# Irish-77/adapting-2D-ViTs-for-3D-point-cloud-understanding

Measured on NVIDIA B200. Metric: tokenized clouds/sec (FPS+kNN+embed), higher is better.
Workload: dtype bf16

## Files before the change

### __graft_entry__.py

```python
import os
import sys

ROOT = os.path.dirname(os.path.abspath(__file__))
PKG = os.path.join(ROOT, "adapting-2d-vits-for-3d-point-cloud-understanding_b200")
for _p in (ROOT, PKG):
    if _p not in sys.path:
        sys.path.insert(0, _p)


def build() -> None:
    from p3tok import _build
    path = _build.build_library()
    print(f"[build] {path}")
    from oracle import oracle
    print(f"[build] {oracle.build()} (test oracle)")
    import p3tok
    from p3tok import _lib
    L = _lib.lib()
    missing = [s for s in _lib.declared_symbols() if not hasattr(L, s)]
    if missing:
        raise RuntimeError(f"libp3tok.so does not export {missing}")
    print(f"[build] ok: {len(_lib.declared_symbols())} C-ABI symbols exported")
    n = fps_fused_multiply_adds(path)
    if n:
        raise RuntimeError(f"fps_kernel SASS holds {n} fused multiply-adds: ptxas contracted the distance arithmetic, "
                           "FPS would no longer be bit-exact (csrc/fps.cu)")
    print("[build] ok: fps_kernel distance arithmetic is unfused (no FFMA / FFMA2 in its SASS)")


def fps_fused_multiply_adds(lib_path: str) -> int:
    import re
    import subprocess
    out = subprocess.run(["cuobjdump", "-sass", lib_path], capture_output=True, text=True).stdout
    n, inside = 0, False
    for line in out.splitlines():
        if "Function :" in line:
            inside = "fps_kernel" in line or "fps_culled_kernel" in line or "fps_nd_kernel" in line
        elif inside and re.search(r"\bFFMA2?\b", line):
            n += 1
    return n


def smoke() -> None:
    import numpy as np
    import torch
    from oracle import oracle
    from p3tok import synth
    from p3tok.modules import PointNet, P3Embed

    assert torch.cuda.is_available(), "smoke() needs a CUDA device"
    dev = torch.device("cuda:0")
    B, N, C, G, k, E = 4, 512, 3, 32, 16, 64
    x = synth.make_cloud("clustered", B, N, 77, C)
    start = synth.start_indices(B, N, 77)
    sd = synth.apf_encoder_state(E, 2 * C, 77)
    ref_tok, grp = oracle.pointnet_apf(sd, x, start, G, k)
    xt, st = torch.from_numpy(x).to(dev), torch.from_numpy(start).to(dev)
    for prec, rtol in (("fp32", 1e-4), ("bf16", 1e-2)):
        net = PointNet(E, G, k, 2 * C, precision=prec).eval().to(dev)
        net.encoder.load_state_dict(synth.to_torch_state(sd))
        fidx, ctr, kidx, perm = net.group.indices(xt, st)
        assert np.array_equal(fidx.cpu().numpy(), grp["fps_idx"]), "FPS indices differ from the oracle"
        assert np.array_equal(kidx.cpu().numpy(), grp["knn_idx"]), "kNN indices differ from the oracle"
        assert np.array_equal(perm.cpu().numpy(), grp["perm"]), "Morton order differs from the oracle"
        try:
            tok = net(xt, st).cpu().numpy().astype(np.float64)
        except Exception as e:
            if prec == "bf16" and "not built yet" in str(e):
                print("[smoke] bf16 path not built yet - skipped")
                continue
            raise
        err = np.abs(tok - ref_tok).max() / np.abs(ref_tok).max()
        print(f"[smoke] PointNet {prec}: max err / max|ref| = {err:.3e}")
        assert err < rtol, f"{prec} tokens off by {err}"
    sd2 = synth.p3embed_state(3, 1 / 16, 4, 4, 64, 78)
    mod = P3Embed(sample_ratio=1 / 16, k=8, embed_dim=64).eval().to(dev)
    mod.load_state_dict(synth.to_torch_state(sd2))
    starts = [synth.start_indices(B, N, 78, 0), synth.start_indices(B, N // 4, 78, 1)]
    ps, fs = mod(xt, xt.transpose(1, 2).contiguous(), [torch.from_numpy(s).to(dev) for s in starts])
    op, of, _ = oracle.p3embed(sd2, x, x.copy(), starts, 8, 2)
    for s in (1, 2):
        assert np.array_equal(ps[s].cpu().numpy(), op[s]), "P3Embed centres differ"
        a, b = fs[s].transpose(1, 2).cpu().numpy(), of[s]
        err = np.abs(a - b).max() / np.abs(b).max()
        print(f"[smoke] P3Embed stage {s - 1}: max err / max|ref| = {err:.3e}")
        assert err < 1e-4
    sd3 = synth.p3embed_state(3, 1 / 16, 4, 4, 256, 79)
    mod3 = P3Embed(sample_ratio=1 / 16, k=32, embed_dim=256, precision="bf16").eval().to(dev)
    mod3.load_state_dict(synth.to_torch_state(sd3))
    x3 = synth.make_cloud("uniform", 2, 1024, 79, 3)
    starts3 = [synth.start_indices(2, 1024, 79, 0), synth.start_indices(2, 256, 79, 1)]
    x3t = torch.from_numpy(x3).to(dev)
    ps3, fs3 = mod3(x3t, x3t.transpose(1, 2).contiguous(), [torch.from_numpy(s).to(dev) for s in starts3])
    op3, of3, _ = oracle.p3embed(sd3, x3, x3.copy(), starts3, 32, 2)
    for s in (1, 2):
        assert np.array_equal(ps3[s].cpu().numpy(), op3[s]), "P3Embed (bf16) centres differ"
        a, b = fs3[s].transpose(1, 2).cpu().numpy(), of3[s]
        err = np.abs(a - b).max() / np.abs(b).max()
        print(f"[smoke] P3Embed bf16 stage {s - 1}: max err / max|ref| = {err:.3e}")
        assert err < 1e-2 * s
    from p3tok.apf_model import APFViTLayer, run_blocks
    sdv = synth.apf_vit_state(E, 2, 15, 80)
    tsd = synth.to_torch_state(sdv)
    blocks = torch.nn.Sequential(*[APFViTLayer(E, 2) for _ in range(2)]).eval().to(dev)
    blocks.load_state_dict({k_[len("blocks."):]: v for k_, v in tsd.items() if k_.startswith("blocks.")})
    norm = torch.nn.LayerNorm(E).eval().to(dev)
    norm.load_state_dict({"weight": tsd["encoder_norm.weight"], "bias": tsd["encoder_norm.bias"]})
    tokv = synth.vit_tokens(B, G, E, 80)
    _, pooled = run_blocks(blocks, torch.from_numpy(tokv).to(dev), norm)
    _, op_, _ = oracle.apf_vit(sdv, tokv, 2, 2)
    err = np.abs(pooled.cpu().numpy() - op_).max() / np.abs(op_).max()
    print(f"[smoke] APF ViT block stack (2 layers): max err / max|ref| = {err:.3e}")
    assert err < 1e-2
    torch.cuda.synchronize()
    print("[smoke] ok")


if __name__ == "__main__":
    build()
    if "--smoke" in sys.argv:
        smoke()
```

### adapting-2d-vits-for-3d-point-cloud-understanding_b200/csrc/fps.cu

```cuda
#include <stdlib.h>

#include <cooperative_groups.h>
#include <cuda/ptx>

#include "common.cuh"

namespace cg = cooperative_groups;

namespace p3tok {

constexpr int FPS_PPT = 8;
constexpr int FPS_CL_PPT = 16;
constexpr int FPS_WIDE_PPT = 24;
constexpr int FPS_MAX_THREADS = 1024;
constexpr int FPS_SLICE = FPS_PPT * FPS_MAX_THREADS;
constexpr int FPS_SLICE_X = FPS_WIDE_PPT * 512;
constexpr int fps_max_threads(int ppt) { return ppt == FPS_WIDE_PPT ? 512 : FPS_SLICE / ppt; }

#ifdef P3TOK_FPS_TRACE
__device__ long long fps_trace_buf[16 * 32];
#define FPS_T(slot)                                                                                       \
  do {                                                                                                    \
    if (g == 100 && cloud == 0 && lane == 0 && (warp == 0 || warp == 5))                                  \
      fps_trace_buf[rank * 32 + (warp ? 16 : 0) + (slot)] = clock64();                                    \
    if ((slot) == 0 && (g == 200 || g == 1200) && cloud == 0 && t == 0)                                   \
      fps_trace_buf[rank * 32 + (g == 200 ? 8 : 9)] = clock64();                                          \
  } while (0)
#else
#define FPS_T(slot) do { } while (0)
#endif

struct __align__(16) FpsCand {
  uint32_t key;
  uint32_t idx;
  float x, y, z;
  uint32_t pad[3];
};

__device__ __forceinline__ void warp_argmax(uint32_t& key, uint32_t& idx) {
  const uint32_t m = __reduce_max_sync(0xffffffffu, key);
  const uint32_t cand = (key == m) ? idx : 0xffffffffu;
  idx = __reduce_min_sync(0xffffffffu, cand);
  key = m;
}

__device__ __forceinline__ uint32_t fps_smem_u32(const void* p) { return (uint32_t)__cvta_generic_to_shared(p); }
__device__ __forceinline__ void fps_push_cand(const FpsCand* local_slot, uint64_t* local_bar, uint32_t dst_cta, const FpsCand& c) {
  uint32_t ra, rb;
  asm volatile("mapa.shared::cluster.u32 %0, %1, %2;" : "=r"(ra) : "r"(fps_smem_u32(local_slot)), "r"(dst_cta));
  asm volatile("mapa.shared::cluster.u32 %0, %1, %2;" : "=r"(rb) : "r"(fps_smem_u32(local_bar)), "r"(dst_cta));
  asm volatile("st.async.weak.shared::cluster.mbarrier::complete_tx::bytes.v4.b32 [%0], {%2, %3, %4, %5}, [%1];" ::"r"(ra), "r"(rb),
               "r"(c.key), "r"(c.idx), "r"(__float_as_uint(c.x)), "r"(__float_as_uint(c.y))
               : "memory");
  asm volatile("st.async.weak.shared::cluster.mbarrier::complete_tx::bytes.v4.b32 [%0], {%2, %3, %4, %5}, [%1];" ::"r"(ra + 16), "r"(rb),
               "r"(__float_as_uint(c.z)), "r"(0u), "r"(0u), "r"(0u)
               : "memory");
}
__device__ __forceinline__ void fps_expect_cands(uint64_t* bar, uint32_t bytes) {
  asm volatile("mbarrier.arrive.expect_tx.shared::cta.b64 _, [%0], %1;" ::"r"(fps_smem_u32(bar)), "r"(bytes) : "memory");
}
__device__ __forceinline__ void fps_wait_cands(uint64_t* bar, uint32_t parity) {
  uint32_t ok = 0;
  while (!ok) {
    asm volatile(
        "{\n\t"
        ".reg .pred p;\n\t"
        "mbarrier.try_wait.parity.acquire.cluster.shared::cta.b64 p, [%1], %2;\n\t"
        "selp.u32 %0, 1, 0, p;\n\t"
        "}"
        : "=r"(ok)
        : "r"(fps_smem_u32(bar)), "r"(parity)
        : "memory");
  }
}

__device__ __forceinline__ void fps_add2(float& o0, float& o1, float a0, float a1, float b0, float b1) {
  asm("{ .reg .b64 ra, rb, rd; mov.b64 ra, {%2,%3}; mov.b64 rb, {%4,%5}; add.rn.f32x2 rd, ra, rb; mov.b64 {%0,%1}, rd; }"
      : "=f"(o0), "=f"(o1)
      : "f"(a0), "f"(a1), "f"(b0), "f"(b1));
}
__device__ __forceinline__ void fps_mul2(float& o0, float& o1, float a0, float a1, float b0, float b1) {
  asm("{ .reg .b64 ra, rb, rd; mov.b64 ra, {%2,%3}; mov.b64 rb, {%4,%5}; mul.rn.f32x2 rd, ra, rb; mov.b64 {%0,%1}, rd; }"
      : "=f"(o0), "=f"(o1)
      : "f"(a0), "f"(a1), "f"(b0), "f"(b1));
}

template <int CL, int PPT = FPS_PPT>
__global__ void __launch_bounds__(fps_max_threads(PPT), 1)
fps_kernel(const float* __restrict__ x, int N, int pt_stride, const int64_t* __restrict__ start_idx,
           int G, int64_t* __restrict__ out_idx, int slice, int ncta) {
  extern __shared__ __align__(128) unsigned char smem_raw[];
  float* rows = reinterpret_cast<float*>(smem_raw);
  const int rows_bytes = ((slice * pt_stride * 4 + 127) / 128) * 128;
  uint64_t* mbar = reinterpret_cast<uint64_t*>(smem_raw + rows_bytes);
  uint2* wslot = reinterpret_cast<uint2*>(smem_raw + rows_bytes + 16);
  FpsCand* ccand = reinterpret_cast<FpsCand*>(smem_raw + rows_bytes + 16 + 2 * 32 * sizeof(uint2));
  uint64_t* cbar = reinterpret_cast<uint64_t*>(ccand + 2 * 16);
  FpsCand* cwin = reinterpret_cast<FpsCand*>(cbar + 2);

  const int T = blockDim.x;
  const int t = threadIdx.x;
  const int lane = t & 31, warp = t >> 5, nwarps = T >> 5;
  int cloud, rank;
  if constexpr (CL > 1) {
    rank = (int)cg::this_cluster().block_rank();
    cloud = blockIdx.x / ncta;
  } else {
    rank = 0;
    cloud = blockIdx.x;
  }
  const int p0 = rank * slice;
  const int np = max(0, min(slice, N - p0));
  const float* src = x + ((size_t)cloud * N + p0) * pt_stride;

  const size_t bytes = (size_t)np * pt_stride * 4;
  const bool tma_ok = (bytes > 0) && (bytes % 16 == 0) && ((reinterpret_cast<uintptr_t>(src) & 15) == 0);
  if (tma_ok) {
    if (t == 0) {
      cuda::ptx::mbarrier_init(mbar, 1);
      cuda::ptx::fence_proxy_async(cuda::ptx::space_shared);
    }
    __syncthreads();
    if (t == 0) {
      cuda::ptx::mbarrier_arrive_expect_tx(cuda::ptx::sem_release, cuda::ptx::scope_cta,
                                           cuda::ptx::space_shared, mbar, (uint32_t)bytes);
      cuda::ptx::cp_async_bulk(cuda::ptx::space_cluster, cuda::ptx::space_global, rows, src,
                               (uint32_t)bytes, mbar);
    }
    while (!cuda::ptx::mbarrier_try_wait_parity(mbar, 0)) {
    }
  } else {
    for (int i = t; i < np * pt_stride; i += T) rows[i] = src[i];
    __syncthreads();
  }

  float px[PPT], py[PPT], pz[PPT], md[PPT];
#pragma unroll
  for (int j = 0; j < PPT; ++j) {
    const int i = j * T + t;
    if (i < np) {
      px[j] = rows[i * pt_stride + 0];
      py[j] = rows[i * pt_stride + 1];
      pz[j] = rows[i * pt_stride + 2];
      md[j] = 1e10f;
    } else {
      px[j] = py[j] = pz[j] = 0.f;
      md[j] = -2.f;
    }
  }
  int far = (int)start_idx[cloud];
  far = min(max(far, 0), N - 1);
  float cx, cy, cz;
  if constexpr (CL > 1) {
    cg::cluster_group cluster = cg::this_cluster();
    if (t == 0) {
      cuda::ptx::mbarrier_init(&cbar[0], 1);
      cuda::ptx::mbarrier_init(&cbar[1], 1);
      asm volatile("fence.mbarrier_init.release.cluster;" ::: "memory");
    }
    if (t == 0 && far >= p0 && far < p0 + np) {
      const int l = far - p0;
      FpsCand c;
      c.key = 0; c.idx = (uint32_t)far;
      c.x = rows[l * pt_stride]; c.y = rows[l * pt_stride + 1]; c.z = rows[l * pt_stride + 2];
      c.pad[0] = c.pad[1] = c.pad[2] = 0;
      for (int r = 0; r < ncta; ++r) *cluster.map_shared_rank(&ccand[0], r) = c;
    }
    cluster.sync();
    cx = ccand[0].x; cy = ccand[0].y; cz = ccand[0].z;
    cluster.sync();
  } else {
    cx = rows[far * pt_stride]; cy = rows[far * pt_stride + 1]; cz = rows[far * pt_stride + 2];
  }

  for (int g = 0; g < G; ++g) {
    if (t == 0 && rank == 0) out_idx[(size_t)cloud * G + g] = far;
    if (g == G - 1) break;
    FPS_T(0);
    const float ncx = -cx, ncy = -cy, ncz = -cz;
#pragma unroll
    for (int j = 0; j < PPT; j += 2) {
      float dx0, dx1, dy0, dy1, dz0, dz1;
      fps_add2(dx0, dx1, px[j], px[j + 1], ncx, ncx);
      fps_add2(dy0, dy1, py[j], py[j + 1], ncy, ncy);
      fps_add2(dz0, dz1, pz[j], pz[j + 1], ncz, ncz);
      fps_mul2(dx0, dx1, dx0, dx1, dx0, dx1);
      fps_mul2(dy0, dy1, dy0, dy1, dy0, dy1);
      fps_mul2(dz0, dz1, dz0, dz1, dz0, dz1);
      const float d0 = __fadd_rn(__fadd_rn(dx0, dy0), dz0);
      const float d1 = __fadd_rn(__fadd_rn(dx1, dy1), dz1);
      md[j] = fminf(md[j], d0);
      md[j + 1] = fminf(md[j + 1], d1);
    }
    float best = md[0];
#pragma unroll
    for (int j = 1; j < PPT; ++j) best = fmaxf(best, md[j]);
    uint32_t key = best >= 0.f ? __float_as_uint(best) : 0u;
    uint32_t idx = 0xffffffffu;
    {
      const uint32_t wmax = __reduce_max_sync(0xffffffffu, key);
      if (key == wmax && best >= 0.f) {
        int besti = PPT - 1;
#pragma unroll
        for (int j = PPT - 2; j >= 0; --j) besti = (md[j] == best) ? j : besti;
        idx = (uint32_t)(p0 + besti * T + t);
      }
      idx = __reduce_min_sync(0xffffffffu, idx);
      key = wmax;
    }
    const int buf = g & 1;
    FPS_T(1);
    if (lane == 0) wslot[buf * 32 + warp] = make_uint2(key, idx);
    __syncthreads();
    FPS_T(2);
    {
      const uint2 s = (lane < nwarps) ? wslot[buf * 32 + lane] : make_uint2(0u, 0xffffffffu);
      key = s.x; idx = s.y;
      warp_argmax(key, idx);
    }
    if constexpr (CL > 1) {
      if (warp == 0) {
        if (lane < ncta) {
          FpsCand c;
          c.key = key; c.idx = idx;
          if (idx != 0xffffffffu) {
            const int l = (int)idx - p0;
            c.x = rows[l * pt_stride]; c.y = rows[l * pt_stride + 1]; c.z = rows[l * pt_stride + 2];
          } else {
            c.x = c.y = c.z = 0.f;
          }
          c.pad[0] = c.pad[1] = c.pad[2] = 0;
          if (lane == 0) fps_expect_cands(&cbar[buf], (uint32_t)ncta * 32u);
          fps_push_cand(&ccand[buf * 16 + rank], &cbar[buf], (uint32_t)lane, c);
        }
        FPS_T(3);
        fps_wait_cands(&cbar[buf], (uint32_t)(g >> 1) & 1);
        FPS_T(4);
        uint32_t k2 = lane < ncta ? ccand[buf * 16 + lane].key : 0u;
        uint32_t i2 = lane < ncta ? ccand[buf * 16 + lane].idx : 0xffffffffu;
        const uint32_t mine = i2;
        warp_argmax(k2, i2);
        const uint32_t src = __ffs(__ballot_sync(0xffffffffu, lane < ncta && mine == i2)) - 1;
        if (lane == (int)src) cwin[buf] = ccand[buf * 16 + lane];
        FPS_T(5);
      }
      __syncthreads();
      FPS_T(6);
      far = (int)min(cwin[buf].idx, (uint32_t)(N - 1));
      cx = cwin[buf].x; cy = cwin[buf].y; cz = cwin[buf].z;
    } else {
      far = (int)min(idx, (uint32_t)(N - 1));
      cx = rows[far * pt_stride]; cy = rows[far * pt_stride + 1]; cz = rows[far * pt_stride + 2];
    }
  }
  if constexpr (CL > 1) cg::this_cluster().sync();
}

static size_t fps_smem_bytes(int slice, int pt_stride) {
  const size_t rows_bytes = (((size_t)slice * pt_stride * 4 + 127) / 128) * 128;
  return rows_bytes + 16 + 2 * 32 * sizeof(uint2) + 2 * 16 * sizeof(FpsCand) + 16 + 2 * sizeof(FpsCand);
}

template <int CL, int PPT>
static int fps_configure() {
  static thread_local bool configured[32] = {false};
  int dev = 0;
  P3_CUDA(cudaGetDevice(&dev));
  if (dev < 32 && !configured[dev]) {
    P3_CUDA((cudaFuncSetAttribute(fps_kernel<CL, PPT>, cudaFuncAttributeMaxDynamicSharedMemorySize, 227 * 1024)));
    if (CL > 8) P3_CUDA((cudaFuncSetAttribute(fps_kernel<CL, PPT>, cudaFuncAttributeNonPortableClusterSizeAllowed, 1)));
    configured[dev] = true;
  }
  return P3TOK_OK;
}

template <int CL, int PPT>
static int fps_max_clusters(int ncta, int threads, size_t smem) {
  if (fps_configure<CL, PPT>() != P3TOK_OK) return -1;
  cudaLaunchConfig_t cfg = {};
  cfg.gridDim = dim3((unsigned)(ncta * 64));
  cfg.blockDim = dim3((unsigned)threads);
  cfg.dynamicSmemBytes = smem;
  cudaLaunchAttribute attr[1];
  attr[0].id = cudaLaunchAttributeClusterDimension;
  attr[0].val.clusterDim.x = (unsigned)ncta;
  attr[0].val.clusterDim.y = 1;
  attr[0].val.clusterDim.z = 1;
  cfg.attrs = attr;
  cfg.numAttrs = 1;
  int n = -1;
  if (cudaOccupancyMaxActiveClusters(&n, fps_kernel<CL, PPT>, &cfg) != cudaSuccess) {
    cudaGetLastError();
    return -1;
  }
  return n;
}

template <int CL, int PPT>
static int fps_launch(const float* x, int B, int N, int pt_stride, const int64_t* start, int G,
                      int64_t* out, int slice, int threads, int ncta, cudaStream_t stream) {
  const size_t smem = fps_smem_bytes(slice, pt_stride);
  int rc = fps_configure<CL, PPT>();
  if (rc) return rc;
  const int CLr = ncta;
  cudaLaunchConfig_t cfg = {};
  cfg.gridDim = dim3((unsigned)(B * CLr));
  cfg.blockDim = dim3((unsigned)threads);
  cfg.dynamicSmemBytes = smem;
  cfg.stream = stream;
  cudaLaunchAttribute attr[1];
  attr[0].id = cudaLaunchAttributeClusterDimension;
  attr[0].val.clusterDim.x = (unsigned)CLr;
  attr[0].val.clusterDim.y = 1;
  attr[0].val.clusterDim.z = 1;
  cfg.attrs = attr;
  cfg.numAttrs = CL > 1 ? 1 : 0;
  P3_CUDA((cudaLaunchKernelEx(&cfg, fps_kernel<CL, PPT>, x, N, pt_stride, start, G, out, slice, ncta)));
  count_launch();
  return P3TOK_OK;
}

}

using namespace p3tok;

extern "C" int p3tok_fps(const float* x, int64_t B, int64_t N, int64_t pt_stride,
                         const int64_t* start_idx, int64_t G, int64_t* out_idx, void* stream) {
  P3_REQUIRE(B >= 0 && N > 0 && G >= 0 && pt_stride >= 3, P3TOK_ERR_INVALID,
             "fps: bad shape B=%lld N=%lld G=%lld stride=%lld", (long long)B, (long long)N, (long long)G,
             (long long)pt_stride);
  if (B == 0 || G == 0) return P3TOK_OK;
  P3_REQUIRE(x && start_idx && out_idx, P3TOK_ERR_INVALID, "fps: null pointer");
  P3_REQUIRE(pt_stride <= 4, P3TOK_ERR_UNSUPPORTED, "fps: pt_stride %lld > 4 (pass xyz or xyz+height rows)",
             (long long)pt_stride);
  P3_REQUIRE(N <= (int64_t)FPS_SLICE * 16, P3TOK_ERR_UNSUPPORTED, "fps: N=%lld exceeds 131072", (long long)N);
  P3_REQUIRE(B * 16 < (1ll << 31) && B * G < (1ll << 40), P3TOK_ERR_UNSUPPORTED, "fps: batch too large");
  cudaStream_t s = as_stream(stream);
  const int Bi = (int)B, Ni = (int)N, Gi = (int)G, ps = (int)pt_stride;
  if (N <= FPS_SLICE) {
    static int ppt_env = -1;
    if (ppt_env < 0) { const char* e = getenv("P3TOK_FPS_PPT"); ppt_env = e ? atoi(e) : 0; }
    const int ppt = ppt_env ? ppt_env : (Ni >= 1024 ? 16 : 8);
    int threads = ((Ni + ppt - 1) / ppt + 31) / 32 * 32;
    if (threads < 32) threads = 32;
    if (ppt == 32) return fps_launch<1, 32>(x, Bi, Ni, ps, start_idx, Gi, out_idx, Ni, threads, 1, s);
    if (ppt == 16) return fps_launch<1, 16>(x, Bi, Ni, ps, start_idx, Gi, out_idx, Ni, threads, 1, s);
    return fps_launch<1, 8>(x, Bi, Ni, ps, start_idx, Gi, out_idx, Ni, threads, 1, s);
  }
  const int lo = (Ni + FPS_SLICE_X - 1) / FPS_SLICE_X;
  const int hi = (Ni + FPS_SLICE - 1) / FPS_SLICE <= 8 ? 8 : 16;
  static thread_local int seats[32][17][33];
  int dev = 0;
  P3_CUDA(cudaGetDevice(&dev));
  static int cl_env = -1;
  if (cl_env < 0) { const char* e = getenv("P3TOK_FPS_CLUSTER"); cl_env = e ? atoi(e) : 0; }
  int best_cl = 0, best_threads = 0, best_slice = 0;
  double best_cost = 0;
  for (int cl = hi; cl >= lo && cl >= 1; --cl) {
    if (cl_env >= lo && cl_env <= hi && cl != cl_env) continue;
    const int slice = (Ni + cl - 1) / cl;
    const bool wide = slice > FPS_SLICE;
    if (wide && cl > 8) continue;
    const int ppt = wide ? FPS_WIDE_PPT : FPS_CL_PPT;
    const int threads = ((slice + ppt - 1) / ppt + 31) / 32 * 32;
    if (threads > fps_max_threads(ppt)) continue;
    int n = dev < 32 ? seats[dev][cl][threads / 32] : 0;
    if (n == 0) {
      const size_t sm = fps_smem_bytes(slice, ps);
      n = cl > 8 ? fps_max_clusters<16, FPS_CL_PPT>(cl, threads, sm)
                 : wide ? fps_max_clusters<8, FPS_WIDE_PPT>(cl, threads, sm) : fps_max_clusters<8, FPS_CL_PPT>(cl, threads, sm);
      if (n <= 0) n = -1;
      if (dev < 32) seats[dev][cl][threads / 32] = n;
    }
    if (n < 0) n = 148 / cl;
    const double cost = (double)((Bi + n - 1) / n) * (1000.0 + 0.11 * slice);
    if (best_cl == 0 || cost < best_cost) { best_cl = cl; best_cost = cost; best_threads = threads; best_slice = slice; }
  }
  P3_REQUIRE(best_cl > 0, P3TOK_ERR_UNSUPPORTED, "fps: no cluster size for N=%lld", (long long)N);
  if (best_cl > 8) return fps_launch<16, FPS_CL_PPT>(x, Bi, Ni, ps, start_idx, Gi, out_idx, best_slice, best_threads, best_cl, s);
  if (best_slice > FPS_SLICE)
    return fps_launch<8, FPS_WIDE_PPT>(x, Bi, Ni, ps, start_idx, Gi, out_idx, best_slice, best_threads, best_cl, s);
  return fps_launch<8, FPS_CL_PPT>(x, Bi, Ni, ps, start_idx, Gi, out_idx, best_slice, best_threads, best_cl, s);
}
```

### adapting-2d-vits-for-3d-point-cloud-understanding_b200/csrc/group.cu

```cuda
#include "common.cuh"

namespace p3tok {

__global__ void gather_points_kernel(const float* __restrict__ x, int64_t N, int C,
                                     const int64_t* __restrict__ idx, int64_t S, int64_t total,
                                     float* __restrict__ out) {
  for (int64_t e = blockIdx.x * (int64_t)blockDim.x + threadIdx.x; e < total;
       e += (int64_t)gridDim.x * blockDim.x) {
    const int c = (int)(e % C);
    const int64_t bs = e / C;
    const int64_t b = bs / S;
    out[e] = x[(b * N + idx[bs]) * C + c];
  }
}

__global__ void apf_group_kernel(const float* __restrict__ x, int64_t N, int C,
                                 const int64_t* __restrict__ fps_idx, const int64_t* __restrict__ knn_idx,
                                 const int64_t* __restrict__ perm, int64_t G, int k, int64_t total,
                                 float* __restrict__ neigh, float* __restrict__ center) {
  const int C2 = 2 * C;
  for (int64_t e = blockIdx.x * (int64_t)blockDim.x + threadIdx.x; e < total;
       e += (int64_t)gridDim.x * blockDim.x) {
    const int c = (int)(e % C2);
    const int64_t r = e / C2;
    const int n = (int)(r % k);
    const int64_t bj = r / k;
    const int64_t b = bj / G;
    const int64_t g = perm ? perm[bj] : (bj - b * G);
    const int64_t ci = fps_idx[b * G + g];
    const float* crow = x + (b * N + ci) * C;
    float v;
    if (c < C) {
      const int64_t ni = knn_idx[(b * G + g) * k + n];
      v = __fsub_rn(x[(b * N + ni) * C + c], crow[c]);
    } else {
      v = crow[c - C];
    }
    neigh[e] = v;
    if (n == 0 && c < 3) center[bj * 3 + c] = crow[c];
  }
}

__global__ void group_gather_kernel(const float* __restrict__ pnts, const float* __restrict__ feats,
                                    int64_t N, int D, const int32_t* __restrict__ idx, int64_t G, int k,
                                    int64_t rows, float* __restrict__ gp, float* __restrict__ gf) {
  const int W = 3 + D;
  const int64_t total = rows * W;
  for (int64_t e = blockIdx.x * (int64_t)blockDim.x + threadIdx.x; e < total;
       e += (int64_t)gridDim.x * blockDim.x) {
    const int c = (int)(e % W);
    const int64_t r = e / W;
    const int64_t b = r / (G * k);
    const int64_t ni = idx[r];
    if (c < 3) gp[r * 3 + c] = pnts[(b * N + ni) * 3 + c];
    else gf[r * D + (c - 3)] = feats[(b * N + ni) * D + (c - 3)];
  }
}

__device__ __forceinline__ int64_t part1by2(int64_t n) {
  n = n & 0x000003ff;
  n = (n ^ (n << 16)) & 0xff0000ff;
  n = (n ^ (n << 8)) & 0x0300f00f;
  n = (n ^ (n << 4)) & 0x030c30c3;
  n = (n ^ (n << 2)) & 0x09249249;
  return n;
}

__global__ void __launch_bounds__(1024)
morton_kernel(const float* __restrict__ centres, int G, int P2, int64_t* __restrict__ perm,
              int64_t* __restrict__ codes_out) {
  extern __shared__ uint64_t keys[];
  __shared__ float red[2][3][32];
  __shared__ float mnmx[2][3];
  const int b = blockIdx.x, t = threadIdx.x, lane = t & 31, warp = t >> 5, nw = blockDim.x >> 5;
  const float* Cn = centres + (size_t)b * G * 3;
  float mn[3] = {3.4e38f, 3.4e38f, 3.4e38f}, mx[3] = {-3.4e38f, -3.4e38f, -3.4e38f};
  for (int g = t; g < G; g += blockDim.x)
#pragma unroll
    for (int a = 0; a < 3; ++a) {
      const float v = Cn[g * 3 + a];
      mn[a] = fminf(mn[a], v);
      mx[a] = fmaxf(mx[a], v);
    }
#pragma unroll
  for (int a = 0; a < 3; ++a) {
#pragma unroll
    for (int o = 16; o > 0; o >>= 1) {
      mn[a] = fminf(mn[a], __shfl_xor_sync(0xffffffffu, mn[a], o));
      mx[a] = fmaxf(mx[a], __shfl_xor_sync(0xffffffffu, mx[a], o));
    }
    if (lane == 0) { red[0][a][warp] = mn[a]; red[1][a][warp] = mx[a]; }
  }
  __syncthreads();
  if (warp == 0) {
#pragma unroll
    for (int a = 0; a < 3; ++a) {
      float m0 = lane < nw ? red[0][a][lane] : 3.4e38f, m1 = lane < nw ? red[1][a][lane] : -3.4e38f;
#pragma unroll
      for (int o = 16; o > 0; o >>= 1) {
        m0 = fminf(m0, __shfl_xor_sync(0xffffffffu, m0, o));
        m1 = fmaxf(m1, __shfl_xor_sync(0xffffffffu, m1, o));
      }
      if (lane == 0) { mnmx[0][a] = m0; mnmx[1][a] = m1; }
    }
  }
  __syncthreads();
  for (int g = t; g < P2; g += blockDim.x) {
    uint64_t key = 0xffffffffffffffffull;
    if (g < G) {
      int64_t q[3];
#pragma unroll
      for (int a = 0; a < 3; ++a) {
        const float num = __fsub_rn(Cn[g * 3 + a], mnmx[0][a]);
        const float den = __fadd_rn(__fsub_rn(mnmx[1][a], mnmx[0][a]), 1e-8f);
        const float sc = __fmul_rn(__fdiv_rn(num, den), 1023.0f);
        q[a] = (int64_t)sc;
      }
      const int64_t code = (part1by2(q[2]) << 2) + (part1by2(q[1]) << 1) + part1by2(q[0]);
      if (codes_out) codes_out[(size_t)b * G + g] = code;
      key = ((uint64_t)code << 32) | (uint32_t)g;
    }
    keys[g] = key;
  }
  __syncthreads();
  for (int k = 2; k <= P2; k <<= 1)
    for (int j = k >> 1; j > 0; j >>= 1) {
      for (int i = t; i < P2; i += blockDim.x) {
        const int p = i ^ j;
        if (p > i) {
          const uint64_t a = keys[i], c = keys[p];
          const bool up = (i & k) == 0;
          if ((a > c) == up) { keys[i] = c; keys[p] = a; }
        }
      }
      __syncthreads();
    }
  for (int g = t; g < G; g += blockDim.x) perm[(size_t)b * G + g] = (int64_t)(keys[g] & 0xffffffffu);
}

static inline unsigned blocks_for(int64_t total, int threads) {
  int64_t b = (total + threads - 1) / threads;
  const int64_t cap = 148 * 16;
  return (unsigned)(b < 1 ? 1 : (b > cap ? cap : b));
}

}

using namespace p3tok;

extern "C" int p3tok_gather_points(const float* x, int64_t B, int64_t N, int64_t C, const int64_t* idx,
                                   int64_t S, float* out, void* stream) {
  P3_REQUIRE(B >= 0 && N > 0 && C > 0 && S >= 0, P3TOK_ERR_INVALID, "gather_points: bad shape");
  const int64_t total = B * S * C;
  if (total == 0) return P3TOK_OK;
  P3_REQUIRE(x && idx && out, P3TOK_ERR_INVALID, "gather_points: null pointer");
  gather_points_kernel<<<blocks_for(total, 256), 256, 0, as_stream(stream)>>>(x, N, (int)C, idx, S, total, out);
  P3_LAUNCH_CHECK("gather_points_kernel");
  return P3TOK_OK;
}

extern "C" int p3tok_apf_group(const float* x, int64_t B, int64_t N, int64_t C, const int64_t* fps_idx,
                               const int64_t* knn_idx, const int64_t* perm, int64_t G, int64_t k,
                               float* neigh, float* center, void* stream) {
  P3_REQUIRE(B >= 0 && N > 0 && C >= 3 && G >= 0 && k > 0, P3TOK_ERR_INVALID, "apf_group: bad shape");
  const int64_t total = B * G * k * 2 * C;
  if (total == 0) return P3TOK_OK;
  P3_REQUIRE(x && fps_idx && knn_idx && neigh && center, P3TOK_ERR_INVALID, "apf_group: null pointer");
  apf_group_kernel<<<blocks_for(total, 256), 256, 0, as_stream(stream)>>>(x, N, (int)C, fps_idx, knn_idx, perm, G,
                                                                          (int)k, total, neigh, center);
  P3_LAUNCH_CHECK("apf_group_kernel");
  return P3TOK_OK;
}

extern "C" int p3tok_group_gather(const float* pnts, const float* feats, int64_t B, int64_t N, int64_t D,
                                  const int32_t* idx, int64_t G, int64_t k, float* gp, float* gf, void* stream) {
  P3_REQUIRE(B >= 0 && N > 0 && D >= 0 && G >= 0 && k > 0, P3TOK_ERR_INVALID, "group_gather: bad shape");
  const int64_t rows = B * G * k;
  if (rows == 0) return P3TOK_OK;
  P3_REQUIRE(pnts && idx && gp && (D == 0 || (feats && gf)), P3TOK_ERR_INVALID, "group_gather: null pointer");
  group_gather_kernel<<<blocks_for(rows * (3 + D), 256), 256, 0, as_stream(stream)>>>(pnts, feats, N, (int)D, idx, G,
                                                                                     (int)k, rows, gp, gf);
  P3_LAUNCH_CHECK("group_gather_kernel");
  return P3TOK_OK;
}

extern "C" int p3tok_morton_order(const float* centres, int64_t B, int64_t G, int64_t* perm, int64_t* codes_out,
                                  void* stream) {
  P3_REQUIRE(B >= 0 && G > 0, P3TOK_ERR_INVALID, "morton_order: bad shape");
  P3_REQUIRE(G <= 8192, P3TOK_ERR_UNSUPPORTED, "morton_order: G=%lld > 8192", (long long)G);
  if (B == 0) return P3TOK_OK;
  P3_REQUIRE(centres && perm, P3TOK_ERR_INVALID, "morton_order: null pointer");
  int P2 = 1;
  while (P2 < G) P2 <<= 1;
  int threads = P2 < 64 ? 64 : (P2 > 1024 ? 1024 : P2);
  const size_t smem = (size_t)P2 * 8;
  if (smem > 48 * 1024) P3_CUDA(cudaFuncSetAttribute(morton_kernel, cudaFuncAttributeMaxDynamicSharedMemorySize, 64 * 1024));
  morton_kernel<<<(unsigned)B, threads, smem, as_stream(stream)>>>(centres, (int)G, P2, perm, codes_out);
  P3_LAUNCH_CHECK("morton_kernel");
  return P3TOK_OK;
}
```

### adapting-2d-vits-for-3d-point-cloud-understanding_b200/csrc/knn.cu

```cuda
#include <stdlib.h>

#include "common.cuh"

namespace p3tok {

constexpr int KNN_WARPS = 8;
constexpr int KNN_CPW = 4;
constexpr int KNN_TILE = 2048;
constexpr uint64_t KNN_SENTINEL = 0xffffffffffffffffull;

__device__ __forceinline__ uint64_t shfl_xor_u64(uint64_t v, int m) {
  uint32_t lo = (uint32_t)v, hi = (uint32_t)(v >> 32);
  lo = __shfl_xor_sync(0xffffffffu, lo, m);
  hi = __shfl_xor_sync(0xffffffffu, hi, m);
  return ((uint64_t)hi << 32) | lo;
}
__device__ __forceinline__ uint64_t shfl_u64(uint64_t v, int src) {
  uint32_t lo = (uint32_t)v, hi = (uint32_t)(v >> 32);
  lo = __shfl_sync(0xffffffffu, lo, src);
  hi = __shfl_sync(0xffffffffu, hi, src);
  return ((uint64_t)hi << 32) | lo;
}
__device__ __forceinline__ uint64_t umin64(uint64_t a, uint64_t b) { return a < b ? a : b; }
__device__ __forceinline__ uint64_t umax64(uint64_t a, uint64_t b) { return a < b ? b : a; }

__device__ __forceinline__ uint64_t warp_sort_asc(uint64_t v, int lane) {
#pragma unroll
  for (int k = 2; k <= 32; k <<= 1) {
#pragma unroll
    for (int j = k >> 1; j > 0; j >>= 1) {
      const uint64_t o = shfl_xor_u64(v, j);
      const bool up = ((lane & k) == 0);
      const bool lower = ((lane & j) == 0);
      v = (up == lower) ? umin64(v, o) : umax64(v, o);
    }
  }
  return v;
}
__device__ __forceinline__ uint64_t warp_bitonic_merge_asc(uint64_t v, int lane) {
#pragma unroll
  for (int j = 16; j > 0; j >>= 1) {
    const uint64_t o = shfl_xor_u64(v, j);
    v = ((lane & j) == 0) ? umin64(v, o) : umax64(v, o);
  }
  return v;
}

template <int KPL>
__device__ __forceinline__ void list_insert_run(uint64_t (&L)[KPL], uint64_t q, int lane) {
#pragma unroll
  for (int j = 0; j < KPL; ++j) {
    const uint64_t r = shfl_u64(q, 31 - lane);
    const uint64_t lo = umin64(L[j], r);
    if (j + 1 < KPL) {
      const uint64_t hi = umax64(L[j], r);
      q = warp_bitonic_merge_asc(hi, lane);
    }
    L[j] = warp_bitonic_merge_asc(lo, lane);
  }
}

template <int KPL, int MODE>
__global__ void __launch_bounds__(KNN_WARPS * 32)
knn_kernel(const float* __restrict__ x, int N, int pt_stride, const float* __restrict__ centres, int G,
           int k, void* __restrict__ idx_out, int idx_is_i64, float* __restrict__ dist_out) {
  __shared__ float4 tile[KNN_TILE];
  __shared__ uint64_t queue[KNN_WARPS * KNN_CPW][64];

  const int t = threadIdx.x, lane = t & 31, warp = t >> 5;
  const int b = blockIdx.y;
  const int g0 = (blockIdx.x * KNN_WARPS + warp) * KNN_CPW;
  const float* P = x + (size_t)b * N * pt_stride;

  float c0[KNN_CPW], c1[KNN_CPW], c2[KNN_CPW], cn[KNN_CPW];
#pragma unroll
  for (int c = 0; c < KNN_CPW; ++c) {
    const int g = min(g0 + c, G - 1);
    const float* cp = centres + ((size_t)b * G + g) * 3;
    const float cx = cp[0], cy = cp[1], cz = cp[2];
    cn[c] = sq3(cx, cy, cz);
    if (MODE == P3TOK_KNN_APF_SQ) {
      c0[c] = cx; c1[c] = cy; c2[c] = cz;
    } else {
      c0[c] = __fmul_rn(-2.f, cx); c1[c] = __fmul_rn(-2.f, cy); c2[c] = __fmul_rn(-2.f, cz);
    }
  }

  uint64_t L[KNN_CPW][KPL];
  float thr[KNN_CPW];
  float thr_d[KNN_CPW];
  int qn[KNN_CPW];
#pragma unroll
  for (int c = 0; c < KNN_CPW; ++c) {
#pragma unroll
    for (int j = 0; j < KPL; ++j) L[c][j] = KNN_SENTINEL;
    thr[c] = __int_as_float(0x7f800000);
    thr_d[c] = __int_as_float(0x7f800000);
    qn[c] = 0;
  }
  const int kth_lane = (k - 1) & 31, kth_j = (k - 1) >> 5;

  auto merge_queue = [&](int c, uint64_t (&Lc)[KPL], int cnt) {
    uint64_t* q = queue[warp * KNN_CPW + c];
    uint64_t v = (lane < cnt) ? q[lane] : KNN_SENTINEL;
    v = warp_sort_asc(v, lane);
    list_insert_run<KPL>(Lc, v, lane);
    uint64_t kth = 0;
#pragma unroll
    for (int j = 0; j < KPL; ++j)
      if (j == kth_j) kth = shfl_u64(Lc[j], kth_lane);
    const uint32_t ko = (uint32_t)(kth >> 32);
    const float kd = (ko == 0xffffffffu) ? __int_as_float(0x7f800000) : ord2f(ko);
    return kd;
  };

  for (int base = 0; base < N; base += KNN_TILE) {
    __syncthreads();
    const int cnt = min(KNN_TILE, N - base);
    for (int i = t; i < cnt; i += KNN_WARPS * 32) {
      const float* pp = P + (size_t)(base + i) * pt_stride;
      const float px = pp[0], py = pp[1], pz = pp[2];
      tile[i] = make_float4(px, py, pz, sq3(px, py, pz));
    }
    __syncthreads();
    if (g0 >= G) continue;
    for (int i0 = 0; i0 < cnt; i0 += 32) {
      const int i = i0 + lane;
      const bool valid = i < cnt;
      const float4 p = tile[valid ? i : 0];
      float dc[KNN_CPW];
      bool pc[KNN_CPW];
      bool any = false;
#pragma unroll
      for (int c = 0; c < KNN_CPW; ++c) {
        if (MODE == P3TOK_KNN_APF_SQ) {
          const float dot = __fmaf_rn(c2[c], p.z, __fmaf_rn(c1[c], p.y, __fmul_rn(c0[c], p.x)));
          float tt = __fmul_rn(-2.f, dot);
          tt = __fadd_rn(tt, cn[c]);
          dc[c] = __fadd_rn(__fadd_rn(tt, p.w), 0.f);
          pc[c] = valid && (dc[c] < thr[c]);
        } else {
          float tt = __fmul_rn(c0[c], p.x);
          tt = __fmaf_rn(c1[c], p.y, tt);
          tt = __fmaf_rn(c2[c], p.z, tt);
          tt = __fadd_rn(tt, cn[c]);
          tt = __fadd_rn(tt, p.w);
          dc[c] = tt;
          pc[c] = valid && (tt <= thr[c]);
        }
        any = any || pc[c];
      }
      if (!__any_sync(0xffffffffu, any)) continue;
#pragma unroll
      for (int c = 0; c < KNN_CPW; ++c) {
        float d = dc[c];
        bool pass = pc[c];
        uint32_t ball = __ballot_sync(0xffffffffu, pass);
        if (ball == 0) continue;
        if (MODE == P3TOK_KNN_P4P_CDIST) {
          d = __fadd_rn(__fsqrt_rn(fmaxf(d, 0.f)), 0.f);
          pass = pass && (d < thr_d[c]);
          ball = __ballot_sync(0xffffffffu, pass);
          if (ball == 0) continue;
        }
        uint64_t* q = queue[warp * KNN_CPW + c];
        if (pass) {
          const int pos = qn[c] + __popc(ball & ((1u << lane) - 1u));
          q[pos] = ((uint64_t)f2ord(d) << 32) | (uint32_t)(base + i);
        }
        qn[c] += __popc(ball);
        __syncwarp();
        if (qn[c] >= 32) {
          const float kd = merge_queue(c, L[c], 32);
          __syncwarp();
          if (lane + 32 < qn[c]) q[lane] = q[lane + 32];
          qn[c] -= 32;
          __syncwarp();
          if (MODE == P3TOK_KNN_APF_SQ) {
            thr[c] = kd;
          } else {
            thr_d[c] = kd;
            thr[c] = (kd == __int_as_float(0x7f800000)) ? kd
                     : __fmul_ru(__fmul_ru(kd, kd), 1.0000002384185791f);
          }
        }
      }
    }
  }
  if (g0 >= G) return;
#pragma unroll
  for (int c = 0; c < KNN_CPW; ++c) {
    if (qn[c] > 0) (void)merge_queue(c, L[c], qn[c]);
    const int g = g0 + c;
    if (g >= G) continue;
    const size_t o = ((size_t)b * G + g) * k;
#pragma unroll
    for (int j = 0; j < KPL; ++j) {
      const int r = j * 32 + lane;
      if (r < k) {
        const uint32_t id = (uint32_t)L[c][j];
        if (idx_is_i64) reinterpret_cast<int64_t*>(idx_out)[o + r] = (int64_t)id;
        else reinterpret_cast<int32_t*>(idx_out)[o + r] = (int32_t)id;
        if (dist_out) dist_out[o + r] = ord2f((uint32_t)(L[c][j] >> 32));
      }
    }
  }
}

template <int KPL>
static int knn_launch(const float* x, int B, int N, int pt_stride, const float* centres, int G, int k,
                      int mode, void* idx_out, int i64, float* dist_out, cudaStream_t s) {
  dim3 grid((unsigned)((G + KNN_WARPS * KNN_CPW - 1) / (KNN_WARPS * KNN_CPW)), (unsigned)B);
  if (mode == P3TOK_KNN_APF_SQ)
    knn_kernel<KPL, P3TOK_KNN_APF_SQ><<<grid, KNN_WARPS * 32, 0, s>>>(x, N, pt_stride, centres, G, k, idx_out, i64, dist_out);
  else
    knn_kernel<KPL, P3TOK_KNN_P4P_CDIST><<<grid, KNN_WARPS * 32, 0, s>>>(x, N, pt_stride, centres, G, k, idx_out, i64, dist_out);
  P3_LAUNCH_CHECK("knn_kernel");
  return P3TOK_OK;
}


#ifndef KNS_MIN_BLOCKS
#define KNS_MIN_BLOCKS 5
#endif
constexpr int KNS_MAX_N = 8192;
constexpr int KNS_MAX_SEG = 16;
constexpr int KNS_CELLS = 512;

struct KnsLayout {
  int64_t S, seg, nblk_seg;
  int64_t off_pts, off_ids, off_bb, off_lut, off_meta, total;
};
static KnsLayout kns_layout(int64_t B, int64_t N) {
  KnsLayout L;
  L.S = (N + KNS_MAX_N - 1) / KNS_MAX_N;
  L.seg = (N + L.S - 1) / L.S;
  L.nblk_seg = (L.seg + 31) / 32;
  const int64_t nblk = L.S * L.nblk_seg;
  int64_t o = 0;
  L.off_pts = o; o += B * nblk * 32 * 16;
  L.off_ids = o; o += B * nblk * 32 * 4;
  L.off_bb = o; o += B * nblk * 32;
  L.off_lut = o; o += B * L.S * (KNS_CELLS + 1) * 4;
  L.off_meta = o; o += B * L.S * 32;
  L.total = o + 256;
  return L;
}

__device__ __forceinline__ uint32_t kns_part1by2(uint32_t n) {
  n &= 0x000003ff;
  n = (n ^ (n << 16)) & 0xff0000ff;
  n = (n ^ (n << 8)) & 0x0300f00f;
  n = (n ^ (n << 4)) & 0x030c30c3;
  n = (n ^ (n << 2)) & 0x09249249;
  return n;
}
__device__ __forceinline__ uint32_t kns_code(float x, float y, float z, const float* meta) {
  const int qx = min(1023, max(0, (int)((x - meta[0]) * meta[3])));
  const int qy = min(1023, max(0, (int)((y - meta[1]) * meta[4])));
  const int qz = min(1023, max(0, (int)((z - meta[2]) * meta[5])));
  return (kns_part1by2((uint32_t)qz) << 2) | (kns_part1by2((uint32_t)qy) << 1) | kns_part1by2((uint32_t)qx);
}

__global__ void __launch_bounds__(1024)
knn_prep_kernel(const float* __restrict__ x, int Ntot, int S, int seg, int nblk, int pt_stride, int P2, float4* __restrict__ pts,
                int* __restrict__ ids, float* __restrict__ bb, int* __restrict__ lut, float* __restrict__ meta_out) {
  extern __shared__ uint64_t keys[];
  __shared__ float red[7][32];
  __shared__ float meta[8];
  __shared__ int slut[KNS_CELLS + 1];
  const int b = blockIdx.x, t = threadIdx.x, lane = t & 31, warp = t >> 5, nw = blockDim.x >> 5, T = blockDim.x;
  const int cloud = b / S, id0 = (b - cloud * S) * seg;
  const int N = min(seg, Ntot - id0);
  const float* P = x + ((size_t)cloud * Ntot + id0) * pt_stride;
  float mn[3] = {3.4e38f, 3.4e38f, 3.4e38f}, mx[3] = {-3.4e38f, -3.4e38f, -3.4e38f}, wmax = 0.f;
  for (int i = t; i < N; i += T) {
    const float px = P[(size_t)i * pt_stride], py = P[(size_t)i * pt_stride + 1], pz = P[(size_t)i * pt_stride + 2];
    mn[0] = fminf(mn[0], px); mx[0] = fmaxf(mx[0], px);
    mn[1] = fminf(mn[1], py); mx[1] = fmaxf(mx[1], py);
    mn[2] = fminf(mn[2], pz); mx[2] = fmaxf(mx[2], pz);
    wmax = fmaxf(wmax, sq3(px, py, pz));
  }
#pragma unroll
  for (int o = 16; o > 0; o >>= 1) {
#pragma unroll
    for (int a = 0; a < 3; ++a) {
      mn[a] = fminf(mn[a], __shfl_xor_sync(0xffffffffu, mn[a], o));
      mx[a] = fmaxf(mx[a], __shfl_xor_sync(0xffffffffu, mx[a], o));
    }
    wmax = fmaxf(wmax, __shfl_xor_sync(0xffffffffu, wmax, o));
  }
  if (lane == 0) {
#pragma unroll
    for (int a = 0; a < 3; ++a) { red[a][warp] = mn[a]; red[3 + a][warp] = mx[a]; }
    red[6][warp] = wmax;
  }
  __syncthreads();
  if (warp == 0) {
    float v[7];
#pragma unroll
    for (int a = 0; a < 7; ++a) v[a] = lane < nw ? red[a][lane] : (a < 3 ? 3.4e38f : (a < 6 ? -3.4e38f : 0.f));
#pragma unroll
    for (int o = 16; o > 0; o >>= 1) {
#pragma unroll
      for (int a = 0; a < 7; ++a) {
        const float u = __shfl_xor_sync(0xffffffffu, v[a], o);
        v[a] = a < 3 ? fminf(v[a], u) : fmaxf(v[a], u);
      }
    }
    if (lane == 0) {
#pragma unroll
      for (int a = 0; a < 3; ++a) {
        meta[a] = v[a];
        const float ext = v[3 + a] - v[a];
        meta[3 + a] = ext > 0.f ? 1023.f / ext : 0.f;
      }
      meta[6] = v[6];
      meta[7] = 0.f;
    }
  }
  for (int c = t; c <= KNS_CELLS; c += T) slut[c] = N;
  __syncthreads();
  if (t < 8) meta_out[(size_t)b * 8 + t] = meta[t];
  for (int i = t; i < P2; i += T) {
    uint64_t key = 0xffffffffffffffffull;
    if (i < N) key = ((uint64_t)kns_code(P[(size_t)i * pt_stride], P[(size_t)i * pt_stride + 1], P[(size_t)i * pt_stride + 2], meta) << 32) | (uint32_t)i;
    keys[i] = key;
  }
  __syncthreads();
  int prev_j = 32;
  for (int kk = 2; kk <= P2; kk <<= 1) {
    for (int j = kk >> 1; j > 0; j >>= 1) {
      if (j >= 32 || prev_j >= 32) __syncthreads();
      else __syncwarp();
      for (int i = t; i < P2; i += T) {
        const int ixj = i ^ j;
        if (ixj > i) {
          const uint64_t a = keys[i], c = keys[ixj];
          const bool up = (i & kk) == 0;
          if ((a > c) == up) { keys[i] = c; keys[ixj] = a; }
        }
      }
      prev_j = j;
    }
  }
  __syncthreads();
  for (int j0 = warp * 32; j0 < nblk * 32; j0 += nw * 32) {
    const int j = j0 + lane;
    float4 pt = make_float4(0.f, 0.f, 0.f, __int_as_float(0x7fc00000));
    int id = -1;
    float lo[3] = {3.4e38f, 3.4e38f, 3.4e38f}, hi[3] = {-3.4e38f, -3.4e38f, -3.4e38f};
    if (j < N) {
      const uint64_t key = keys[j];
      id = (int)(uint32_t)key;
      const float px = P[(size_t)id * pt_stride], py = P[(size_t)id * pt_stride + 1], pz = P[(size_t)id * pt_stride + 2];
      pt = make_float4(px, py, pz, sq3(px, py, pz));
      lo[0] = hi[0] = px; lo[1] = hi[1] = py; lo[2] = hi[2] = pz;
      const int cell = (int)(key >> (32 + 21));
      const int prev = j > 0 ? (int)(keys[j - 1] >> (32 + 21)) : -1;
      if (cell != prev) slut[cell] = j;
    }
    pts[((size_t)b * nblk) * 32 + j] = pt;
    ids[((size_t)b * nblk) * 32 + j] = id < 0 ? id : id + id0;
#pragma unroll
    for (int o = 16; o > 0; o >>= 1) {
#pragma unroll
      for (int a = 0; a < 3; ++a) {
        lo[a] = fminf(lo[a], __shfl_xor_sync(0xffffffffu, lo[a], o));
        hi[a] = fmaxf(hi[a], __shfl_xor_sync(0xffffffffu, hi[a], o));
      }
    }
    if (lane < 8) {
      const float v = lane < 3 ? lo[lane] : (lane < 6 ? hi[lane - 3] : 0.f);
      bb[(((size_t)b * nblk) + (j0 >> 5)) * 8 + lane] = v;
    }
  }
  __syncthreads();
  if (t == 0) {
    for (int c = KNS_CELLS - 1; c >= 0; --c) slut[c] = min(slut[c], slut[c + 1]);
  }
  __syncthreads();
  for (int c = t; c <= KNS_CELLS; c += T) lut[(size_t)b * (KNS_CELLS + 1) + c] = slut[c];
}

template <int KPL, int MODE>
__global__ void __launch_bounds__(KNN_WARPS * 32, KPL == 1 ? KNS_MIN_BLOCKS : 4)
knn_sorted_kernel(const float4* __restrict__ pts, const int* __restrict__ ids, const float* __restrict__ bb,
                  const int* __restrict__ lut, const float* __restrict__ meta_all, int S, int nblk, const float* __restrict__ centres,
                  int G, int64_t total, int k, void* __restrict__ idx_out, int idx_is_i64, float* __restrict__ dist_out, int best_first) {
  __shared__ uint64_t queue[KNN_WARPS][64];
  const int lane = threadIdx.x & 31, warp = threadIdx.x >> 5;
  const int64_t cw = (int64_t)blockIdx.x * KNN_WARPS + warp;
  if (cw >= total) return;
  const int b = (int)(cw / G);
  const float* cp = centres + (size_t)cw * 3;
  const float cx = cp[0], cy = cp[1], cz = cp[2];
  const float cn = sq3(cx, cy, cz);
  float c0, c1, c2;
  if (MODE == P3TOK_KNN_APF_SQ) { c0 = cx; c1 = cy; c2 = cz; }
  else { c0 = __fmul_rn(-2.f, cx); c1 = __fmul_rn(-2.f, cy); c2 = __fmul_rn(-2.f, cz); }

  uint64_t L[KPL];
#pragma unroll
  for (int j = 0; j < KPL; ++j) L[j] = KNN_SENTINEL;
  float thr = __int_as_float(0x7f800000);
  float thr_d = __int_as_float(0x7f800000);
  int qn = 0;
  const int kth_lane = (k - 1) & 31, kth_j = (k - 1) >> 5;
  uint64_t* q = queue[warp];

  auto merge = [&](int cnt) {
    uint64_t v = (lane < cnt) ? q[lane] : KNN_SENTINEL;
    v = warp_sort_asc(v, lane);
    list_insert_run<KPL>(L, v, lane);
    uint64_t kth = 0;
#pragma unroll
    for (int j = 0; j < KPL; ++j)
      if (j == kth_j) kth = shfl_u64(L[j], kth_lane);
    const uint32_t ko = (uint32_t)(kth >> 32);
    const float kd = (ko == 0xffffffffu) ? __int_as_float(0x7f800000) : ord2f(ko);
    if (MODE == P3TOK_KNN_APF_SQ) {
      thr = kd;
    } else {
      thr_d = kd;
      thr = (kd == __int_as_float(0x7f800000)) ? kd : __fmul_ru(__fmul_ru(kd, kd), 1.0000002384185791f);
    }
  };
  auto process = [&](const float4 p, const int id) {
    float d;
    bool pass;
    if (MODE == P3TOK_KNN_APF_SQ) {
      const float dot = __fmaf_rn(c2, p.z, __fmaf_rn(c1, p.y, __fmul_rn(c0, p.x)));
      float tt = __fmul_rn(-2.f, dot);
      tt = __fadd_rn(tt, cn);
      d = __fadd_rn(__fadd_rn(tt, p.w), 0.f);
      pass = (id >= 0) && (d <= thr);
    } else {
      float tt = __fmul_rn(c0, p.x);
      tt = __fmaf_rn(c1, p.y, tt);
      tt = __fmaf_rn(c2, p.z, tt);
      tt = __fadd_rn(tt, cn);
      tt = __fadd_rn(tt, p.w);
      d = tt;
      pass = (id >= 0) && (tt <= thr);
    }
    uint32_t ball = __ballot_sync(0xffffffffu, pass);
    if (ball == 0) return;
    if (MODE == P3TOK_KNN_P4P_CDIST) {
      d = __fadd_rn(__fsqrt_rn(fmaxf(d, 0.f)), 0.f);
      pass = pass && (d <= thr_d);
      ball = __ballot_sync(0xffffffffu, pass);
      if (ball == 0) return;
    }
    if (pass) q[qn + __popc(ball & ((1u << lane) - 1u))] = ((uint64_t)f2ord(d) << 32) | (uint32_t)id;
    qn += __popc(ball);
    __syncwarp();
    if (qn >= 32) {
      merge(32);
      __syncwarp();
      if (lane + 32 < qn) q[lane] = q[lane + 32];
      qn -= 32;
      __syncwarp();
    }
  };

  for (int sg = 0; sg < S; ++sg) {
  const size_t bs = (size_t)b * S + sg;
  const float* meta = meta_all + bs * 8;
  const float4* P4 = pts + bs * nblk * 32;
  const int* ID = ids + bs * nblk * 32;
  const float* BB = bb + bs * nblk * 8;
  const float margin = 1e-5f * (cn + meta[6]) + 1e-30f;
  if (best_first && nblk >= 128) {
    for (int r0 = 0; r0 < nblk; r0 += 256) {
      uint32_t key[8];
#pragma unroll
      for (int u = 0; u < 8; ++u) {
        const int blk = r0 + u * 32 + lane;
        key[u] = 0xffffffffu;
        if (blk < nblk) {
          const float4 lo = *reinterpret_cast<const float4*>(BB + (size_t)blk * 8);
          const float4 hi = *reinterpret_cast<const float4*>(BB + (size_t)blk * 8 + 4);
          const float dx = fmaxf(fmaxf(lo.x - cx, cx - lo.w), 0.f);
          const float dy = fmaxf(fmaxf(lo.y - cy, cy - hi.x), 0.f);
          const float dz = fmaxf(fmaxf(lo.z - cz, cz - hi.y), 0.f);
          const float lb = fmaxf((dx * dx + dy * dy + dz * dz) * 0.999999f - margin, 0.f);
          if (lb <= thr) key[u] = (__float_as_uint(lb) & 0xffffff00u) | (uint32_t)(u * 32 + lane);
        }
      }
      while (true) {
        uint32_t m = key[0];
#pragma unroll
        for (int u = 1; u < 8; ++u) m = min(m, key[u]);
        const uint32_t w = __reduce_min_sync(0xffffffffu, m);
        if (w == 0xffffffffu) break;
        if (__uint_as_float(w & 0xffffff00u) > thr) break;
        const int id = (int)(w & 0xffu);
#pragma unroll
        for (int u = 0; u < 8; ++u)
          if (u == (id >> 5) && lane == (id & 31)) key[u] = 0xffffffffu;
        const int bk = r0 + id;
        process(P4[bk * 32 + lane], ID[bk * 32 + lane]);
      }
    }
    continue;
  }
  const int cell = (int)(kns_code(cx, cy, cz, meta) >> 21);
  const int pos = lut[bs * (KNS_CELLS + 1) + cell];
  int s0 = (pos >> 5) - 1;
  s0 = max(0, min(s0, nblk - 3));
  const int s1 = min(nblk, s0 + 3);
  {
    float4 sp[3];
    int si[3];
#pragma unroll
    for (int u = 0; u < 3; ++u) {
      const int blk = min(s0 + u, nblk - 1);
      sp[u] = P4[blk * 32 + lane];
      si[u] = ID[blk * 32 + lane];
    }
#pragma unroll
    for (int u = 0; u < 3; ++u)
      if (s0 + u < s1) process(sp[u], si[u]);
  }

  for (int r0 = 0; r0 < nblk; r0 += 32) {
    const int blk = r0 + lane;
    float lb = __int_as_float(0x7f800000);
    const bool mine = blk < nblk && (blk < s0 || blk >= s1);
    if (mine) {
      const float4 lo = *reinterpret_cast<const float4*>(BB + (size_t)blk * 8);
      const float4 hi = *reinterpret_cast<const float4*>(BB + (size_t)blk * 8 + 4);
      const float dx = fmaxf(fmaxf(lo.x - cx, cx - lo.w), 0.f);
      const float dy = fmaxf(fmaxf(lo.y - cy, cy - hi.x), 0.f);
      const float dz = fmaxf(fmaxf(lo.z - cz, cz - hi.y), 0.f);
      lb = (dx * dx + dy * dy + dz * dz) * 0.999999f - margin;
    }
    uint32_t todo = __ballot_sync(0xffffffffu, mine && lb <= thr);
    while (todo) {
      const int bit = __ffs(todo) - 1;
      todo &= todo - 1;
      const float lbb = __shfl_sync(0xffffffffu, lb, bit);
      if (lbb > thr) continue;
      const int bk = r0 + bit;
      process(P4[bk * 32 + lane], ID[bk * 32 + lane]);
    }
  }
  }
  if (qn > 0) merge(qn);
  const int g = (int)(cw - (int64_t)b * G);
  const size_t o = ((size_t)b * G + g) * k;
#pragma unroll
  for (int j = 0; j < KPL; ++j) {
    const int r = j * 32 + lane;
    if (r < k) {
      const uint32_t id = (uint32_t)L[j];
      if (idx_is_i64) reinterpret_cast<int64_t*>(idx_out)[o + r] = (int64_t)id;
      else reinterpret_cast<int32_t*>(idx_out)[o + r] = (int32_t)id;
      if (dist_out) dist_out[o + r] = ord2f((uint32_t)(L[j] >> 32));
    }
  }
}

template <int KPL>
static int knn_sorted_launch(const float4* pts, const int* ids, const float* bb, const int* lut, const float* meta, int S, int nblk,
                             const float* centres, int G, int64_t total, int k, int mode, void* idx_out, int i64, float* dist_out,
                             cudaStream_t s) {
  const unsigned grid = (unsigned)((total + KNN_WARPS - 1) / KNN_WARPS);
  static int bf = -1;
  if (bf < 0) { const char* e = getenv("P3TOK_KNN_BEST_FIRST"); bf = e ? atoi(e) : 1; }
  if (mode == P3TOK_KNN_APF_SQ)
    knn_sorted_kernel<KPL, P3TOK_KNN_APF_SQ><<<grid, KNN_WARPS * 32, 0, s>>>(pts, ids, bb, lut, meta, S, nblk, centres, G, total, k, idx_out, i64, dist_out, bf);
  else
    knn_sorted_kernel<KPL, P3TOK_KNN_P4P_CDIST><<<grid, KNN_WARPS * 32, 0, s>>>(pts, ids, bb, lut, meta, S, nblk, centres, G, total, k, idx_out, i64, dist_out, bf);
  P3_LAUNCH_CHECK("knn_sorted_kernel");
  return P3TOK_OK;
}

}

using namespace p3tok;

extern "C" int p3tok_knn(const float* x, int64_t B, int64_t N, int64_t pt_stride, const float* centres,
                         int64_t G, int64_t k, int mode, void* idx_out, int idx_dtype, float* dist_out,
                         void* stream) {
  P3_REQUIRE(B >= 0 && N > 0 && G >= 0 && pt_stride >= 3, P3TOK_ERR_INVALID, "knn: bad shape");
  P3_REQUIRE(mode == P3TOK_KNN_APF_SQ || mode == P3TOK_KNN_P4P_CDIST, P3TOK_ERR_INVALID, "knn: bad mode %d", mode);
  P3_REQUIRE(idx_dtype == P3TOK_I64 || idx_dtype == P3TOK_I32, P3TOK_ERR_INVALID, "knn: idx dtype must be i32/i64");
  P3_REQUIRE(k >= 1 && k <= N, P3TOK_ERR_INVALID, "knn: k=%lld out of range for N=%lld", (long long)k, (long long)N);
  P3_REQUIRE(k <= 128, P3TOK_ERR_UNSUPPORTED, "knn: k=%lld > 128", (long long)k);
  P3_REQUIRE(N < (1ll << 31) && B < 65536, P3TOK_ERR_UNSUPPORTED, "knn: N or B too large");
  if (B == 0 || G == 0) return P3TOK_OK;
  P3_REQUIRE(x && centres && idx_out, P3TOK_ERR_INVALID, "knn: null pointer");
  cudaStream_t s = as_stream(stream);
  const int i64 = idx_dtype == P3TOK_I64;
  if (k <= 32) return knn_launch<1>(x, (int)B, (int)N, (int)pt_stride, centres, (int)G, (int)k, mode, idx_out, i64, dist_out, s);
  if (k <= 64) return knn_launch<2>(x, (int)B, (int)N, (int)pt_stride, centres, (int)G, (int)k, mode, idx_out, i64, dist_out, s);
  return knn_launch<4>(x, (int)B, (int)N, (int)pt_stride, centres, (int)G, (int)k, mode, idx_out, i64, dist_out, s);
}

extern "C" int64_t p3tok_knn_workspace_bytes(int64_t B, int64_t N) {
  if (B < 0 || N <= 0 || N > (int64_t)KNS_MAX_N * KNS_MAX_SEG) return 0;
  return kns_layout(B, N).total;
}

struct KnsPtrs {
  float4* pts; int* ids; float* bb; int* lut; float* meta;
};
static KnsPtrs kns_ptrs(void* workspace, int64_t B, int64_t N) {
  const KnsLayout L = kns_layout(B, N);
  char* base = reinterpret_cast<char*>((reinterpret_cast<uintptr_t>(workspace) + 255) & ~(uintptr_t)255);
  KnsPtrs p;
  p.pts = reinterpret_cast<float4*>(base + L.off_pts);
  p.ids = reinterpret_cast<int*>(base + L.off_ids);
  p.bb = reinterpret_cast<float*>(base + L.off_bb);
  p.lut = reinterpret_cast<int*>(base + L.off_lut);
  p.meta = reinterpret_cast<float*>(base + L.off_meta);
  return p;
}

namespace p3tok {
int kns_workspace_views(const void* workspace, int64_t workspace_bytes, int64_t B, int64_t N, const float4** pts, const int** ids,
                        const float** bb) {
  P3_REQUIRE(N > 0 && N <= KNS_MAX_N && B >= 0, P3TOK_ERR_UNSUPPORTED, "sorted workspace: N=%lld outside (0, %d]", (long long)N, KNS_MAX_N);
  P3_REQUIRE(workspace_bytes >= kns_layout(B, N).total, P3TOK_ERR_WORKSPACE, "sorted workspace %lld < %lld bytes",
             (long long)workspace_bytes, (long long)kns_layout(B, N).total);
  const KnsPtrs w = kns_ptrs(const_cast<void*>(workspace), B, N);
  *pts = w.pts; *ids = w.ids; *bb = w.bb;
  return P3TOK_OK;
}
}

extern "C" int p3tok_knn_prepare(const float* x, int64_t B, int64_t N, int64_t pt_stride, void* workspace, int64_t workspace_bytes,
                                 void* stream) {
  P3_REQUIRE(B >= 0 && N > 0 && pt_stride >= 3, P3TOK_ERR_INVALID, "knn_prepare: bad shape");
  P3_REQUIRE(N <= (int64_t)KNS_MAX_N * KNS_MAX_SEG, P3TOK_ERR_UNSUPPORTED, "knn_prepare: N=%lld > %d (use p3tok_knn)", (long long)N,
             KNS_MAX_N * KNS_MAX_SEG);
  P3_REQUIRE(B < 65536, P3TOK_ERR_UNSUPPORTED, "knn_prepare: B too large");
  if (B == 0) return P3TOK_OK;
  P3_REQUIRE(x && workspace, P3TOK_ERR_INVALID, "knn_prepare: null pointer");
  P3_REQUIRE(workspace_bytes >= kns_layout(B, N).total, P3TOK_ERR_WORKSPACE, "knn_prepare: workspace %lld < %lld bytes",
             (long long)workspace_bytes, (long long)kns_layout(B, N).total);
  const KnsPtrs w = kns_ptrs(workspace, B, N);
  const KnsLayout L = kns_layout(B, N);
  int P2 = 32;
  while (P2 < L.seg) P2 <<= 1;
  const int threads = P2 > 1024 ? 1024 : P2;
  const size_t smem = (size_t)P2 * 8;
  static thread_local bool configured[32] = {false};
  int dev = 0;
  P3_CUDA(cudaGetDevice(&dev));
  if (dev < 32 && !configured[dev]) {
    P3_CUDA(cudaFuncSetAttribute(knn_prep_kernel, cudaFuncAttributeMaxDynamicSharedMemorySize, KNS_MAX_N * 8));
    configured[dev] = true;
  }
  knn_prep_kernel<<<(unsigned)(B * L.S), threads, smem, as_stream(stream)>>>(x, (int)N, (int)L.S, (int)L.seg, (int)L.nblk_seg, (int)pt_stride,
                                                                              P2, w.pts, w.ids, w.bb, w.lut, w.meta);
  P3_LAUNCH_CHECK("knn_prep_kernel");
  return P3TOK_OK;
}

extern "C" int p3tok_knn_query(const void* workspace, int64_t workspace_bytes, int64_t B, int64_t N, const float* centres, int64_t G,
                               int64_t k, int mode, void* idx_out, int idx_dtype, float* dist_out, void* stream) {
  P3_REQUIRE(B >= 0 && N > 0 && G >= 0, P3TOK_ERR_INVALID, "knn_query: bad shape");
  P3_REQUIRE(mode == P3TOK_KNN_APF_SQ || mode == P3TOK_KNN_P4P_CDIST, P3TOK_ERR_INVALID, "knn_query: bad mode %d", mode);
  P3_REQUIRE(idx_dtype == P3TOK_I64 || idx_dtype == P3TOK_I32, P3TOK_ERR_INVALID, "knn_query: idx dtype must be i32/i64");
  P3_REQUIRE(k >= 1 && k <= N, P3TOK_ERR_INVALID, "knn_query: k=%lld out of range for N=%lld", (long long)k, (long long)N);
  P3_REQUIRE(k <= 128, P3TOK_ERR_UNSUPPORTED, "knn_query: k=%lld > 128", (long long)k);
  P3_REQUIRE(N <= (int64_t)KNS_MAX_N * KNS_MAX_SEG, P3TOK_ERR_UNSUPPORTED, "knn_query: N=%lld > %d (use p3tok_knn)", (long long)N,
             KNS_MAX_N * KNS_MAX_SEG);
  if (B == 0 || G == 0) return P3TOK_OK;
  P3_REQUIRE(centres && idx_out && workspace, P3TOK_ERR_INVALID, "knn_query: null pointer");
  P3_REQUIRE(workspace_bytes >= kns_layout(B, N).total, P3TOK_ERR_WORKSPACE, "knn_query: workspace %lld < %lld bytes",
             (long long)workspace_bytes, (long long)kns_layout(B, N).total);
  const KnsPtrs w = kns_ptrs(const_cast<void*>(workspace), B, N);
  cudaStream_t s = as_stream(stream);
  const int i64 = idx_dtype == P3TOK_I64;
  const int64_t total = B * G;
  const KnsLayout L = kns_layout(B, N);
  const int S = (int)L.S, nb = (int)L.nblk_seg;
  if (k <= 32) return knn_sorted_launch<1>(w.pts, w.ids, w.bb, w.lut, w.meta, S, nb, centres, (int)G, total, (int)k, mode, idx_out, i64, dist_out, s);
  if (k <= 64) return knn_sorted_launch<2>(w.pts, w.ids, w.bb, w.lut, w.meta, S, nb, centres, (int)G, total, (int)k, mode, idx_out, i64, dist_out, s);
  return knn_sorted_launch<4>(w.pts, w.ids, w.bb, w.lut, w.meta, S, nb, centres, (int)G, total, (int)k, mode, idx_out, i64, dist_out, s);
}

extern "C" int p3tok_knn_sorted(const float* x, int64_t B, int64_t N, int64_t pt_stride, const float* centres, int64_t G,
                                int64_t k, int mode, void* idx_out, int idx_dtype, float* dist_out, void* workspace,
                                int64_t workspace_bytes, void* stream) {
  P3_REQUIRE(k >= 1 && k <= N, P3TOK_ERR_INVALID, "knn_sorted: k=%lld out of range for N=%lld", (long long)k, (long long)N);
  if (B == 0 || G == 0) return P3TOK_OK;
  int rc = p3tok_knn_prepare(x, B, N, pt_stride, workspace, workspace_bytes, stream);
  if (rc) return rc;
  return p3tok_knn_query(workspace, workspace_bytes, B, N, centres, G, k, mode, idx_out, idx_dtype, dist_out, stream);
}
```

### adapting-2d-vits-for-3d-point-cloud-understanding_b200/p3tok/_build.py

```python
from __future__ import annotations

import concurrent.futures as cf
import os
import shutil
import subprocess
from typing import List

_PKG = os.path.dirname(os.path.abspath(__file__))
_ROOT = os.path.dirname(os.path.dirname(_PKG))
CSRC = os.path.join(os.path.dirname(_PKG), "csrc")
INCLUDE = os.path.join(_ROOT, "include")
LIB_PATH = os.path.join(_PKG, "libp3tok.so")
OBJ_DIR = os.path.join(CSRC, "_obj")

SOURCES = ["capi.cu", "fps.cu", "fps_culled.cu", "fps_nd.cu", "sqdist.cu", "knn.cu", "group.cu", "mlp_f32.cu", "embed_tc.cu", "embed_fused.cu", "embed_stage.cu", "embed_gather.cu", "vit.cu", "train.cu", "train_vit.cu"]
NVCC_FLAGS = [
    "-gencode", "arch=compute_100a,code=sm_100a", "-lineinfo", "-O3", "-std=c++17",
    "--expt-extended-lambda", "--expt-relaxed-constexpr", "-Xcompiler", "-fPIC",
    "-Xcompiler", "-fvisibility=hidden", "-I", INCLUDE, "-I", CSRC,
]


def _nvcc() -> str:
    for cand in (os.environ.get("NVCC"), shutil.which("nvcc"), "/usr/local/cuda/bin/nvcc"):
        if cand and os.path.isfile(cand):
            return cand
    raise RuntimeError("nvcc not found; libp3tok.so must be built where the CUDA toolkit is installed")


def _newer(target: str, deps: List[str]) -> bool:
    if not os.path.isfile(target):
        return True
    t = os.path.getmtime(target)
    return any(os.path.getmtime(d) > t for d in deps)


def build_library(force: bool = False, verbose: bool = False) -> str:
    os.makedirs(OBJ_DIR, exist_ok=True)
    extra = []
    if os.environ.get("P3TOK_EPI_WARPS"):
        extra = ["-DP3TOK_EPI_WARPS=" + os.environ["P3TOK_EPI_WARPS"]]
        force = True
    headers = [os.path.join(CSRC, f) for f in os.listdir(CSRC) if f.endswith((".cuh", ".h"))]
    headers += [os.path.join(INCLUDE, f) for f in os.listdir(INCLUDE)]
    nvcc = _nvcc()
    jobs = []
    objs = []
    for src in SOURCES:
        s = os.path.join(CSRC, src)
        o = os.path.join(OBJ_DIR, src.replace(".cu", ".o"))
        objs.append(o)
        if force or _newer(o, [s] + headers):
            jobs.append([nvcc] + NVCC_FLAGS + extra + (["-Xptxas", "-v"] if verbose else []) + ["-c", s, "-o", o])

    def run(cmd):
        r = subprocess.run(cmd, capture_output=True, text=True)
        if r.returncode != 0:
            raise RuntimeError("nvcc failed:\n" + " ".join(cmd) + "\n" + r.stdout + r.stderr)
        return r.stderr

    if jobs:
        with cf.ThreadPoolExecutor(max_workers=min(len(jobs), os.cpu_count() or 1)) as ex:
            for out in ex.map(run, jobs):
                if verbose and out:
                    print(out)
    if jobs or force or _newer(LIB_PATH, objs):
        run([nvcc, "-shared", "-o", LIB_PATH] + objs + ["-gencode", "arch=compute_100a,code=sm_100a"])
    return LIB_PATH


if __name__ == "__main__":
    import sys
    print(build_library(force="--force" in sys.argv, verbose="-v" in sys.argv))
```

### adapting-2d-vits-for-3d-point-cloud-understanding_b200/p3tok/_lib.py

```python
from __future__ import annotations

import ctypes
import os
import re
from typing import List

_PKG = os.path.dirname(os.path.abspath(__file__))
LIB_PATH = os.environ.get("P3TOK_LIB") or os.path.join(_PKG, "libp3tok.so")
HEADER_PATH = os.path.join(os.path.dirname(os.path.dirname(_PKG)), "include", "p3tok.h")

OK, ERR_INVALID, ERR_UNSUPPORTED, ERR_CUDA, ERR_WORKSPACE = 0, 1, 2, 3, 4
KNN_APF_SQ, KNN_P4P_CDIST = 0, 1
F32, BF16, I32, I64, BF16X3 = 0, 1, 2, 3, 4
ROWS_APF, ROWS_P4P, ROWS_DIRECT = 0, 1, 2
EW_AXPBY, EW_MUL, EW_GELU, EW_GELU_BWD, EW_RELU, EW_RELU_BWD = 0, 1, 2, 3, 4, 5

_i32, _i64, _vp, _int = ctypes.c_int32, ctypes.c_int64, ctypes.c_void_p, ctypes.c_int


class MlpStruct(ctypes.Structure):
    _fields_ = [
        ("cin", _i32), ("n_pre", _i32), ("pre_dim", _i32 * 4), ("pre_relu", _i32 * 4),
        ("mid_dim", _i32), ("out_dim", _i32), ("out_relu", _i32), ("wdtype", _i32),
        ("w_pre", _vp * 4), ("b_pre", _vp * 4),
        ("w_mid_g", _vp), ("w_mid_f", _vp), ("b_mid", _vp), ("w_out", _vp), ("b_out", _vp),
    ]


class RowsStruct(ctypes.Structure):
    _fields_ = [
        ("kind", _i32), ("C", _i32), ("D", _i32), ("idx_dtype", _i32),
        ("B", _i64), ("N", _i64), ("G", _i64), ("k", _i64),
        ("x", _vp), ("feats", _vp), ("ctr_idx", _vp), ("knn_idx", _vp), ("perm", _vp),
    ]


class VitLayerStruct(ctypes.Structure):
    _fields_ = [(n, _vp) for n in ("qkv_w", "qkv_b", "proj_w", "proj_b", "fc1d_w", "fc1d_b", "fc2u_w", "fc2u_b")]


_f32 = ctypes.c_float

_SIGNATURES = {
    "p3tok_abi_version": (_int, []),
    "p3tok_last_error": (ctypes.c_char_p, []),
    "p3tok_kernel_launches": (_i64, []),
    "p3tok_fps": (_int, [_vp, _i64, _i64, _i64, _vp, _i64, _vp, _vp]),
    "p3tok_fps_sorted": (_int, [_vp, _i64, _i64, _i64, _vp, _i64, _vp, _vp]),
    "p3tok_fps_nd": (_int, [_vp, _i64, _i64, _i64, _i64, _vp, _i64, _vp, _vp, _vp]),
    "p3tok_square_distance": (_int, [_vp, _i64, _i64, _vp, _i64, _i64, _vp, _vp]),
    "p3tok_gather_points": (_int, [_vp, _i64, _i64, _i64, _vp, _i64, _vp, _vp]),
    "p3tok_knn": (_int, [_vp, _i64, _i64, _i64, _vp, _i64, _i64, _int, _vp, _int, _vp, _vp]),
    "p3tok_knn_workspace_bytes": (_i64, [_i64, _i64]),
    "p3tok_knn_sorted": (_int, [_vp, _i64, _i64, _i64, _vp, _i64, _i64, _int, _vp, _int, _vp, _vp, _i64, _vp]),
    "p3tok_knn_prepare": (_int, [_vp, _i64, _i64, _i64, _vp, _i64, _vp]),
    "p3tok_knn_query": (_int, [_vp, _i64, _i64, _i64, _vp, _i64, _i64, _int, _vp, _int, _vp, _vp]),
    "p3tok_morton_order": (_int, [_vp, _i64, _i64, _vp, _vp, _vp]),
    "p3tok_apf_group": (_int, [_vp, _i64, _i64, _i64, _vp, _vp, _vp, _i64, _i64, _vp, _vp, _vp]),
    "p3tok_group_gather": (_int, [_vp, _vp, _i64, _i64, _i64, _vp, _i64, _i64, _vp, _vp, _vp]),
    "p3tok_patch_embed_workspace_bytes": (_i64, [ctypes.POINTER(MlpStruct), _i64, _i64, _int]),
    "p3tok_patch_embed": (_int, [ctypes.POINTER(RowsStruct), ctypes.POINTER(MlpStruct), _int, _int, _vp, _i64, _vp, _vp]),
    "p3tok_linear_f32": (_int, [_vp, _i64, _i64, _vp, _i64, _vp, _vp, _i64, _int, _vp, _vp]),
    "p3tok_linear_x3_workspace_bytes": (_i64, [_i64, _i64, _i64]),
    "p3tok_linear_x3_f32": (_int, [_vp, _i64, _i64, _vp, _i64, _vp, _vp, _i64, _int, _vp, _vp, _i64, _vp]),
    "p3tok_linear_bf16": (_int, [_vp, _i64, _i64, _vp, _i64, _vp, _vp, _i64, _int, _vp, _vp, _vp, _vp]),
    "p3tok_token_head_f32": (_int, [_vp, _vp, _i64, _i64, _i64, _i64, _i64] + [_vp] * 12),
    "p3tok_group_max": (_int, [_vp, _i64, _i64, _i64, _vp, _vp]),
    "p3tok_linear_tn_f32": (_int, [_vp, _vp, _i64, _i64, _i64, _vp, _int, _vp]),
    "p3tok_colstats_f32": (_int, [_vp, _i64, _i64, _vp, _vp, _vp]),
    "p3tok_bn_act_f32": (_int, [_vp, _i64, _i64, _vp, _vp, _vp, _vp, _int, _vp, _vp]),
    "p3tok_bn_bwd_stats_f32": (_int, [_vp, _vp, _i64, _i64, _vp, _vp, _vp, _vp, _int, _vp, _vp, _vp]),
    "p3tok_bn_bwd_apply_f32": (_int, [_vp, _vp, _i64, _i64, _i64, _vp, _vp, _vp, _vp, _int, _vp, _vp, _vp, _vp]),
    "p3tok_group_max_arg_f32": (_int, [_vp, _i64, _i64, _i64, _vp, _vp, _vp]),
    "p3tok_group_max_bwd_f32": (_int, [_vp, _vp, _i64, _i64, _i64, _int, _vp, _vp]),
    "p3tok_group_sum_f32": (_int, [_vp, _i64, _i64, _i64, _vp, _vp]),
    "p3tok_scatter_rows_add_f32": (_int, [_vp, _vp, _i64, _i64, _i64, _i64, _i64, _vp, _vp, _vp]),
    "p3tok_build_rows_f32": (_int, [ctypes.POINTER(RowsStruct), _vp, _vp]),
    "p3tok_ln_fwd_f32": (_int, [_vp, _i64, _i64, _vp, _vp, _f32, _vp, _vp, _vp, _vp]),
    "p3tok_ln_bwd_f32": (_int, [_vp, _vp, _i64, _i64, _vp, _vp, _vp, _int, _vp, _vp]),
    "p3tok_ln_param_grad_f32": (_int, [_vp, _vp, _i64, _i64, _vp, _vp, _vp, _vp, _vp]),
    "p3tok_attn_fwd_f32": (_int, [_vp, _i64, _i64, _i64, _i64, _f32, _vp, _vp, _vp]),
    "p3tok_attn_bwd_f32": (_int, [_vp, _vp, _vp, _i64, _i64, _i64, _i64, _f32, _vp, _vp, _vp]),
    "p3tok_ew_f32": (_int, [_int, _vp, _vp, _f32, _f32, _i64, _i64, _vp, _vp]),
    "p3tok_apf_vit_workspace_bytes": (_i64, [_i64, _i64, _i64, _i64, _i64]),
    "p3tok_apf_vit_forward": (_int, [_vp, _i64, _i64, _i64, _i64, _i64, _i64, ctypes.POINTER(VitLayerStruct), _i64, _vp, _vp,
                                     _f32, _vp, _vp, _i64, _vp]),
    "p3tok_vit_forward": (_int, [_vp, _i64, _i64, _i64, _i64, _i64, ctypes.POINTER(VitLayerStruct), _i64, _vp, _vp, _vp, _f32, _vp, _vp,
                                 _i64, _vp, _i64, _vp]),
    "p3tok_layernorm_bf16": (_int, [_vp, _i64, _i64, _f32, _vp, _vp, _vp, _vp]),
    "p3tok_attention_bf16": (_int, [_vp, _i64, _i64, _i64, _i64, _vp, _vp]),
    "p3tok_linear_bf16_ex": (_int, [_vp, _i64, _i64, _vp, _i64, _vp, _int, _i64, _vp, _f32, _f32, _vp, _vp, _vp]),
}


def declared_symbols() -> List[str]:
    with open(HEADER_PATH) as f:
        return sorted(set(re.findall(r"P3TOK_API\s+[\w\s\*]+?\b(p3tok_\w+)\s*\(", f.read())))


_lib = None


def lib() -> ctypes.CDLL:
    global _lib
    if _lib is None:
        if not os.path.isfile(LIB_PATH):
            raise RuntimeError(
                f"{LIB_PATH} is missing: build it with `python -c 'import __graft_entry__ as g; g.build()'` "
                "(p3tok has no CPU or eager fallback)")
        L = ctypes.CDLL(LIB_PATH)
        for name, (res, args) in _SIGNATURES.items():
            fn = getattr(L, name)
            fn.restype = res
            fn.argtypes = args
        if L.p3tok_abi_version() != 2:
            raise RuntimeError("libp3tok.so ABI version mismatch; rebuild")
        _lib = L
    return _lib


class P3tokError(RuntimeError):
    pass


def check(rc: int, what: str) -> None:
    if rc != OK:
        msg = lib().p3tok_last_error().decode("utf-8", "replace")
        kind = {ERR_INVALID: "invalid argument", ERR_UNSUPPORTED: "unsupported", ERR_CUDA: "CUDA failure",
                ERR_WORKSPACE: "workspace too small"}.get(rc, f"error {rc}")
        raise P3tokError(f"{what}: {kind}: {msg}")
```

### adapting-2d-vits-for-3d-point-cloud-understanding_b200/p3tok/modules.py

```python
from __future__ import annotations

import math
from typing import List, Optional, Tuple

import torch
from torch import nn

from . import _lib, fold, ops, train
from .functional import _start


def _check_precision(p: str) -> bool:
    if p not in ("fp32", "bf16", "fp32tc"):
        raise ValueError(f"precision must be 'fp32', 'fp32tc' or 'bf16', got {p!r}")
    return p == "bf16"


def _check_token_dtype(token_dtype, precision: str) -> bool:
    if token_dtype in (None, torch.float32):
        return False
    if token_dtype != torch.bfloat16:
        raise ValueError(f"token_dtype must be torch.float32 or torch.bfloat16, got {token_dtype!r}")
    if precision != "bf16":
        raise ValueError("token_dtype=torch.bfloat16 needs precision='bf16'")
    return True


def _bn_eps(module: nn.Module):
    return {name: float(m.eps) for name, m in module.named_modules()
            if isinstance(m, (nn.BatchNorm1d, nn.BatchNorm2d))}


class _FoldedMixin:

    def _folded(self, build, device, bf16: bool) -> fold.PatchMLP:
        ver = tuple((t._version, t.data_ptr()) for t in list(self.parameters()) + list(self.buffers()))
        cache = self.__dict__.setdefault("_fold_cache", {})
        if cache.get("ver") != ver:
            cache.clear()
            cache["ver"] = ver
            cache["host"] = build()
        if getattr(self, "precision", None) == "fp32tc":
            return cache["host"].to_x3(device)
        return cache["host"].to(device, torch.bfloat16 if bf16 else torch.float32)

    def _require_eval(self):
        if self.training:
            raise RuntimeError(
                f"{type(self).__name__}: p3tok implements the eval-mode (folded BatchNorm) forward only; "
                "call .eval() first (training-mode batch statistics are out of scope, SURVEY.md 8f)")


class Group(nn.Module):

    def __init__(self, num_group: int, group_size: int):
        super().__init__()
        self.num_group = num_group
        self.group_size = group_size

    def indices(self, x: torch.Tensor, start_idx: Optional[torch.Tensor] = None):
        fps_idx, ws = ops.fps_with_knn_prepare(x, _start(x, start_idx), self.num_group)
        center = ops.gather_points(x, fps_idx)[..., :3].contiguous() if x.shape[-1] != 3 else ops.gather_points(x, fps_idx)
        knn_idx = ops.knn_query(x, ws, center, self.group_size, _lib.KNN_APF_SQ, False)
        perm = ops.morton_order(center)[0]
        return fps_idx, center, knn_idx, perm

    @staticmethod
    def _xyz_is_prefix_of(x: torch.Tensor, xyz: torch.Tensor) -> bool:
        return (xyz.shape[-1] == 3 and xyz.dtype == x.dtype and xyz.device == x.device and xyz.data_ptr() == x.data_ptr()
                and xyz.stride() == x.stride())

    def forward(self, x: torch.Tensor, xyz: torch.Tensor, start_idx: Optional[torch.Tensor] = None):
        if xyz.shape[:2] != x.shape[:2] or xyz.shape[-1] != 3:
            raise RuntimeError("Group.forward: xyz must be (B,N,3) with x's B and N")
        if x.dtype == torch.float32 and x.is_contiguous() and self._xyz_is_prefix_of(x, xyz):
            fps_idx, _, knn_idx, perm = self.indices(x, start_idx)
            return ops.apf_group(x, fps_idx, knn_idx, perm)
        x = x.float().contiguous()
        pts = xyz.float().contiguous()
        fps_idx, center, knn_idx, perm = self.indices(pts, start_idx)
        neigh, _ = ops.apf_group(x, fps_idx, knn_idx, perm)
        center = torch.gather(center, 1, perm.unsqueeze(-1).expand(-1, -1, 3))
        return neigh, center


class Encoder(nn.Module, _FoldedMixin):

    def __init__(self, encoder_channel: int, in_channel: int, precision: str = "fp32", token_dtype=None, sync_bn: bool = False):
        super().__init__()
        self.encoder_channel = encoder_channel
        self.precision = precision
        self.token_dtype = token_dtype
        self.sync_bn = sync_bn
        E = encoder_channel
        self.first_conv = nn.Sequential(
            nn.Conv1d(in_channel, 256, 1), nn.BatchNorm1d(256), nn.ReLU(inplace=True),
            nn.Conv1d(256, 512, 1), nn.BatchNorm1d(512), nn.ReLU(inplace=True),
            nn.Conv1d(512, E, 1))
        self.second_conv = nn.Sequential(
            nn.Conv1d(2 * E, 2 * E, 1), nn.BatchNorm1d(2 * E), nn.ReLU(inplace=True),
            nn.Conv1d(2 * E, E, 1))

    def folded(self, device) -> fold.PatchMLP:
        return self._folded(lambda: fold.fold_apf_encoder(self.state_dict(), _bn_eps(self)), device,
                            _check_precision(self.precision))

    def forward(self, point_groups: torch.Tensor) -> torch.Tensor:
        B, G, k, cin = point_groups.shape
        if self.training:
            rows = point_groups.float().reshape(B * G * k, cin)
            return train.encoder_train(self, rows, k, self.sync_bn).view(B, G, self.encoder_channel)
        m = self.folded(point_groups.device)
        rows = point_groups.float().reshape(B * G * k, cin)
        tok = ops.patch_embed(_lib.ROWS_DIRECT, rows, None, None, None, None, B * G, k, m.tensors(), m.meta(),
                              _check_precision(self.precision), _check_token_dtype(self.token_dtype, self.precision),
                              self.precision == "fp32tc")
        return tok.view(B, G, self.encoder_channel)

    get_features = forward


class PointNet(nn.Module):

    def __init__(self, embed_dim: int, num_group: int, group_size: int, in_channel: int, precision: str = "fp32",
                 token_dtype=None, sync_bn: bool = False):
        super().__init__()
        self.group = Group(num_group, group_size)
        self.encoder = Encoder(embed_dim, in_channel, precision, token_dtype, sync_bn)

    def forward(self, x: torch.Tensor, start_idx: Optional[torch.Tensor] = None) -> torch.Tensor:
        x = x.float().contiguous()
        B, N, C = x.shape
        G, k = self.group.num_group, self.group.group_size
        with torch.no_grad():
            fps_idx, _, knn_idx, perm = self.group.indices(x, start_idx)
        if self.encoder.training:
            rows = train.apf_rows(x, fps_idx, knn_idx, perm)
            return train.encoder_train(self.encoder, rows, k, self.encoder.sync_bn).view(B, G, -1)
        m = self.encoder.folded(x.device)
        if m.cin != 2 * C:
            raise RuntimeError(f"PointNet: in_channel={m.cin} but input has C={C} (expects in_channel == 2*C)")
        tok = ops.patch_embed(_lib.ROWS_APF, x, None, fps_idx, knn_idx, perm, B * G, k, m.tensors(), m.meta(),
                              _check_precision(self.encoder.precision),
                              _check_token_dtype(self.encoder.token_dtype, self.encoder.precision), self.encoder.precision == "fp32tc")
        return tok.view(B, G, -1)


class P3Embed(nn.Module, _FoldedMixin):

    def __init__(self, in_channels: int = 3, sample_ratio: float = 0.25, scale: int = 4, k: int = 32,
                 layers: int = 4, embed_dim: int = 256, precision: str = "fp32", token_dtype=None, sync_bn: bool = False,
                 **kwargs):
        super().__init__()
        if layers != 4:
            raise ValueError("p3tok P3Embed supports the reference's layers=4 layout only")
        self.sample_ratio = sample_ratio
        self.k = k
        self.precision = precision
        self.token_dtype = token_dtype
        self.sync_bn = sync_bn
        stages = int(math.log(1 / sample_ratio, scale))
        embed_dim = int(embed_dim // 2 ** (stages - 1))
        self.convs = nn.ModuleList()
        self.channel_list = [in_channels]
        for _ in range(stages):
            W = embed_dim
            conv1 = nn.Sequential(nn.Conv2d(in_channels + 3, W, 1, bias=False), nn.Conv2d(W, W, 1, bias=True),
                                  nn.BatchNorm2d(W), nn.ReLU())
            conv2 = nn.Sequential(nn.Conv2d(2 * W, 2 * W, 1, bias=False), nn.BatchNorm2d(2 * W), nn.ReLU(),
                                  nn.Conv2d(2 * W, W, 1, bias=False), nn.BatchNorm2d(W), nn.ReLU())
            self.convs.append(nn.ModuleList([conv1, conv2]))
            self.channel_list.append(W)
            in_channels = W
            embed_dim *= 2
        self.out_channels = self.channel_list[-1]

    def folded(self, device) -> List[fold.PatchMLP]:
        bf16 = _check_precision(self.precision)
        ver = tuple((t._version, t.data_ptr()) for t in list(self.parameters()) + list(self.buffers()))
        cache = self.__dict__.setdefault("_fold_cache", {})
        if cache.get("ver") != ver:
            cache.clear()
            cache["ver"] = ver
            sd = self.state_dict()
            eps = _bn_eps(self)
            cache["host"] = [fold.fold_p3embed_stage(sd, s, eps) for s in range(len(self.convs))]
        if self.precision == "fp32tc":
            return [m.to_x3(device) for m in cache["host"]]
        return [m.to(device, torch.bfloat16 if bf16 else torch.float32) for m in cache["host"]]

    def forward(self, p: torch.Tensor, f: torch.Tensor, start_idx: Optional[List[torch.Tensor]] = None
                ) -> Tuple[List[torch.Tensor], List[torch.Tensor]]:
        if self.training:
            return self._forward_train(p, f, start_idx)
        bf16 = _check_precision(self.precision)
        B, N = int(p.shape[0]), int(p.shape[1])
        out_p, out_f = [p], [f]
        pts = p.float().contiguous()
        feat = f.float().transpose(1, 2).contiguous()
        folded = self.folded(p.device)
        bf16_last = _check_token_dtype(self.token_dtype, self.precision)
        for s, m in enumerate(folded):
            N = N // 4
            G = min(N, int(pts.shape[1]))
            st = None if start_idx is None else start_idx[s]
            cidx, ws = ops.fps_with_knn_prepare(pts, _start(pts, st, device_draw=True), G)
            ctr = ops.gather_points(pts, cidx)
            kidx = ops.knn_query(pts, ws, ctr, self.k, _lib.KNN_P4P_CDIST, True)
            tok = ops.patch_embed(_lib.ROWS_P4P, pts, feat, None, kidx, None, B * G, self.k, m.tensors(), m.meta(), bf16,
                                  bf16_last and s == len(folded) - 1, self.precision == "fp32tc")
            feat = tok.view(B, G, -1)
            pts = ctr
            out_p.append(ctr)
            out_f.append(feat.transpose(1, 2))
        return out_p, out_f


def _p3embed_forward_train(self, p, f, start_idx=None):
    B, N = int(p.shape[0]), int(p.shape[1])
    out_p, out_f = [p], [f]
    pts = p.float()
    feat = f.float().transpose(1, 2)
    for s, (conv1, conv2) in enumerate(self.convs):
        N = N // 4
        G = min(N, int(pts.shape[1]))
        st = None if start_idx is None else start_idx[s]
        with torch.no_grad():
            pd = pts.detach().contiguous()
            cidx, ws = ops.fps_with_knn_prepare(pd, _start(pd, st, device_draw=True), G)
            ctr_nd = ops.gather_points(pd, cidx)
            kidx = ops.knn_query(pd, ws, ctr_nd, self.k, _lib.KNN_P4P_CDIST, True)
        ctr = torch.gather(pts, 1, cidx.unsqueeze(-1).expand(-1, -1, 3))
        rows = train.GatherRowsFn.apply(pts.contiguous(), feat.contiguous(), kidx)
        tok = train.p3stage_train(conv1, conv2, rows, self.k, self.sync_bn)
        feat = tok.view(B, G, -1)
        pts = ctr
        out_p.append(ctr)
        out_f.append(feat.transpose(1, 2))
    return out_p, out_f


P3Embed._forward_train = _p3embed_forward_train


class PointViTTokens(nn.Module):

    def __init__(self, in_channels: int = 3, embed_dim: int = 384, k_neighbors: int = 16, precision: str = "fp32",
                 **p3embed_kwargs):
        super().__init__()
        self.num_features = self.embed_dim = embed_dim
        self.patch_embed = P3Embed(in_channels=in_channels, k=k_neighbors, precision=precision, **p3embed_kwargs)
        self.proj = nn.Linear(self.patch_embed.out_channels, embed_dim)
        self.pos_embed = nn.Sequential(nn.Linear(3, 128, bias=True), nn.GELU(), nn.Linear(128, embed_dim))
        self.cls_token = nn.Parameter(torch.zeros(1, 1, embed_dim))
        self.cls_pos = nn.Parameter(torch.zeros(1, 1, embed_dim))

    def forward(self, p: torch.Tensor, x: Optional[torch.Tensor] = None, start_idx: Optional[List[torch.Tensor]] = None):
        if x is None:
            x = p.transpose(1, 2)
        p_list, x_list = self.patch_embed(p, x, start_idx)
        tokens = x_list[-1].transpose(1, 2)
        if self.training or (torch.is_grad_enabled() and tokens.requires_grad):
            from . import train_vit
            feats, pos = train_vit.token_head_train(self, tokens, p_list[-1])
            return p_list, x_list, feats, pos
        d = lambda t: t.detach()
        feats, pos = ops.token_head(tokens, p_list[-1], d(self.proj.weight), d(self.proj.bias),
                                    d(self.pos_embed[0].weight), d(self.pos_embed[0].bias), d(self.pos_embed[2].weight),
                                    d(self.pos_embed[2].bias), d(self.cls_token), d(self.cls_pos))
        return p_list, x_list, feats, pos
```

### adapting-2d-vits-for-3d-point-cloud-understanding_b200/p3tok/ops.py

```python
from __future__ import annotations

import ctypes
import os
from typing import List, Optional, Sequence, Tuple

import torch

from . import _lib
from ._lib import check

_lib_handle = None


def _L():
    global _lib_handle
    if _lib_handle is None:
        _lib_handle = _lib.lib()
    return _lib_handle


def _stream() -> int:
    return torch.cuda.current_stream().cuda_stream


_PROFILE = None


def set_profile(sink):
    global _PROFILE
    _PROFILE = sink


class _timed:
    def __init__(self, name):
        self.name = name

    def __enter__(self):
        if _PROFILE is not None:
            self.e0 = torch.cuda.Event(enable_timing=True)
            self.e1 = torch.cuda.Event(enable_timing=True)
            self.e0.record(torch.cuda.current_stream())

    def __exit__(self, *a):
        if _PROFILE is not None:
            self.e1.record(torch.cuda.current_stream())
            _PROFILE.append((self.name, self.e0, self.e1))
        return False


def kernel_launches() -> int:
    return int(_L().p3tok_kernel_launches())


def _need_cuda(name: str, *tensors: Optional[torch.Tensor]) -> torch.device:
    dev = None
    for t in tensors:
        if t is None:
            continue
        if not t.is_cuda:
            raise RuntimeError(f"p3tok::{name}: CUDA tensors only (got {t.device}); p3tok has no CPU fallback")
        if dev is None:
            dev = t.device
        elif t.device != dev:
            raise RuntimeError(f"p3tok::{name}: tensors on different devices ({dev} vs {t.device})")
    return dev


def _f32c(name: str, t: torch.Tensor) -> torch.Tensor:
    if t.dtype != torch.float32:
        raise RuntimeError(f"p3tok::{name}: expected float32, got {t.dtype}")
    return t.contiguous()


def _ptr(t: Optional[torch.Tensor]) -> Optional[int]:
    return None if t is None else t.data_ptr()


def _point_stride(x: torch.Tensor) -> Tuple[torch.Tensor, int]:
    if x.dim() != 3 or x.shape[-1] < 3:
        raise RuntimeError(f"expected (B,N,C>=3) points, got {tuple(x.shape)}")
    if x.is_contiguous() and x.shape[-1] in (3, 4):
        return x, int(x.shape[-1])
    if x.shape[-1] == 3 and x.stride(-1) == 1 and x.stride(1) == 4 and x.stride(0) == 4 * x.shape[1]:
        return x, 4
    return x[..., :3].contiguous(), 3


_FPS_CULLED = os.environ.get("P3TOK_FPS_CULLED", "0") != "0"
_FPS_CULLED_MIN_N = int(os.environ.get("P3TOK_FPS_CULLED_MIN_N", "4096"))


def _use_culled_fps(B: int, N: int, npoint: int) -> bool:
    return (_FPS_CULLED and _KNN_SORTED and B > 0 and npoint >= 8 and _FPS_CULLED_MIN_N <= N <= 8192
            and int(_L().p3tok_knn_workspace_bytes(B, N)) > 0)


@torch.library.custom_op("p3tok::fps", mutates_args=(), device_types="cuda")
def fps(x: torch.Tensor, start_idx: torch.Tensor, npoint: int) -> torch.Tensor:
    _need_cuda("fps", x, start_idx)
    B, N = int(x.shape[0]), int(x.shape[1])
    if _use_culled_fps(B, N, npoint):
        return fps_sorted(x, knn_prepare(x), start_idx, npoint)
    return fps_sweep(x, start_idx, npoint)


@fps.register_fake
def _(x, start_idx, npoint):
    return x.new_empty((x.shape[0], npoint), dtype=torch.int64)


@torch.library.custom_op("p3tok::fps_sweep", mutates_args=(), device_types="cuda")
def fps_sweep(x: torch.Tensor, start_idx: torch.Tensor, npoint: int) -> torch.Tensor:
    _need_cuda("fps", x, start_idx)
    B, N = int(x.shape[0]), int(x.shape[1])
    x = x if x.dtype == torch.float32 else x.float()
    x, stride = _point_stride(x)
    start = start_idx.to(torch.int64).contiguous()
    if start.shape != (B,):
        raise RuntimeError(f"p3tok::fps: start_idx must have shape ({B},)")
    out = torch.empty((B, npoint), dtype=torch.int64, device=x.device)
    with torch.cuda.device(x.device), _timed("fps"):
        check(_L().p3tok_fps(x.data_ptr(), B, N, stride, start.data_ptr(), npoint, out.data_ptr(), _stream()), "fps")
    return out


@fps_sweep.register_fake
def _(x, start_idx, npoint):
    return x.new_empty((x.shape[0], npoint), dtype=torch.int64)


@torch.library.custom_op("p3tok::fps_nd", mutates_args=(), device_types="cuda")
def fps_nd(points: torch.Tensor, start_idx: torch.Tensor, npoint: int) -> torch.Tensor:
    _need_cuda("fps_nd", points, start_idx)
    if points.dim() != 3:
        raise RuntimeError(f"p3tok::fps_nd: expected (B,N,D) points, got {tuple(points.shape)}")
    x = (points if points.dtype == torch.float32 else points.float()).contiguous()
    B, N, D = (int(v) for v in x.shape)
    start = start_idx.to(torch.int64).contiguous()
    if start.shape != (B,):
        raise RuntimeError(f"p3tok::fps_nd: start_idx must have shape ({B},)")
    out = torch.empty((B, npoint), dtype=torch.int64, device=x.device)
    ws = torch.empty((B, N), dtype=torch.float32, device=x.device)
    with torch.cuda.device(x.device), _timed("fps"):
        check(_L().p3tok_fps_nd(x.data_ptr(), B, N, D, D, start.data_ptr(), npoint, out.data_ptr(), ws.data_ptr(), _stream()),
              "fps_nd")
    return out


@fps_nd.register_fake
def _(points, start_idx, npoint):
    return points.new_empty((points.shape[0], npoint), dtype=torch.int64)


@torch.library.custom_op("p3tok::square_distance", mutates_args=(), device_types="cuda")
def square_distance(src: torch.Tensor, dst: torch.Tensor) -> torch.Tensor:
    _need_cuda("square_distance", src, dst)
    if src.dim() != 3 or dst.dim() != 3 or src.shape[0] != dst.shape[0] or src.shape[-1] != 3 or dst.shape[-1] != 3:
        raise RuntimeError(f"p3tok::square_distance: expected (B,S,3) and (B,N,3), got {tuple(src.shape)} and {tuple(dst.shape)}")
    if dst.dtype != torch.float32:
        raise RuntimeError(f"p3tok::square_distance: expected float32, got {dst.dtype}")
    c = _f32c("square_distance", src)
    d, stride = _point_stride(dst)
    B, S, N = int(c.shape[0]), int(c.shape[1]), int(d.shape[1])
    out = torch.empty((B, S, N), dtype=torch.float32, device=c.device)
    with torch.cuda.device(c.device), _timed("sqdist"):
        check(_L().p3tok_square_distance(c.data_ptr(), B, S, d.data_ptr(), N, stride, out.data_ptr(), _stream()),
              "square_distance")
    return out


@square_distance.register_fake
def _(src, dst):
    return src.new_empty((src.shape[0], src.shape[1], dst.shape[1]), dtype=torch.float32)


@torch.library.custom_op("p3tok::gather_points", mutates_args=(), device_types="cuda")
def gather_points(x: torch.Tensor, idx: torch.Tensor) -> torch.Tensor:
    _need_cuda("gather_points", x, idx)
    x = _f32c("gather_points", x)
    B, N, C = (int(v) for v in x.shape)
    flat = idx.to(torch.int64).reshape(B, -1).contiguous()
    S = int(flat.shape[1])
    out = torch.empty((B, S, C), dtype=torch.float32, device=x.device)
    with torch.cuda.device(x.device), _timed("gather"):
        check(_L().p3tok_gather_points(x.data_ptr(), B, N, C, flat.data_ptr(), S, out.data_ptr(), _stream()),
              "gather_points")
    return out.view(*idx.shape, C)


@gather_points.register_fake
def _(x, idx):
    return x.new_empty((*idx.shape, x.shape[-1]))


_KNN_SORTED = os.environ.get("P3TOK_KNN_SORTED", "1") != "0"
_OVERLAP = os.environ.get("P3TOK_OVERLAP", "auto")


@torch.library.custom_op("p3tok::knn", mutates_args=(), device_types="cuda")
def knn(x: torch.Tensor, centres: torch.Tensor, k: int, mode: int, int32_out: bool,
        return_dist: bool) -> Tuple[torch.Tensor, torch.Tensor]:
    _need_cuda("knn", x, centres)
    x = x if x.dtype == torch.float32 else x.float()
    x, stride = _point_stride(x)
    c = _f32c("knn", centres[..., :3])
    B, N = int(x.shape[0]), int(x.shape[1])
    if c.dim() != 3 or c.shape[0] != B:
        raise RuntimeError("p3tok::knn: centres must be (B,G,3)")
    G = int(c.shape[1])
    if k > N:
        raise RuntimeError(f"p3tok::knn: selected index k out of range (k={k} > N={N})")
    idx = torch.empty((B, G, k), dtype=torch.int32 if int32_out else torch.int64, device=x.device)
    dist = torch.empty((B, G, k) if return_dist else (0,), dtype=torch.float32, device=x.device)
    ws_bytes = int(_L().p3tok_knn_workspace_bytes(B, N)) if _KNN_SORTED and B * G > 0 else 0
    with torch.cuda.device(x.device), _timed("knn"):
        if ws_bytes > 0:
            ws = torch.empty(ws_bytes, dtype=torch.uint8, device=x.device)
            check(_L().p3tok_knn_sorted(x.data_ptr(), B, N, stride, c.data_ptr(), G, k, mode, idx.data_ptr(),
                                        _lib.I32 if int32_out else _lib.I64, dist.data_ptr() if return_dist else None,
                                        ws.data_ptr(), ws_bytes, _stream()), "knn_sorted")
        else:
            check(_L().p3tok_knn(x.data_ptr(), B, N, stride, c.data_ptr(), G, k, mode, idx.data_ptr(),
                                 _lib.I32 if int32_out else _lib.I64, dist.data_ptr() if return_dist else None,
                                 _stream()), "knn")
    return idx, dist


@knn.register_fake
def _(x, centres, k, mode, int32_out, return_dist):
    B, G = x.shape[0], centres.shape[1]
    return (x.new_empty((B, G, k), dtype=torch.int32 if int32_out else torch.int64),
            x.new_empty((B, G, k) if return_dist else (0,), dtype=torch.float32))


@torch.library.custom_op("p3tok::knn_prepare", mutates_args=(), device_types="cuda")
def knn_prepare(x: torch.Tensor) -> torch.Tensor:
    _need_cuda("knn_prepare", x)
    x_in = x
    x = x if x.dtype == torch.float32 else x.float()
    x, stride = _point_stride(x)
    B, N = int(x.shape[0]), int(x.shape[1])
    ws_bytes = int(_L().p3tok_knn_workspace_bytes(B, N)) if _KNN_SORTED and B > 0 else 0
    ws = torch.empty(max(ws_bytes, 0), dtype=torch.uint8, device=x.device)
    if ws_bytes > 0:
        with torch.cuda.device(x.device), _timed("knn"):
            check(_L().p3tok_knn_prepare(x.data_ptr(), B, N, stride, ws.data_ptr(), ws_bytes, _stream()), "knn_prepare")
        _ws_bind(ws, x_in)
    return ws


@knn_prepare.register_fake
def _(x):
    return x.new_empty((0,), dtype=torch.uint8)


@torch.library.custom_op("p3tok::knn_query", mutates_args=(), device_types="cuda")
def knn_query(x: torch.Tensor, ws: torch.Tensor, centres: torch.Tensor, k: int, mode: int, int32_out: bool) -> torch.Tensor:
    if ws.numel() == 0:
        return knn(x, centres, k, mode, int32_out, False)[0]
    _need_cuda("knn_query", x, ws, centres)
    _ws_check(ws, x)
    c = _f32c("knn_query", centres[..., :3])
    B, N, G = int(x.shape[0]), int(x.shape[1]), int(c.shape[1])
    if c.dim() != 3 or c.shape[0] != B:
        raise RuntimeError("p3tok::knn_query: centres must be (B,G,3)")
    if k > N:
        raise RuntimeError(f"p3tok::knn: selected index k out of range (k={k} > N={N})")
    idx = torch.empty((B, G, k), dtype=torch.int32 if int32_out else torch.int64, device=x.device)
    with torch.cuda.device(x.device), _timed("knn"):
        check(_L().p3tok_knn_query(ws.data_ptr(), int(ws.numel()), B, N, c.data_ptr(), G, k, mode, idx.data_ptr(),
                                   _lib.I32 if int32_out else _lib.I64, None, _stream()), "knn_query")
    return idx


@knn_query.register_fake
def _(x, ws, centres, k, mode, int32_out):
    return x.new_empty((x.shape[0], centres.shape[1], k), dtype=torch.int32 if int32_out else torch.int64)


_WS_OWNER = {}


def _ws_key(x: torch.Tensor):
    return (x.data_ptr(), tuple(x.shape), tuple(x.stride()), x._version)


def _ws_bind(ws: torch.Tensor, x: torch.Tensor) -> None:
    if len(_WS_OWNER) > 64:
        _WS_OWNER.clear()
    _WS_OWNER[ws.data_ptr()] = _ws_key(x)


def _ws_check(ws: torch.Tensor, x: torch.Tensor) -> None:
    owner = _WS_OWNER.get(ws.data_ptr())
    if owner is not None and owner != _ws_key(x):
        raise RuntimeError("p3tok::knn_query: this workspace was prepared from a different (or since modified) point tensor; "
                           "call knn_prepare(x) again")


@torch.library.custom_op("p3tok::fps_sorted", mutates_args=(), device_types="cuda")
def fps_sorted(x: torch.Tensor, ws: torch.Tensor, start_idx: torch.Tensor, npoint: int) -> torch.Tensor:
    _need_cuda("fps_sorted", x, ws, start_idx)
    _ws_check(ws, x)
    B, N = int(x.shape[0]), int(x.shape[1])
    start = start_idx.to(torch.int64).contiguous()
    if start.shape != (B,):
        raise RuntimeError(f"p3tok::fps: start_idx must have shape ({B},)")
    out = torch.empty((B, npoint), dtype=torch.int64, device=x.device)
    with torch.cuda.device(x.device), _timed("fps"):
        check(_L().p3tok_fps_sorted(ws.data_ptr(), int(ws.numel()), B, N, start.data_ptr(), npoint, out.data_ptr(), _stream()),
              "fps_sorted")
    return out


@fps_sorted.register_fake
def _(x, ws, start_idx, npoint):
    return x.new_empty((x.shape[0], npoint), dtype=torch.int64)


def fps_with_knn_prepare(x: torch.Tensor, start_idx: torch.Tensor, npoint: int) -> Tuple[torch.Tensor, torch.Tensor]:
    _need_cuda("fps_with_knn_prepare", x)
    if _use_culled_fps(int(x.shape[0]), int(x.shape[1]), npoint):
        ws = knn_prepare(x)
        return fps_sorted(x, ws, start_idx, npoint), ws
    if _OVERLAP == "0" or (_OVERLAP != "1" and 2 * int(x.shape[0]) > _sm_count(x.device)):
        return fps(x, start_idx, npoint), knn_prepare(x)
    cur = torch.cuda.current_stream(x.device)
    side = _side_stream(x.device)
    side.wait_stream(cur)
    with torch.cuda.stream(side):
        ws = knn_prepare(x)
    idx = fps(x, start_idx, npoint)
    cur.wait_stream(side)
    ws.record_stream(cur)
    return idx, ws


_SIDE = {}
_SMS = {}


def _sm_count(device) -> int:
    key = device.index if device.index is not None else torch.cuda.current_device()
    if key not in _SMS:
        _SMS[key] = torch.cuda.get_device_properties(key).multi_processor_count
    return _SMS[key]


def _side_stream(device) -> torch.cuda.Stream:
    key = (device.index if device.index is not None else torch.cuda.current_device())
    s = _SIDE.get(key)
    if s is None:
        s = _SIDE[key] = torch.cuda.Stream(device=device)
    return s


@torch.library.custom_op("p3tok::morton_order", mutates_args=(), device_types="cuda")
def morton_order(centres: torch.Tensor) -> Tuple[torch.Tensor, torch.Tensor]:
    _need_cuda("morton_order", centres)
    c = _f32c("morton_order", centres)
    B, G = int(c.shape[0]), int(c.shape[1])
    perm = torch.empty((B, G), dtype=torch.int64, device=c.device)
    codes = torch.empty((B, G), dtype=torch.int64, device=c.device)
    with torch.cuda.device(c.device), _timed("morton"):
        check(_L().p3tok_morton_order(c.data_ptr(), B, G, perm.data_ptr(), codes.data_ptr(), _stream()), "morton_order")
    return perm, codes


@morton_order.register_fake
def _(centres):
    s = (centres.shape[0], centres.shape[1])
    return centres.new_empty(s, dtype=torch.int64), centres.new_empty(s, dtype=torch.int64)


@torch.library.custom_op("p3tok::apf_group", mutates_args=(), device_types="cuda")
def apf_group(x: torch.Tensor, fps_idx: torch.Tensor, knn_idx: torch.Tensor,
              perm: Optional[torch.Tensor]) -> Tuple[torch.Tensor, torch.Tensor]:
    _need_cuda("apf_group", x, fps_idx, knn_idx, perm)
    x = _f32c("apf_group", x)
    B, N, C = (int(v) for v in x.shape)
    G, k = int(knn_idx.shape[1]), int(knn_idx.shape[2])
    f = fps_idx.to(torch.int64).contiguous()
    kn = knn_idx.to(torch.int64).contiguous()
    pm = perm.to(torch.int64).contiguous() if perm is not None else None
    neigh = torch.empty((B, G, k, 2 * C), dtype=torch.float32, device=x.device)
    center = torch.empty((B, G, 3), dtype=torch.float32, device=x.device)
    with torch.cuda.device(x.device), _timed("apf_group"):
        check(_L().p3tok_apf_group(x.data_ptr(), B, N, C, f.data_ptr(), kn.data_ptr(), _ptr(pm), G, k,
                                   neigh.data_ptr(), center.data_ptr(), _stream()), "apf_group")
    return neigh, center


@apf_group.register_fake
def _(x, fps_idx, knn_idx, perm):
    B, G, k = knn_idx.shape
    return x.new_empty((B, G, k, 2 * x.shape[-1])), x.new_empty((B, G, 3))


@torch.library.custom_op("p3tok::group_gather", mutates_args=(), device_types="cuda")
def group_gather(pnts: torch.Tensor, feats: torch.Tensor, idx: torch.Tensor) -> Tuple[torch.Tensor, torch.Tensor]:
    _need_cuda("group_gather", pnts, feats, idx)
    p = _f32c("group_gather", pnts)
    f = _f32c("group_gather", feats)
    B, N, _ = (int(v) for v in p.shape)
    D = int(f.shape[-1])
    G, k = int(idx.shape[1]), int(idx.shape[2])
    i32 = idx.to(torch.int32).contiguous()
    gp = torch.empty((B, G, k, 3), dtype=torch.float32, device=p.device)
    gf = torch.empty((B, G, k, D), dtype=torch.float32, device=p.device)
    with torch.cuda.device(p.device), _timed("group_gather"):
        check(_L().p3tok_group_gather(p.data_ptr(), f.data_ptr(), B, N, D, i32.data_ptr(), G, k, gp.data_ptr(),
                                      gf.data_ptr(), _stream()), "group_gather")
    return gp, gf


@group_gather.register_fake
def _(pnts, feats, idx):
    B, G, k = idx.shape
    return pnts.new_empty((B, G, k, 3)), pnts.new_empty((B, G, k, feats.shape[-1]))


def _mlp_struct(weights: Sequence[torch.Tensor], meta: Sequence[int], wdtype: int) -> _lib.MlpStruct:
    m = _lib.MlpStruct()
    cin, n_pre = int(meta[0]), int(meta[1])
    m.cin, m.n_pre = cin, n_pre
    dims = [int(v) for v in meta[2:2 + n_pre]]
    relu = [int(v) for v in meta[2 + n_pre:2 + 2 * n_pre]]
    m.mid_dim, m.out_dim, m.out_relu = (int(v) for v in meta[2 + 2 * n_pre:5 + 2 * n_pre])
    m.wdtype = wdtype
    x3 = wdtype == _lib.BF16X3
    want = torch.float32 if wdtype == _lib.F32 else torch.bfloat16
    kw = (lambda k_: 3 * ((k_ + 63) // 64 * 64)) if x3 else (lambda k_: k_)
    kin = cin
    for i in range(n_pre):
        w, b = weights[2 * i], weights[2 * i + 1]
        if x3 and i == 0 and cin <= 16:
            if w.dtype != torch.float32 or tuple(w.shape) != (dims[i], kin) or not w.is_contiguous():
                raise RuntimeError(f"p3tok::patch_embed: bf16x3 layer 0 weight must be contiguous float32 ({dims[i]},{kin})")
        elif w.dtype != want or tuple(w.shape) != (dims[i], kw(kin)) or not w.is_contiguous():
            raise RuntimeError(f"p3tok::patch_embed: layer {i} weight must be contiguous {want} ({dims[i]},{kw(kin)})")
        if b.dtype != torch.float32 or tuple(b.shape) != (dims[i],):
            raise RuntimeError(f"p3tok::patch_embed: layer {i} bias must be float32 ({dims[i]},)")
        m.pre_dim[i], m.pre_relu[i] = dims[i], relu[i]
        m.w_pre[i], m.b_pre[i] = w.data_ptr(), b.data_ptr()
        kin = dims[i]
    wg, wf, bm, wo, bo = weights[2 * n_pre:2 * n_pre + 5]
    for t, shp, dt, nm in ((wg, (m.mid_dim, kw(kin)), want, "w_mid_g"), (wf, (m.mid_dim, kw(kin)), want, "w_mid_f"),
                           (bm, (m.mid_dim,), torch.float32, "b_mid"), (wo, (m.out_dim, kw(m.mid_dim)), want, "w_out"),
                           (bo, (m.out_dim,), torch.float32, "b_out")):
        if t.dtype != dt or tuple(t.shape) != shp or not t.is_contiguous():
            raise RuntimeError(f"p3tok::patch_embed: {nm} must be contiguous {dt} {shp}, got {t.dtype} {tuple(t.shape)}")
    m.w_mid_g, m.w_mid_f, m.b_mid, m.w_out, m.b_out = (t.data_ptr() for t in (wg, wf, bm, wo, bo))
    return m


@torch.library.custom_op("p3tok::patch_embed", mutates_args=(), device_types="cuda")
def patch_embed(kind: int, x: torch.Tensor, feats: Optional[torch.Tensor], ctr_idx: Optional[torch.Tensor],
                knn_idx: Optional[torch.Tensor], perm: Optional[torch.Tensor], ngroups: int, k: int,
                weights: Sequence[torch.Tensor], meta: Sequence[int], bf16: bool, bf16_tokens: bool = False,
                x3: bool = False) -> torch.Tensor:
    _need_cuda("patch_embed", x, feats, ctr_idx, knn_idx, perm, *weights)
    x = _f32c("patch_embed", x)
    prec = _lib.BF16X3 if x3 else (_lib.BF16 if bf16 else _lib.F32)
    m = _mlp_struct(weights, meta, prec)
    r = _lib.RowsStruct()
    r.kind = kind
    keep = [x]
    if kind == _lib.ROWS_DIRECT:
        if x.dim() != 2 or x.shape[0] != ngroups * k or x.shape[1] != m.cin:
            raise RuntimeError(f"p3tok::patch_embed: rows must be ({ngroups * k},{m.cin}), got {tuple(x.shape)}")
        r.B, r.G, r.N, r.k, r.C, r.D = 1, ngroups, 0, k, 0, 0
    else:
        B, N, C = (int(v) for v in x.shape)
        kn = knn_idx if knn_idx.dtype in (torch.int32, torch.int64) else knn_idx.to(torch.int64)
        kn = kn.contiguous()
        G = int(kn.shape[1])
        if B * G != ngroups or int(kn.shape[2]) != k:
            raise RuntimeError("p3tok::patch_embed: knn_idx shape does not match ngroups/k")
        r.B, r.G, r.N, r.k, r.C = B, G, N, k, C
        r.idx_dtype = _lib.I32 if kn.dtype == torch.int32 else _lib.I64
        r.knn_idx = kn.data_ptr()
        keep.append(kn)
        if kind == _lib.ROWS_APF:
            ci = ctr_idx.to(torch.int64).contiguous()
            r.ctr_idx = ci.data_ptr()
            keep.append(ci)
            if perm is not None:
                pm = perm.to(torch.int64).contiguous()
                r.perm = pm.data_ptr()
                keep.append(pm)
        else:
            f = _f32c("patch_embed", feats)
            r.D = int(f.shape[-1])
            r.feats = f.data_ptr()
            keep.append(f)
    r.x = x.data_ptr()
    L = _L()
    ws_bytes = L.p3tok_patch_embed_workspace_bytes(ctypes.byref(m), ngroups, k, prec)
    if ws_bytes < 0:
        raise RuntimeError("p3tok::patch_embed: bad descriptor")
    ws = torch.empty((max(int(ws_bytes), 256),), dtype=torch.uint8, device=x.device)
    if bf16_tokens and not bf16:
        raise RuntimeError("p3tok::patch_embed: bfloat16 tokens are emitted by the bf16 path only")
    tokens = torch.empty((ngroups, m.out_dim), dtype=torch.bfloat16 if bf16_tokens else torch.float32, device=x.device)
    with torch.cuda.device(x.device), _timed("embed"):
        check(L.p3tok_patch_embed(ctypes.byref(r), ctypes.byref(m), prec, _lib.BF16 if bf16_tokens else _lib.F32, ws.data_ptr(),
                                  int(ws.numel()), tokens.data_ptr(), _stream()), "patch_embed")
    del keep
    return tokens


@patch_embed.register_fake
def _(kind, x, feats, ctr_idx, knn_idx, perm, ngroups, k, weights, meta, bf16, bf16_tokens=False, x3=False):
    n_pre = meta[1]
    return x.new_empty((ngroups, meta[3 + 2 * n_pre]), dtype=torch.bfloat16 if bf16_tokens else torch.float32)


@torch.library.custom_op("p3tok::linear_f32", mutates_args=(), device_types="cuda")
def linear_f32(a: torch.Tensor, w: torch.Tensor, bias: Optional[torch.Tensor], relu: bool) -> torch.Tensor:
    _need_cuda("linear_f32", a, w, bias)
    a2 = _f32c("linear_f32", a).reshape(-1, a.shape[-1])
    w = _f32c("linear_f32", w)
    b = _f32c("linear_f32", bias) if bias is not None else None
    M, K = (int(v) for v in a2.shape)
    N = int(w.shape[0])
    out = torch.empty((M, N), dtype=torch.float32, device=a.device)
    with torch.cuda.device(a.device), _timed("linear_f32"):
        check(_L().p3tok_linear_f32(a2.data_ptr(), M, K, w.data_ptr(), N, _ptr(b), None, 1, int(relu), out.data_ptr(),
                                    _stream()), "linear_f32")
    return out.view(*a.shape[:-1], N)


@linear_f32.register_fake
def _(a, w, bias, relu):
    return a.new_empty((*a.shape[:-1], w.shape[0]))


@torch.library.custom_op("p3tok::linear_bf16", mutates_args=(), device_types="cuda")
def linear_bf16(a: torch.Tensor, w: torch.Tensor, bias: Optional[torch.Tensor], relu: bool,
                want_max32: bool) -> Tuple[torch.Tensor, torch.Tensor, torch.Tensor]:
    _need_cuda("linear_bf16", a, w, bias)
    if a.dtype != torch.bfloat16 or w.dtype != torch.bfloat16:
        raise RuntimeError("p3tok::linear_bf16: operands must be bfloat16")
    a, w = a.contiguous(), w.contiguous()
    b = _f32c("linear_bf16", bias) if bias is not None else None
    M, K = (int(v) for v in a.shape)
    N = int(w.shape[0])
    ob = torch.empty((M, N), dtype=torch.bfloat16, device=a.device)
    of = torch.empty((M, N), dtype=torch.float32, device=a.device)
    om = torch.empty(((M + 31) // 32 if want_max32 else 0, N), dtype=torch.float32, device=a.device)
    with torch.cuda.device(a.device), _timed("linear_bf16"):
        check(_L().p3tok_linear_bf16(a.data_ptr(), M, K, w.data_ptr(), N, _ptr(b), None, 1, int(relu), ob.data_ptr(),
                                     of.data_ptr(), om.data_ptr() if want_max32 else None, _stream()), "linear_bf16")
    return ob, of, om


@linear_bf16.register_fake
def _(a, w, bias, relu, want_max32):
    M, N = a.shape[0], w.shape[0]
    return (a.new_empty((M, N)), a.new_empty((M, N), dtype=torch.float32),
            a.new_empty(((M + 31) // 32 if want_max32 else 0, N), dtype=torch.float32))


@torch.library.custom_op("p3tok::token_head", mutates_args=(), device_types="cuda")
def token_head(tokens: torch.Tensor, centres: torch.Tensor, proj_w: torch.Tensor, proj_b: torch.Tensor,
               pos_w1: torch.Tensor, pos_b1: torch.Tensor, pos_w2: torch.Tensor, pos_b2: torch.Tensor,
               cls_token: torch.Tensor, cls_pos: torch.Tensor) -> Tuple[torch.Tensor, torch.Tensor]:
    ts = [_f32c("token_head", t) for t in (tokens, centres, proj_w, proj_b, pos_w1, pos_b1, pos_w2, pos_b2,
                                           cls_token.reshape(-1), cls_pos.reshape(-1))]
    _need_cuda("token_head", *ts)
    tk, ct, pw, pb, w1, b1, w2, b2, cl, cp = ts
    B, G, W = (int(v) for v in tk.shape)
    E, H = int(pw.shape[0]), int(w1.shape[0])
    if tuple(pw.shape) != (E, W) or tuple(w1.shape) != (H, 3) or tuple(w2.shape) != (E, H) or cl.numel() != E or cp.numel() != E:
        raise RuntimeError("p3tok::token_head: weight shapes do not match tokens/centres")
    feats = torch.empty((B, G + 1, E), dtype=torch.float32, device=tk.device)
    pos = torch.empty((B, G + 1, E), dtype=torch.float32, device=tk.device)
    hidden = torch.empty((B * G, H), dtype=torch.float32, device=tk.device)
    with torch.cuda.device(tk.device), _timed("token_head"):
        check(_L().p3tok_token_head_f32(tk.data_ptr(), ct.data_ptr(), B, G, W, E, H, pw.data_ptr(), pb.data_ptr(),
                                        w1.data_ptr(), b1.data_ptr(), w2.data_ptr(), b2.data_ptr(), cl.data_ptr(),
                                        cp.data_ptr(), hidden.data_ptr(), feats.data_ptr(), pos.data_ptr(), _stream()),
              "token_head")
    return feats, pos


@token_head.register_fake
def _(tokens, centres, proj_w, proj_b, pos_w1, pos_b1, pos_w2, pos_b2, cls_token, cls_pos):
    B, G = tokens.shape[0], tokens.shape[1]
    E = proj_w.shape[0]
    return tokens.new_empty((B, G + 1, E)), tokens.new_empty((B, G + 1, E))


@torch.library.custom_op("p3tok::group_max", mutates_args=(), device_types="cuda")
def group_max(x: torch.Tensor, k: int) -> torch.Tensor:
    _need_cuda("group_max", x)
    x = _f32c("group_max", x)
    C = int(x.shape[-1])
    ng = x.numel() // (C * k)
    out = torch.empty((ng, C), dtype=torch.float32, device=x.device)
    with torch.cuda.device(x.device), _timed("group_max"):
        check(_L().p3tok_group_max(x.data_ptr(), ng, k, C, out.data_ptr(), _stream()), "group_max")
    return out


@group_max.register_fake
def _(x, k):
    return x.new_empty((x.numel() // (x.shape[-1] * k), x.shape[-1]))


VIT_LAYER_TENSORS = ("qkv_w", "qkv_b", "proj_w", "proj_b", "fc1d_w", "fc1d_b", "fc2u_w", "fc2u_b")
_NVT = len(VIT_LAYER_TENSORS)


@torch.library.custom_op("p3tok::apf_vit", mutates_args=(), device_types="cuda")
def apf_vit(tokens: torch.Tensor, params: Sequence[torch.Tensor], heads: int, bottleneck: int, final_w: torch.Tensor,
            final_b: torch.Tensor, ln_eps: float = 1e-5) -> Tuple[torch.Tensor, torch.Tensor]:
    if len(params) % _NVT:
        raise RuntimeError(f"p3tok::apf_vit: expected {_NVT} tensors per layer")
    nl = len(params) // _NVT
    _need_cuda("apf_vit", tokens, final_w, final_b, *params)
    x = _f32c("apf_vit", tokens).clone()
    B, G, D = (int(v) for v in x.shape)
    fw, fb = _f32c("apf_vit", final_w), _f32c("apf_vit", final_b)
    keep = []
    layers = (_lib.VitLayerStruct * max(nl, 1))()
    R = int(bottleneck)
    H = 64
    for li in range(nl):
        for j, name in enumerate(VIT_LAYER_TENSORS):
            t = params[li * _NVT + j]
            want = torch.bfloat16 if name.endswith("_w") else torch.float32
            if t.dtype != want:
                raise RuntimeError(f"p3tok::apf_vit: layer {li} {name} must be {want}, got {t.dtype}")
            t = t.contiguous()
            keep.append(t)
            setattr(layers[li], name, t.data_ptr())
        qkv, proj, fc1d, fc2u = (params[li * _NVT + j] for j in (0, 2, 4, 6))
        HR = int(fc1d.shape[0])
        if tuple(qkv.shape) != (3 * D, D) or tuple(proj.shape) != (D, D) or fc1d.shape[1] != D or tuple(fc2u.shape) != (D, HR):
            raise RuntimeError("p3tok::apf_vit: weight shapes do not match the token width")
        H = HR - R
        for j in (1, 3, 5, 7):
            if params[li * _NVT + j].numel() != params[li * _NVT + j - 1].shape[0]:
                raise RuntimeError("p3tok::apf_vit: bias length does not match its matrix")
    pooled = torch.empty((B, D), dtype=torch.float32, device=x.device)
    with torch.cuda.device(x.device):
        nbytes = int(_L().p3tok_apf_vit_workspace_bytes(B, G, D, H, R))
        ws = torch.empty((max(nbytes, 1024),), dtype=torch.uint8, device=x.device)
        with _timed("apf_vit"):
            check(_L().p3tok_apf_vit_forward(x.data_ptr(), B, G, D, int(heads), H, R, layers, nl, fw.data_ptr(), fb.data_ptr(),
                                             float(ln_eps), pooled.data_ptr(), ws.data_ptr(), nbytes, _stream()), "apf_vit")
    return x, pooled


@apf_vit.register_fake
def _(tokens, params, heads, bottleneck, final_w, final_b, ln_eps=1e-5):
    return tokens.new_empty(tokens.shape), tokens.new_empty((tokens.shape[0], tokens.shape[2]))


@torch.library.custom_op("p3tok::vit_blocks", mutates_args=(), device_types="cuda")
def vit_blocks(feats: torch.Tensor, pos: Optional[torch.Tensor], params: Sequence[torch.Tensor], heads: int, final_w: torch.Tensor,
               final_b: torch.Tensor, ln_eps: float, pool_skip: int) -> Tuple[torch.Tensor, torch.Tensor]:
    if len(params) % _NVT:
        raise RuntimeError(f"p3tok::vit_blocks: expected {_NVT} tensors per layer")
    nl = len(params) // _NVT
    _need_cuda("vit_blocks", feats, pos, final_w, final_b, *params)
    x = _f32c("vit_blocks", feats).clone()
    B, S, D = (int(v) for v in x.shape)
    p = _f32c("vit_blocks", pos) if pos is not None else None
    if p is not None and tuple(p.shape) != (B, S, D):
        raise RuntimeError("p3tok::vit_blocks: pos must have the shape of feats")
    fw, fb = _f32c("vit_blocks", final_w), _f32c("vit_blocks", final_b)
    keep = []
    layers = (_lib.VitLayerStruct * max(nl, 1))()
    H = 64
    for li in range(nl):
        for j, name in enumerate(VIT_LAYER_TENSORS):
            t = params[li * _NVT + j]
            want = torch.bfloat16 if name.endswith("_w") else torch.float32
            if t.dtype != want:
                raise RuntimeError(f"p3tok::vit_blocks: layer {li} {name} must be {want}, got {t.dtype}")
            t = t.contiguous()
            keep.append(t)
            setattr(layers[li], name, t.data_ptr())
        qkv, proj, fc1, fc2 = (params[li * _NVT + j] for j in (0, 2, 4, 6))
        H = int(fc1.shape[0])
        if tuple(qkv.shape) != (3 * D, D) or tuple(proj.shape) != (D, D) or fc1.shape[1] != D or tuple(fc2.shape) != (D, H):
            raise RuntimeError("p3tok::vit_blocks: weight shapes do not match the token width")
    out = torch.empty((B, S, D), dtype=torch.float32, device=x.device)
    pooled = torch.empty((B, D), dtype=torch.float32, device=x.device)
    with torch.cuda.device(x.device):
        nbytes = int(_L().p3tok_apf_vit_workspace_bytes(B, S, D, H, 0))
        ws = torch.empty((max(nbytes, 1024),), dtype=torch.uint8, device=x.device)
        with _timed("vit_blocks"):
            check(_L().p3tok_vit_forward(x.data_ptr(), B, S, D, int(heads), H, layers, nl, _ptr(p), fw.data_ptr(), fb.data_ptr(),
                                         float(ln_eps), out.data_ptr(), pooled.data_ptr(), int(pool_skip), ws.data_ptr(), nbytes,
                                         _stream()), "vit_blocks")
    del keep
    return out, pooled


@vit_blocks.register_fake
def _(feats, pos, params, heads, final_w, final_b, ln_eps, pool_skip):
    return feats.new_empty(feats.shape), feats.new_empty((feats.shape[0], feats.shape[2]))


@torch.library.custom_op("p3tok::layernorm_bf16", mutates_args=(), device_types="cuda")
def layernorm_bf16(x: torch.Tensor, w: Optional[torch.Tensor], b: Optional[torch.Tensor], eps: float) -> torch.Tensor:
    _need_cuda("layernorm_bf16", x, w, b)
    x = _f32c("layernorm_bf16", x)
    w = None if w is None else _f32c("layernorm_bf16", w)
    b = None if b is None else _f32c("layernorm_bf16", b)
    M, D = int(x.shape[0]), int(x.shape[1])
    out = torch.empty((M, D), dtype=torch.bfloat16, device=x.device)
    with torch.cuda.device(x.device), _timed("layernorm_bf16"):
        check(_L().p3tok_layernorm_bf16(x.data_ptr(), M, D, float(eps), _ptr(w), _ptr(b), out.data_ptr(), _stream()),
              "layernorm_bf16")
    return out


@layernorm_bf16.register_fake
def _(x, w, b, eps):
    return x.new_empty(x.shape, dtype=torch.bfloat16)


@torch.library.custom_op("p3tok::attention_bf16", mutates_args=(), device_types="cuda")
def attention_bf16(qkv: torch.Tensor, B: int, G: int, heads: int) -> torch.Tensor:
    _need_cuda("attention_bf16", qkv)
    if qkv.dtype != torch.bfloat16 or qkv.dim() != 2 or qkv.shape[0] != B * G or qkv.shape[1] % 3:
        raise RuntimeError("p3tok::attention_bf16: expected (B*G, 3D) bf16")
    qkv = qkv.contiguous()
    D = int(qkv.shape[1]) // 3
    out = torch.empty((B * G, D), dtype=torch.bfloat16, device=qkv.device)
    with torch.cuda.device(qkv.device), _timed("attention_bf16"):
        check(_L().p3tok_attention_bf16(qkv.data_ptr(), B, G, D, int(heads), out.data_ptr(), _stream()), "attention_bf16")
    return out


@attention_bf16.register_fake
def _(qkv, B, G, heads):
    return qkv.new_empty((qkv.shape[0], qkv.shape[1] // 3))


@torch.library.custom_op("p3tok::linear_bf16_ex", mutates_args=(), device_types="cuda")
def linear_bf16_ex(a: torch.Tensor, w: torch.Tensor, bias: torch.Tensor, act: int, gelu_cols: int,
                   residual: Optional[torch.Tensor], res_mul: float, out_scale: float) -> torch.Tensor:
    _need_cuda("linear_bf16_ex", a, w, bias, residual)
    if a.dtype != torch.bfloat16 or w.dtype != torch.bfloat16:
        raise RuntimeError("p3tok::linear_bf16_ex: bf16 operands expected")
    a, w, bias = a.contiguous(), w.contiguous(), _f32c("linear_bf16_ex", bias)
    M, K, N = int(a.shape[0]), int(a.shape[1]), int(w.shape[0])
    with torch.cuda.device(a.device), _timed("linear_bf16_ex"):
        if residual is None:
            out = torch.empty((M, N), dtype=torch.bfloat16, device=a.device)
            check(_L().p3tok_linear_bf16_ex(a.data_ptr(), M, K, w.data_ptr(), N, bias.data_ptr(), int(act), int(gelu_cols), None,
                                            0.0, 1.0, out.data_ptr(), None, _stream()), "linear_bf16_ex")
        else:
            res = _f32c("linear_bf16_ex", residual)
            if float(res_mul) == 1.0:
                out = res.clone()
                res = out
            else:
                out = torch.empty((M, N), dtype=torch.float32, device=a.device)
            check(_L().p3tok_linear_bf16_ex(a.data_ptr(), M, K, w.data_ptr(), N, bias.data_ptr(), int(act), int(gelu_cols),
                                            res.data_ptr(), float(res_mul), float(out_scale), None, out.data_ptr(), _stream()),
                  "linear_bf16_ex")
    return out


@linear_bf16_ex.register_fake
def _(a, w, bias, act, gelu_cols, residual, res_mul, out_scale):
    return a.new_empty((a.shape[0], w.shape[0]), dtype=torch.bfloat16 if residual is None else torch.float32)
```

### include/p3tok.h

```cpp
#ifndef P3TOK_H_
#define P3TOK_H_

#include <stdint.h>

#ifdef __cplusplus
extern "C" {
#endif

#define P3TOK_ABI_VERSION 2

#if defined(__GNUC__)
#define P3TOK_API __attribute__((visibility("default")))
#else
#define P3TOK_API
#endif

enum p3tok_status {
  P3TOK_OK = 0,
  P3TOK_ERR_INVALID = 1,
  P3TOK_ERR_UNSUPPORTED = 2,
  P3TOK_ERR_CUDA = 3,
  P3TOK_ERR_WORKSPACE = 4
};

enum p3tok_knn_mode {
  P3TOK_KNN_APF_SQ = 0,
  P3TOK_KNN_P4P_CDIST = 1
};

enum p3tok_dtype { P3TOK_F32 = 0, P3TOK_BF16 = 1, P3TOK_I32 = 2, P3TOK_I64 = 3,
                   P3TOK_BF16X3 = 4  };

P3TOK_API int p3tok_abi_version(void);
P3TOK_API const char* p3tok_last_error(void);
P3TOK_API int64_t p3tok_kernel_launches(void);

P3TOK_API int p3tok_fps(const float* x, int64_t B, int64_t N, int64_t pt_stride, const int64_t* start_idx,
              int64_t G, int64_t* out_idx, void* stream);

P3TOK_API int p3tok_fps_sorted(const void* workspace, int64_t workspace_bytes, int64_t B, int64_t N,
                     const int64_t* start_idx, int64_t G, int64_t* out_idx, void* stream);

P3TOK_API int p3tok_fps_nd(const float* x, int64_t B, int64_t N, int64_t D, int64_t pt_stride, const int64_t* start_idx,
                 int64_t G, int64_t* out_idx, float* min_dist_ws, void* stream);

P3TOK_API int p3tok_gather_points(const float* x, int64_t B, int64_t N, int64_t C, const int64_t* idx,
                        int64_t S, float* out, void* stream);

P3TOK_API int p3tok_knn(const float* x, int64_t B, int64_t N, int64_t pt_stride, const float* centres,
              int64_t G, int64_t k, int mode, void* idx_out, int idx_dtype, float* dist_out,
              void* stream);

P3TOK_API int64_t p3tok_knn_workspace_bytes(int64_t B, int64_t N);
P3TOK_API int p3tok_knn_sorted(const float* x, int64_t B, int64_t N, int64_t pt_stride, const float* centres,
                     int64_t G, int64_t k, int mode, void* idx_out, int idx_dtype, float* dist_out,
                     void* workspace, int64_t workspace_bytes, void* stream);

P3TOK_API int p3tok_knn_prepare(const float* x, int64_t B, int64_t N, int64_t pt_stride, void* workspace,
                      int64_t workspace_bytes, void* stream);
P3TOK_API int p3tok_knn_query(const void* workspace, int64_t workspace_bytes, int64_t B, int64_t N, const float* centres,
                    int64_t G, int64_t k, int mode, void* idx_out, int idx_dtype, float* dist_out, void* stream);

P3TOK_API int p3tok_square_distance(const float* src, int64_t B, int64_t S, const float* dst, int64_t N,
                          int64_t dst_stride, float* out, void* stream);

P3TOK_API int p3tok_morton_order(const float* centres, int64_t B, int64_t G, int64_t* perm,
                       int64_t* codes_out, void* stream);

P3TOK_API int p3tok_apf_group(const float* x, int64_t B, int64_t N, int64_t C, const int64_t* fps_idx,
                    const int64_t* knn_idx, const int64_t* perm, int64_t G, int64_t k,
                    float* neigh, float* center, void* stream);

P3TOK_API int p3tok_group_gather(const float* pnts, const float* feats, int64_t B, int64_t N, int64_t D,
                       const int32_t* idx, int64_t G, int64_t k, float* grouped_pnts,
                       float* grouped_feats, void* stream);

typedef struct p3tok_mlp {
  int32_t cin;
  int32_t n_pre;
  int32_t pre_dim[4];
  int32_t pre_relu[4];
  int32_t mid_dim;
  int32_t out_dim;
  int32_t out_relu;
  int32_t wdtype;
  const void* w_pre[4];
  const float* b_pre[4];
  const void* w_mid_g;
  const void* w_mid_f;
  const float* b_mid;
  const void* w_out;
  const float* b_out;
} p3tok_mlp;

typedef struct p3tok_rows {
  int32_t kind;
  int32_t C;
  int32_t D;
  int32_t idx_dtype;
  int64_t B, N, G, k;
  const float* x;
  const float* feats;
  const int64_t* ctr_idx;
  const void* knn_idx;
  const int64_t* perm;
} p3tok_rows;

P3TOK_API int64_t p3tok_patch_embed_workspace_bytes(const p3tok_mlp* mlp, int64_t ngroups, int64_t k,
                                          int precision);

P3TOK_API int p3tok_patch_embed(const p3tok_rows* rows, const p3tok_mlp* mlp, int precision, int tokens_dtype,
                      void* workspace, int64_t workspace_bytes, void* tokens, void* stream);

P3TOK_API int p3tok_linear_f32(const float* A, int64_t M, int64_t K, const float* W, int64_t N,
                     const float* bias, const float* gbias, int64_t rows_per_group, int relu,
                     float* C, void* stream);

P3TOK_API int p3tok_linear_bf16(const void* A, int64_t M, int64_t K, const void* W, int64_t N, const float* bias,
                      const float* gbias, int64_t rows_per_group, int relu, void* out_bf16,
                      float* out_f32, float* out_max32, void* stream);

P3TOK_API int64_t p3tok_linear_x3_workspace_bytes(int64_t M, int64_t K, int64_t N);
P3TOK_API int p3tok_linear_x3_f32(const float* A, int64_t M, int64_t K, const float* W, int64_t N, const float* bias,
                        const float* gbias, int64_t rows_per_group, int relu, float* C, void* workspace,
                        int64_t workspace_bytes, void* stream);

P3TOK_API int p3tok_token_head_f32(const float* tokens, const float* centres, int64_t B, int64_t G, int64_t W, int64_t E,
                         int64_t H, const float* proj_w, const float* proj_b, const float* pos_w1,
                         const float* pos_b1, const float* pos_w2, const float* pos_b2,
                         const float* cls_token, const float* cls_pos, float* hidden_ws, float* feats_out,
                         float* pos_out, void* stream);

typedef struct p3tok_vit_layer {
  const void* qkv_w; const float* qkv_b;
  const void* proj_w; const float* proj_b;
  const void* fc1d_w; const float* fc1d_b;
  const void* fc2u_w; const float* fc2u_b;
} p3tok_vit_layer;

P3TOK_API int64_t p3tok_apf_vit_workspace_bytes(int64_t B, int64_t G, int64_t D, int64_t H, int64_t R);

P3TOK_API int p3tok_apf_vit_forward(float* x, int64_t B, int64_t G, int64_t D, int64_t heads, int64_t H, int64_t R,
                          const p3tok_vit_layer* layers, int64_t n_layers, const float* final_norm_w,
                          const float* final_norm_b, float ln_eps, float* pooled_out, void* workspace,
                          int64_t workspace_bytes, void* stream);

P3TOK_API int p3tok_vit_forward(float* x, int64_t B, int64_t S, int64_t D, int64_t heads, int64_t H,
                      const p3tok_vit_layer* layers, int64_t n_layers, const float* pos, const float* final_norm_w,
                      const float* final_norm_b, float ln_eps, float* out_norm, float* pooled_out, int64_t pool_skip,
                      void* workspace, int64_t workspace_bytes, void* stream);

P3TOK_API int p3tok_layernorm_bf16(const float* x, int64_t M, int64_t D, float eps, const float* w, const float* b,
                         void* out, void* stream);
P3TOK_API int p3tok_attention_bf16(const void* qkv, int64_t B, int64_t G, int64_t D, int64_t heads, void* out, void* stream);
P3TOK_API int p3tok_linear_bf16_ex(const void* A, int64_t M, int64_t K, const void* W, int64_t N, const float* bias, int act,
                         int64_t gelu_cols, const float* residual, float res_mul, float out_scale, void* out_bf16,
                         float* out_f32, void* stream);

P3TOK_API int p3tok_linear_tn_f32(const float* dY, const float* X, int64_t M, int64_t N, int64_t K, float* dW, int accumulate,
                        void* stream);
P3TOK_API int p3tok_colstats_f32(const float* X, int64_t M, int64_t N, double* sum, double* sumsq, void* stream);
P3TOK_API int p3tok_bn_act_f32(const float* Z, int64_t M, int64_t N, const float* mean, const float* rstd, const float* gamma,
                     const float* beta, int relu, float* Y, void* stream);
P3TOK_API int p3tok_bn_bwd_stats_f32(const float* dY, const float* Z, int64_t M, int64_t N, const float* mean, const float* rstd,
                           const float* gamma, const float* beta, int relu, double* s1, double* s2, void* stream);
P3TOK_API int p3tok_bn_bwd_apply_f32(const float* dY, const float* Z, int64_t M, int64_t N, int64_t count, const float* mean,
                           const float* rstd, const float* gamma, const float* beta, int relu, const double* s1,
                           const double* s2, float* dZ, void* stream);
P3TOK_API int p3tok_group_max_arg_f32(const float* X, int64_t G, int64_t k, int64_t C, float* out, int32_t* arg, void* stream);
P3TOK_API int p3tok_group_max_bwd_f32(const float* dOut, const int32_t* arg, int64_t G, int64_t k, int64_t C, int accumulate,
                            float* dX, void* stream);
P3TOK_API int p3tok_group_sum_f32(const float* X, int64_t G, int64_t k, int64_t C, float* out, void* stream);
P3TOK_API int p3tok_scatter_rows_add_f32(const float* dRows, const int32_t* idx, int64_t B, int64_t N, int64_t G, int64_t k,
                               int64_t D, float* dP, float* dF, void* stream);
P3TOK_API int p3tok_build_rows_f32(const p3tok_rows* rows, float* X, void* stream);

P3TOK_API int p3tok_ln_fwd_f32(const float* X, int64_t M, int64_t D, const float* gamma, const float* beta, float eps, float* Y,
                     float* mean, float* rstd, void* stream);
P3TOK_API int p3tok_ln_bwd_f32(const float* dY, const float* X, int64_t M, int64_t D, const float* mean, const float* rstd,
                     const float* gamma, int accumulate, float* dX, void* stream);
P3TOK_API int p3tok_ln_param_grad_f32(const float* dY, const float* X, int64_t M, int64_t D, const float* mean, const float* rstd,
                            double* dgamma, double* dbeta, void* stream);
P3TOK_API int p3tok_attn_fwd_f32(const float* qkv, int64_t B, int64_t G, int64_t heads, int64_t hd, float scale, float* O, float* P,
                       void* stream);
P3TOK_API int p3tok_attn_bwd_f32(const float* qkv, const float* P, const float* dO, int64_t B, int64_t G, int64_t heads, int64_t hd,
                       float scale, float* scratch, float* dqkv, void* stream);
P3TOK_API int p3tok_ew_f32(int op, const float* A, const float* B, float alpha, float beta, int64_t total, int64_t bdiv, float* out,
                 void* stream);

P3TOK_API int p3tok_group_max(const float* in, int64_t ngroups, int64_t k, int64_t C, float* out, void* stream);

#ifdef __cplusplus
}
#endif
#endif
```

Baseline: 154,500.

## Fuse FPS, kNN, centre gather and Morton ordering into one per-cloud kernel

Adds a single kernel per cloud that keeps the points in shared memory. Some warps run farthest point sampling and publish each selected centre through an acquire/release counter, while the other warps run the kNN for those centres at the same time. The centre gather and Morton sort happen at the end of the same kernel. This replaces five separate launches and their global-memory round trips, and overlaps kNN with the serial FPS loop. In exchange, each cloud runs on one CTA with fewer FPS threads, kNN is a brute-force scan, and shared-memory use is large.

```diff
diff --git a/__graft_entry__.py b/__graft_entry__.py
--- a/__graft_entry__.py
+++ b/__graft_entry__.py
@@ -26,19 +26,40 @@
         raise RuntimeError(f"fps_kernel SASS holds {n} fused multiply-adds: ptxas contracted the distance arithmetic, "
                            "FPS would no longer be bit-exact (csrc/fps.cu)")
     print("[build] ok: fps_kernel distance arithmetic is unfused (no FFMA / FFMA2 in its SASS)")
+    bad = fused_group_excess_fmas(path)
+    if bad:
+        raise RuntimeError(f"apf_group_fused_kernel SASS holds fused multiply-adds beyond its kNN dot product and Morton "
+                           f"division: {bad} - FPS would no longer be bit-exact (csrc/group_fused.cu)")
+    print("[build] ok: apf_group_fused_kernel holds no FFMA2 and no FFMA beyond its kNN / Morton budget")
+
+
+def _sass_fma_counts(lib_path: str):
+    import re
+    import subprocess
+    out = subprocess.run(["cuobjdump", "-sass", lib_path], capture_output=True, text=True).stdout
+    counts, fn = {}, None
+    for line in out.splitlines():
+        if "Function :" in line:
+            fn = line.split("Function :", 1)[1].strip()
+            counts.setdefault(fn, [0, 0])
+        elif fn is not None:
+            if re.search(r"\bFFMA2\b", line):
+                counts[fn][1] += 1
+            elif re.search(r"\bFFMA\b", line):
+                counts[fn][0] += 1
+    return counts
 
 
 def fps_fused_multiply_adds(lib_path: str) -> int:
-    import re
-    import subprocess
-    out = subprocess.run(["cuobjdump", "-sass", lib_path], capture_output=True, text=True).stdout
-    n, inside = 0, False
-    for line in out.splitlines():
-        if "Function :" in line:
-            inside = "fps_kernel" in line or "fps_culled_kernel" in line or "fps_nd_kernel" in line
-        elif inside and re.search(r"\bFFMA2?\b", line):
-            n += 1
-    return n
+    return sum(a + b for fn, (a, b) in _sass_fma_counts(lib_path).items()
+               if "fps_kernel" in fn or "fps_culled_kernel" in fn or "fps_nd_kernel" in fn)
+
+
+def fused_group_excess_fmas(lib_path: str) -> dict:
+    counts = _sass_fma_counts(lib_path)
+    morton = [a for fn, (a, _) in counts.items() if "morton_kernel" in fn]
+    budget = 2 * 2 + (max(morton) if morton else 0)
+    return {fn: (a, b) for fn, (a, b) in counts.items() if "apf_group_fused_kernel" in fn and (b > 0 or a > budget)}
 
 
 def smoke() -> None:
diff --git a/adapting-2d-vits-for-3d-point-cloud-understanding_b200/csrc/fps.cu b/adapting-2d-vits-for-3d-point-cloud-understanding_b200/csrc/fps.cu
--- a/adapting-2d-vits-for-3d-point-cloud-understanding_b200/csrc/fps.cu
+++ b/adapting-2d-vits-for-3d-point-cloud-understanding_b200/csrc/fps.cu
@@ -3,7 +3,7 @@
 #include <cooperative_groups.h>
 #include <cuda/ptx>
 
-#include "common.cuh"
+#include "index_device.cuh"
 
 namespace cg = cooperative_groups;
 
@@ -37,13 +37,6 @@
   uint32_t pad[3];
 };
 
-__device__ __forceinline__ void warp_argmax(uint32_t& key, uint32_t& idx) {
-  const uint32_t m = __reduce_max_sync(0xffffffffu, key);
-  const uint32_t cand = (key == m) ? idx : 0xffffffffu;
-  idx = __reduce_min_sync(0xffffffffu, cand);
-  key = m;
-}
-
 __device__ __forceinline__ uint32_t fps_smem_u32(const void* p) { return (uint32_t)__cvta_generic_to_shared(p); }
 __device__ __forceinline__ void fps_push_cand(const FpsCand* local_slot, uint64_t* local_bar, uint32_t dst_cta, const FpsCand& c) {
   uint32_t ra, rb;
@@ -74,17 +67,6 @@
   }
 }
 
-__device__ __forceinline__ void fps_add2(float& o0, float& o1, float a0, float a1, float b0, float b1) {
-  asm("{ .reg .b64 ra, rb, rd; mov.b64 ra, {%2,%3}; mov.b64 rb, {%4,%5}; add.rn.f32x2 rd, ra, rb; mov.b64 {%0,%1}, rd; }"
-      : "=f"(o0), "=f"(o1)
-      : "f"(a0), "f"(a1), "f"(b0), "f"(b1));
-}
-__device__ __forceinline__ void fps_mul2(float& o0, float& o1, float a0, float a1, float b0, float b1) {
-  asm("{ .reg .b64 ra, rb, rd; mov.b64 ra, {%2,%3}; mov.b64 rb, {%4,%5}; mul.rn.f32x2 rd, ra, rb; mov.b64 {%0,%1}, rd; }"
-      : "=f"(o0), "=f"(o1)
-      : "f"(a0), "f"(a1), "f"(b0), "f"(b1));
-}
-
 template <int CL, int PPT = FPS_PPT>
 __global__ void __launch_bounds__(fps_max_threads(PPT), 1)
 fps_kernel(const float* __restrict__ x, int N, int pt_stride, const int64_t* __restrict__ start_idx,
@@ -177,37 +159,8 @@
     if (t == 0 && rank == 0) out_idx[(size_t)cloud * G + g] = far;
     if (g == G - 1) break;
     FPS_T(0);
-    const float ncx = -cx, ncy = -cy, ncz = -cz;
-#pragma unroll
-    for (int j = 0; j < PPT; j += 2) {
-      float dx0, dx1, dy0, dy1, dz0, dz1;
-      fps_add2(dx0, dx1, px[j], px[j + 1], ncx, ncx);
-      fps_add2(dy0, dy1, py[j], py[j + 1], ncy, ncy);
-      fps_add2(dz0, dz1, pz[j], pz[j + 1], ncz, ncz);
-      fps_mul2(dx0, dx1, dx0, dx1, dx0, dx1);
-      fps_mul2(dy0, dy1, dy0, dy1, dy0, dy1);
-      fps_mul2(dz0, dz1, dz0, dz1, dz0, dz1);
-      const float d0 = __fadd_rn(__fadd_rn(dx0, dy0), dz0);
-      const float d1 = __fadd_rn(__fadd_rn(dx1, dy1), dz1);
-      md[j] = fminf(md[j], d0);
-      md[j + 1] = fminf(md[j + 1], d1);
-    }
-    float best = md[0];
-#pragma unroll
-    for (int j = 1; j < PPT; ++j) best = fmaxf(best, md[j]);
-    uint32_t key = best >= 0.f ? __float_as_uint(best) : 0u;
-    uint32_t idx = 0xffffffffu;
-    {
-      const uint32_t wmax = __reduce_max_sync(0xffffffffu, key);
-      if (key == wmax && best >= 0.f) {
-        int besti = PPT - 1;
-#pragma unroll
-        for (int j = PPT - 2; j >= 0; --j) besti = (md[j] == best) ? j : besti;
-        idx = (uint32_t)(p0 + besti * T + t);
-      }
-      idx = __reduce_min_sync(0xffffffffu, idx);
-      key = wmax;
-    }
+    uint32_t key, idx;
+    fps_update_argmax<PPT>(px, py, pz, md, cx, cy, cz, p0, T, t, key, idx);
     const int buf = g & 1;
     FPS_T(1);
     if (lane == 0) wslot[buf * 32 + warp] = make_uint2(key, idx);
diff --git a/adapting-2d-vits-for-3d-point-cloud-understanding_b200/csrc/group.cu b/adapting-2d-vits-for-3d-point-cloud-understanding_b200/csrc/group.cu
--- a/adapting-2d-vits-for-3d-point-cloud-understanding_b200/csrc/group.cu
+++ b/adapting-2d-vits-for-3d-point-cloud-understanding_b200/csrc/group.cu
@@ -1,4 +1,4 @@
-#include "common.cuh"
+#include "index_device.cuh"
 
 namespace p3tok {
 
@@ -57,15 +57,6 @@
   }
 }
 
-__device__ __forceinline__ int64_t part1by2(int64_t n) {
-  n = n & 0x000003ff;
-  n = (n ^ (n << 16)) & 0xff0000ff;
-  n = (n ^ (n << 8)) & 0x0300f00f;
-  n = (n ^ (n << 4)) & 0x030c30c3;
-  n = (n ^ (n << 2)) & 0x09249249;
-  return n;
-}
-
 __global__ void __launch_bounds__(1024)
 morton_kernel(const float* __restrict__ centres, int G, int P2, int64_t* __restrict__ perm,
               int64_t* __restrict__ codes_out) {
@@ -108,15 +99,8 @@
   for (int g = t; g < P2; g += blockDim.x) {
     uint64_t key = 0xffffffffffffffffull;
     if (g < G) {
-      int64_t q[3];
-#pragma unroll
-      for (int a = 0; a < 3; ++a) {
-        const float num = __fsub_rn(Cn[g * 3 + a], mnmx[0][a]);
-        const float den = __fadd_rn(__fsub_rn(mnmx[1][a], mnmx[0][a]), 1e-8f);
-        const float sc = __fmul_rn(__fdiv_rn(num, den), 1023.0f);
-        q[a] = (int64_t)sc;
-      }
-      const int64_t code = (part1by2(q[2]) << 2) + (part1by2(q[1]) << 1) + part1by2(q[0]);
+      const float c[3] = {Cn[g * 3], Cn[g * 3 + 1], Cn[g * 3 + 2]};
+      const int64_t code = morton_code(c, mnmx[0], mnmx[1]);
       if (codes_out) codes_out[(size_t)b * G + g] = code;
       key = ((uint64_t)code << 32) | (uint32_t)g;
     }
diff --git a/adapting-2d-vits-for-3d-point-cloud-understanding_b200/csrc/group_fused.cu b/adapting-2d-vits-for-3d-point-cloud-understanding_b200/csrc/group_fused.cu
--- /dev/null
+++ b/adapting-2d-vits-for-3d-point-cloud-understanding_b200/csrc/group_fused.cu
@@ -0,0 +1,313 @@
+#include <stdlib.h>
+
+#include "index_device.cuh"
+
+namespace p3tok {
+
+constexpr int GF_MAX_N = 8192;
+constexpr int GF_MAX_G = 1024;
+constexpr int GF_MAX_K = 64;
+constexpr int GF_CPW = 2;
+constexpr int GF_TRACE_WORDS = 72;
+
+__device__ __forceinline__ uint32_t gf_smem_u32(const void* p) { return (uint32_t)__cvta_generic_to_shared(p); }
+__device__ __forceinline__ int gf_ld_acquire(const int* p) {
+  int v;
+  asm volatile("ld.acquire.cta.shared::cta.b32 %0, [%1];" : "=r"(v) : "r"(gf_smem_u32(p)) : "memory");
+  return v;
+}
+__device__ __forceinline__ void gf_st_release(int* p, int v) {
+  asm volatile("st.release.cta.shared::cta.b32 [%0], %1;" ::"r"(gf_smem_u32(p)), "r"(v) : "memory");
+}
+
+static size_t gf_smem_bytes(int N, int G, int nk) {
+  int P2 = 1;
+  while (P2 < G) P2 <<= 1;
+  return (size_t)N * 16 + (size_t)P2 * 8 + (size_t)nk * GF_CPW * 64 * 8 + (((size_t)G * 4 + 15) / 16) * 16;
+}
+
+template <int PPT, int KPL, int MAXW>
+__global__ void __launch_bounds__(MAXW * 32, 1)
+apf_group_fused_kernel(const float* __restrict__ x, int N, int pt_stride, const int64_t* __restrict__ start_idx, int G, int k,
+                       int nf, int64_t* __restrict__ fps_out, float* __restrict__ ctr_out, int64_t* __restrict__ knn_out,
+                       int64_t* __restrict__ perm_out, unsigned long long* __restrict__ trace) {
+  extern __shared__ __align__(16) unsigned char smem_raw[];
+  __shared__ uint2 wslot[2 * 32];
+  __shared__ float red[2][3][32];
+  __shared__ float mnmx[2][3];
+  __shared__ int nready;
+
+  const int t = threadIdx.x, lane = t & 31, warp = t >> 5, nwarps = blockDim.x >> 5;
+  const int nk = nwarps - nf;
+  const int cloud = blockIdx.x;
+  int P2 = 1;
+  while (P2 < G) P2 <<= 1;
+  float4* pts = reinterpret_cast<float4*>(smem_raw);
+  uint64_t* keys = reinterpret_cast<uint64_t*>(smem_raw + (size_t)N * 16);
+  uint64_t* kq = keys + P2;
+  int* fidx = reinterpret_cast<int*>(kq + nk * GF_CPW * 64);
+  const bool tr = trace != nullptr && cloud == 0;
+
+  const float* src = x + (size_t)cloud * N * pt_stride;
+  for (int i = t; i < N; i += blockDim.x) {
+    const float px = src[(size_t)i * pt_stride], py = src[(size_t)i * pt_stride + 1], pz = src[(size_t)i * pt_stride + 2];
+    pts[i] = make_float4(px, py, pz, sq3(px, py, pz));
+  }
+  if (t == 0) nready = 0;
+  __syncthreads();
+  if (tr && t == 0) trace[0] = clock64();
+
+  if (warp < nf) {
+    const int T = nf * 32;
+    float px[PPT], py[PPT], pz[PPT], md[PPT];
+#pragma unroll
+    for (int j = 0; j < PPT; ++j) {
+      const int i = j * T + t;
+      if (i < N) {
+        const float4 p = pts[i];
+        px[j] = p.x; py[j] = p.y; pz[j] = p.z;
+        md[j] = 1e10f;
+      } else {
+        px[j] = py[j] = pz[j] = 0.f;
+        md[j] = -2.f;
+      }
+    }
+    int far = (int)start_idx[cloud];
+    far = min(max(far, 0), N - 1);
+    for (int g = 0; g < G; ++g) {
+      if (t == 0) {
+        fidx[g] = far;
+        gf_st_release(&nready, g + 1);
+      }
+      if (g == G - 1) break;
+      const float4 c = pts[far];
+      uint32_t key, idx;
+      fps_update_argmax<PPT>(px, py, pz, md, c.x, c.y, c.z, 0, T, t, key, idx);
+      const int buf = g & 1;
+      if (lane == 0) wslot[buf * 32 + warp] = make_uint2(key, idx);
+      asm volatile("bar.sync 1, %0;" ::"r"(T) : "memory");
+      const uint2 s = (lane < nf) ? wslot[buf * 32 + lane] : make_uint2(0u, 0xffffffffu);
+      key = s.x; idx = s.y;
+      warp_argmax(key, idx);
+      far = (int)min(idx, (uint32_t)(N - 1));
+    }
+    if (tr && t == 0) trace[1] = clock64();
+  } else {
+    const int kw = warp - nf;
+    const int kth_lane = (k - 1) & 31, kth_j = (k - 1) >> 5;
+    long long waited = 0;
+    for (int g0 = kw * GF_CPW; g0 < G; g0 += nk * GF_CPW) {
+      const int glast = min(g0 + GF_CPW, G) - 1;
+      if (gf_ld_acquire(&nready) <= glast) {
+        const long long w0 = tr ? clock64() : 0;
+        while (gf_ld_acquire(&nready) <= glast) __nanosleep(64);
+        if (tr) waited += clock64() - w0;
+      }
+      float4 c[GF_CPW];
+      uint64_t L[GF_CPW][KPL];
+      float thr[GF_CPW];
+      int qn[GF_CPW];
+#pragma unroll
+      for (int u = 0; u < GF_CPW; ++u) {
+        c[u] = pts[fidx[min(g0 + u, glast)]];
+#pragma unroll
+        for (int j = 0; j < KPL; ++j) L[u][j] = KNN_SENTINEL;
+        thr[u] = __int_as_float(0x7f800000);
+        qn[u] = 0;
+      }
+      auto merge = [&](int u, uint64_t (&Lu)[KPL], int cnt) {
+        const uint64_t* q = kq + (kw * GF_CPW + u) * 64;
+        uint64_t v = (lane < cnt) ? q[lane] : KNN_SENTINEL;
+        v = warp_sort_asc(v, lane);
+        list_insert_run<KPL>(Lu, v, lane);
+        uint64_t kth = 0;
+#pragma unroll
+        for (int j = 0; j < KPL; ++j)
+          if (j == kth_j) kth = shfl_u64(Lu[j], kth_lane);
+        const uint32_t ko = (uint32_t)(kth >> 32);
+        return (ko == 0xffffffffu) ? __int_as_float(0x7f800000) : ord2f(ko);
+      };
+#pragma unroll 1
+      for (int i0 = 0; i0 < N; i0 += 32) {
+        const int i = i0 + lane;
+        const bool valid = i < N;
+        const float4 p = pts[valid ? i : 0];
+        float d[GF_CPW];
+        bool pass[GF_CPW];
+        bool any = false;
+#pragma unroll
+        for (int u = 0; u < GF_CPW; ++u) {
+          d[u] = knn_apf_dist(c[u].x, c[u].y, c[u].z, c[u].w, p);
+          pass[u] = valid && (d[u] < thr[u]);
+          any = any || pass[u];
+        }
+        if (!__any_sync(0xffffffffu, any)) continue;
+#pragma unroll
+        for (int u = 0; u < GF_CPW; ++u) {
+          const uint32_t ball = __ballot_sync(0xffffffffu, pass[u]);
+          if (ball == 0) continue;
+          uint64_t* q = kq + (kw * GF_CPW + u) * 64;
+          if (pass[u]) q[qn[u] + __popc(ball & ((1u << lane) - 1u))] = ((uint64_t)f2ord(d[u]) << 32) | (uint32_t)i;
+          qn[u] += __popc(ball);
+          __syncwarp();
+          if (qn[u] >= 32) {
+            thr[u] = merge(u, L[u], 32);
+            __syncwarp();
+            if (lane + 32 < qn[u]) q[lane] = q[lane + 32];
+            qn[u] -= 32;
+            __syncwarp();
+          }
+        }
+      }
+#pragma unroll
+      for (int u = 0; u < GF_CPW; ++u) {
+        if (qn[u] > 0) (void)merge(u, L[u], qn[u]);
+        __syncwarp();
+        if (g0 + u > glast) continue;
+        int64_t* o = knn_out + ((size_t)cloud * G + g0 + u) * k;
+#pragma unroll
+        for (int j = 0; j < KPL; ++j) {
+          const int r = j * 32 + lane;
+          if (r < k) o[r] = (int64_t)(uint32_t)L[u][j];
+        }
+      }
+    }
+    if (tr && lane == 0) {
+      trace[8 + kw] = clock64();
+      trace[40 + kw] = (unsigned long long)waited;
+    }
+  }
+  __syncthreads();
+
+  float mn[3] = {3.4e38f, 3.4e38f, 3.4e38f}, mx[3] = {-3.4e38f, -3.4e38f, -3.4e38f};
+  for (int g = t; g < G; g += blockDim.x) {
+    const int f = fidx[g];
+    const float4 c = pts[f];
+    const size_t o = (size_t)cloud * G + g;
+    fps_out[o] = f;
+    ctr_out[o * 3] = c.x; ctr_out[o * 3 + 1] = c.y; ctr_out[o * 3 + 2] = c.z;
+    const float v[3] = {c.x, c.y, c.z};
+#pragma unroll
+    for (int a = 0; a < 3; ++a) {
+      mn[a] = fminf(mn[a], v[a]);
+      mx[a] = fmaxf(mx[a], v[a]);
+    }
+  }
+#pragma unroll
+  for (int a = 0; a < 3; ++a) {
+#pragma unroll
+    for (int o = 16; o > 0; o >>= 1) {
+      mn[a] = fminf(mn[a], __shfl_xor_sync(0xffffffffu, mn[a], o));
+      mx[a] = fmaxf(mx[a], __shfl_xor_sync(0xffffffffu, mx[a], o));
+    }
+    if (lane == 0) { red[0][a][warp] = mn[a]; red[1][a][warp] = mx[a]; }
+  }
+  __syncthreads();
+  if (warp == 0) {
+#pragma unroll
+    for (int a = 0; a < 3; ++a) {
+      float m0 = lane < nwarps ? red[0][a][lane] : 3.4e38f, m1 = lane < nwarps ? red[1][a][lane] : -3.4e38f;
+#pragma unroll
+      for (int o = 16; o > 0; o >>= 1) {
+        m0 = fminf(m0, __shfl_xor_sync(0xffffffffu, m0, o));
+        m1 = fmaxf(m1, __shfl_xor_sync(0xffffffffu, m1, o));
+      }
+      if (lane == 0) { mnmx[0][a] = m0; mnmx[1][a] = m1; }
+    }
+  }
+  __syncthreads();
+  for (int g = t; g < P2; g += blockDim.x) {
+    uint64_t key = 0xffffffffffffffffull;
+    if (g < G) {
+      const float4 p = pts[fidx[g]];
+      const float c[3] = {p.x, p.y, p.z};
+      key = ((uint64_t)morton_code(c, mnmx[0], mnmx[1]) << 32) | (uint32_t)g;
+    }
+    keys[g] = key;
+  }
+  __syncthreads();
+  for (int kk = 2; kk <= P2; kk <<= 1)
+    for (int j = kk >> 1; j > 0; j >>= 1) {
+      for (int i = t; i < P2; i += blockDim.x) {
+        const int p = i ^ j;
+        if (p > i) {
+          const uint64_t a = keys[i], c = keys[p];
+          const bool up = (i & kk) == 0;
+          if ((a > c) == up) { keys[i] = c; keys[p] = a; }
+        }
+      }
+      __syncthreads();
+    }
+  for (int g = t; g < G; g += blockDim.x) perm_out[(size_t)cloud * G + g] = (int64_t)(keys[g] & 0xffffffffu);
+  if (tr && t == 0) trace[2] = clock64();
+}
+
+template <int PPT, int KPL, int MAXW>
+static int gf_launch(const float* x, int B, int N, int ps, const int64_t* start, int G, int k, int nf, int nk, int64_t* fps_idx,
+                     float* center, int64_t* knn_idx, int64_t* perm, unsigned long long* trace, cudaStream_t s) {
+  static thread_local bool configured[32] = {false};
+  int dev = 0;
+  P3_CUDA(cudaGetDevice(&dev));
+  if (dev < 32 && !configured[dev]) {
+    P3_CUDA((cudaFuncSetAttribute(apf_group_fused_kernel<PPT, KPL, MAXW>, cudaFuncAttributeMaxDynamicSharedMemorySize,
+                                  (int)gf_smem_bytes(GF_MAX_N, GF_MAX_G, MAXW))));
+    configured[dev] = true;
+  }
+  apf_group_fused_kernel<PPT, KPL, MAXW><<<(unsigned)B, (nf + nk) * 32, gf_smem_bytes(N, G, nk), s>>>(
+      x, N, ps, start, G, k, nf, fps_idx, center, knn_idx, perm, trace);
+  P3_LAUNCH_CHECK("apf_group_fused_kernel");
+  return P3TOK_OK;
+}
+
+}
+
+using namespace p3tok;
+
+extern "C" int p3tok_apf_group_indices(const float* x, int64_t B, int64_t N, int64_t pt_stride, const int64_t* start_idx,
+                                       int64_t G, int64_t k, int64_t* fps_idx, float* center, int64_t* knn_idx, int64_t* perm,
+                                       void* stream) {
+  P3_REQUIRE(B >= 0 && N > 0 && G >= 0 && pt_stride >= 3, P3TOK_ERR_INVALID,
+             "apf_group_indices: bad shape B=%lld N=%lld G=%lld stride=%lld", (long long)B, (long long)N, (long long)G,
+             (long long)pt_stride);
+  P3_REQUIRE(k >= 1 && k <= N, P3TOK_ERR_INVALID, "apf_group_indices: k=%lld out of range for N=%lld", (long long)k, (long long)N);
+  P3_REQUIRE(pt_stride <= 4, P3TOK_ERR_UNSUPPORTED, "apf_group_indices: pt_stride %lld > 4", (long long)pt_stride);
+  P3_REQUIRE(N <= GF_MAX_N && G <= GF_MAX_G && k <= GF_MAX_K, P3TOK_ERR_UNSUPPORTED,
+             "apf_group_indices: N=%lld G=%lld k=%lld outside N <= %d, G <= %d, k <= %d", (long long)N, (long long)G, (long long)k,
+             GF_MAX_N, GF_MAX_G, GF_MAX_K);
+  P3_REQUIRE(B < (1ll << 31), P3TOK_ERR_UNSUPPORTED, "apf_group_indices: batch too large");
+  if (B == 0 || G == 0) return P3TOK_OK;
+  P3_REQUIRE(x && start_idx && fps_idx && center && knn_idx && perm, P3TOK_ERR_INVALID, "apf_group_indices: null pointer");
+  const int Ni = (int)N, Gi = (int)G, ki = (int)k, Bi = (int)B, ps = (int)pt_stride;
+  const bool small = Ni <= 2048;
+  const int ppt = small ? 8 : 16, maxw = small && ki <= 32 ? 32 : 24;
+  const int nf = ((Ni + ppt - 1) / ppt + 31) / 32;
+  static int nk_env = -1;
+  if (nk_env < 0) { const char* e = getenv("P3TOK_GROUP_KNN_WARPS"); nk_env = e ? atoi(e) : 0; }
+  const int nk = nk_env >= 1 && nf + nk_env <= maxw ? nk_env : maxw - nf;
+  static int trace_on = -1;
+  if (trace_on < 0) trace_on = getenv("P3TOK_GROUP_TRACE") ? 1 : 0;
+  unsigned long long* trace = nullptr;
+  cudaStream_t s = as_stream(stream);
+  if (trace_on) {
+    P3_CUDA(cudaMalloc(&trace, GF_TRACE_WORDS * 8));
+    P3_CUDA(cudaMemsetAsync(trace, 0, GF_TRACE_WORDS * 8, s));
+  }
+  int rc;
+  if (small)
+    rc = ki <= 32 ? gf_launch<8, 1, 32>(x, Bi, Ni, ps, start_idx, Gi, ki, nf, nk, fps_idx, center, knn_idx, perm, trace, s)
+                  : gf_launch<8, 2, 24>(x, Bi, Ni, ps, start_idx, Gi, ki, nf, nk, fps_idx, center, knn_idx, perm, trace, s);
+  else
+    rc = ki <= 32 ? gf_launch<16, 1, 24>(x, Bi, Ni, ps, start_idx, Gi, ki, nf, nk, fps_idx, center, knn_idx, perm, trace, s)
+                  : gf_launch<16, 2, 24>(x, Bi, Ni, ps, start_idx, Gi, ki, nf, nk, fps_idx, center, knn_idx, perm, trace, s);
+  if (rc || !trace_on) return rc;
+  unsigned long long h[GF_TRACE_WORDS];
+  P3_CUDA(cudaStreamSynchronize(s));
+  P3_CUDA(cudaMemcpy(h, trace, sizeof(h), cudaMemcpyDeviceToHost));
+  P3_CUDA(cudaFree(trace));
+  auto rel = [&](unsigned long long v) { return v ? (long long)(v - h[0]) : -1ll; };
+  fprintf(stderr, "[group_trace] B=%d N=%d G=%d k=%d fps_warps=%d knn_warps=%d fps_done=%lld morton_done=%lld\n", Bi, Ni, Gi, ki,
+          nf, nk, rel(h[1]), rel(h[2]));
+  for (int w = 0; w < nk; ++w)
+    fprintf(stderr, "[group_trace]   knn warp %d done=%lld waited=%lld\n", w, rel(h[8 + w]), (long long)h[40 + w]);
+  return P3TOK_OK;
+}
diff --git a/adapting-2d-vits-for-3d-point-cloud-understanding_b200/csrc/index_device.cuh b/adapting-2d-vits-for-3d-point-cloud-understanding_b200/csrc/index_device.cuh
--- /dev/null
+++ b/adapting-2d-vits-for-3d-point-cloud-understanding_b200/csrc/index_device.cuh
@@ -0,0 +1,140 @@
+#pragma once
+#include "common.cuh"
+
+namespace p3tok {
+
+__device__ __forceinline__ void fps_add2(float& o0, float& o1, float a0, float a1, float b0, float b1) {
+  asm("{ .reg .b64 ra, rb, rd; mov.b64 ra, {%2,%3}; mov.b64 rb, {%4,%5}; add.rn.f32x2 rd, ra, rb; mov.b64 {%0,%1}, rd; }"
+      : "=f"(o0), "=f"(o1)
+      : "f"(a0), "f"(a1), "f"(b0), "f"(b1));
+}
+__device__ __forceinline__ void fps_mul2(float& o0, float& o1, float a0, float a1, float b0, float b1) {
+  asm("{ .reg .b64 ra, rb, rd; mov.b64 ra, {%2,%3}; mov.b64 rb, {%4,%5}; mul.rn.f32x2 rd, ra, rb; mov.b64 {%0,%1}, rd; }"
+      : "=f"(o0), "=f"(o1)
+      : "f"(a0), "f"(a1), "f"(b0), "f"(b1));
+}
+
+template <int PPT>
+__device__ __forceinline__ void fps_update_argmax(const float (&px)[PPT], const float (&py)[PPT], const float (&pz)[PPT],
+                                                  float (&md)[PPT], float cx, float cy, float cz, int p0, int T, int t,
+                                                  uint32_t& key, uint32_t& idx) {
+  const float ncx = -cx, ncy = -cy, ncz = -cz;
+#pragma unroll
+  for (int j = 0; j < PPT; j += 2) {
+    float dx0, dx1, dy0, dy1, dz0, dz1;
+    fps_add2(dx0, dx1, px[j], px[j + 1], ncx, ncx);
+    fps_add2(dy0, dy1, py[j], py[j + 1], ncy, ncy);
+    fps_add2(dz0, dz1, pz[j], pz[j + 1], ncz, ncz);
+    fps_mul2(dx0, dx1, dx0, dx1, dx0, dx1);
+    fps_mul2(dy0, dy1, dy0, dy1, dy0, dy1);
+    fps_mul2(dz0, dz1, dz0, dz1, dz0, dz1);
+    const float d0 = __fadd_rn(__fadd_rn(dx0, dy0), dz0);
+    const float d1 = __fadd_rn(__fadd_rn(dx1, dy1), dz1);
+    md[j] = fminf(md[j], d0);
+    md[j + 1] = fminf(md[j + 1], d1);
+  }
+  float best = md[0];
+#pragma unroll
+  for (int j = 1; j < PPT; ++j) best = fmaxf(best, md[j]);
+  key = best >= 0.f ? __float_as_uint(best) : 0u;
+  idx = 0xffffffffu;
+  const uint32_t wmax = __reduce_max_sync(0xffffffffu, key);
+  if (key == wmax && best >= 0.f) {
+    int besti = PPT - 1;
+#pragma unroll
+    for (int j = PPT - 2; j >= 0; --j) besti = (md[j] == best) ? j : besti;
+    idx = (uint32_t)(p0 + besti * T + t);
+  }
+  idx = __reduce_min_sync(0xffffffffu, idx);
+  key = wmax;
+}
+
+__device__ __forceinline__ void warp_argmax(uint32_t& key, uint32_t& idx) {
+  const uint32_t m = __reduce_max_sync(0xffffffffu, key);
+  const uint32_t cand = (key == m) ? idx : 0xffffffffu;
+  idx = __reduce_min_sync(0xffffffffu, cand);
+  key = m;
+}
+
+constexpr uint64_t KNN_SENTINEL = 0xffffffffffffffffull;
+
+__device__ __forceinline__ float knn_apf_dist(float cx, float cy, float cz, float cn, const float4 p) {
+  const float dot = __fmaf_rn(cz, p.z, __fmaf_rn(cy, p.y, __fmul_rn(cx, p.x)));
+  float tt = __fmul_rn(-2.f, dot);
+  tt = __fadd_rn(tt, cn);
+  return __fadd_rn(__fadd_rn(tt, p.w), 0.f);
+}
+
+__device__ __forceinline__ uint64_t shfl_xor_u64(uint64_t v, int m) {
+  uint32_t lo = (uint32_t)v, hi = (uint32_t)(v >> 32);
+  lo = __shfl_xor_sync(0xffffffffu, lo, m);
+  hi = __shfl_xor_sync(0xffffffffu, hi, m);
+  return ((uint64_t)hi << 32) | lo;
+}
+__device__ __forceinline__ uint64_t shfl_u64(uint64_t v, int src) {
+  uint32_t lo = (uint32_t)v, hi = (uint32_t)(v >> 32);
+  lo = __shfl_sync(0xffffffffu, lo, src);
+  hi = __shfl_sync(0xffffffffu, hi, src);
+  return ((uint64_t)hi << 32) | lo;
+}
+__device__ __forceinline__ uint64_t umin64(uint64_t a, uint64_t b) { return a < b ? a : b; }
+__device__ __forceinline__ uint64_t umax64(uint64_t a, uint64_t b) { return a < b ? b : a; }
+
+__device__ __forceinline__ uint64_t warp_sort_asc(uint64_t v, int lane) {
+#pragma unroll
+  for (int k = 2; k <= 32; k <<= 1) {
+#pragma unroll
+    for (int j = k >> 1; j > 0; j >>= 1) {
+      const uint64_t o = shfl_xor_u64(v, j);
+      const bool up = ((lane & k) == 0);
+      const bool lower = ((lane & j) == 0);
+      v = (up == lower) ? umin64(v, o) : umax64(v, o);
+    }
+  }
+  return v;
+}
+__device__ __forceinline__ uint64_t warp_bitonic_merge_asc(uint64_t v, int lane) {
+#pragma unroll
+  for (int j = 16; j > 0; j >>= 1) {
+    const uint64_t o = shfl_xor_u64(v, j);
+    v = ((lane & j) == 0) ? umin64(v, o) : umax64(v, o);
+  }
+  return v;
+}
+
+template <int KPL>
+__device__ __forceinline__ void list_insert_run(uint64_t (&L)[KPL], uint64_t q, int lane) {
+#pragma unroll
+  for (int j = 0; j < KPL; ++j) {
+    const uint64_t r = shfl_u64(q, 31 - lane);
+    const uint64_t lo = umin64(L[j], r);
+    if (j + 1 < KPL) {
+      const uint64_t hi = umax64(L[j], r);
+      q = warp_bitonic_merge_asc(hi, lane);
+    }
+    L[j] = warp_bitonic_merge_asc(lo, lane);
+  }
+}
+
+__device__ __forceinline__ int64_t part1by2(int64_t n) {
+  n = n & 0x000003ff;
+  n = (n ^ (n << 16)) & 0xff0000ff;
+  n = (n ^ (n << 8)) & 0x0300f00f;
+  n = (n ^ (n << 4)) & 0x030c30c3;
+  n = (n ^ (n << 2)) & 0x09249249;
+  return n;
+}
+
+__device__ __forceinline__ int64_t morton_code(const float (&c)[3], const float* mn, const float* mx) {
+  int64_t q[3];
+#pragma unroll
+  for (int a = 0; a < 3; ++a) {
+    const float num = __fsub_rn(c[a], mn[a]);
+    const float den = __fadd_rn(__fsub_rn(mx[a], mn[a]), 1e-8f);
+    const float sc = __fmul_rn(__fdiv_rn(num, den), 1023.0f);
+    q[a] = (int64_t)sc;
+  }
+  return (part1by2(q[2]) << 2) + (part1by2(q[1]) << 1) + part1by2(q[0]);
+}
+
+}
diff --git a/adapting-2d-vits-for-3d-point-cloud-understanding_b200/csrc/knn.cu b/adapting-2d-vits-for-3d-point-cloud-understanding_b200/csrc/knn.cu
--- a/adapting-2d-vits-for-3d-point-cloud-understanding_b200/csrc/knn.cu
+++ b/adapting-2d-vits-for-3d-point-cloud-understanding_b200/csrc/knn.cu
@@ -1,64 +1,12 @@
 #include <stdlib.h>
 
-#include "common.cuh"
+#include "index_device.cuh"
 
 namespace p3tok {
 
 constexpr int KNN_WARPS = 8;
 constexpr int KNN_CPW = 4;
 constexpr int KNN_TILE = 2048;
-constexpr uint64_t KNN_SENTINEL = 0xffffffffffffffffull;
-
-__device__ __forceinline__ uint64_t shfl_xor_u64(uint64_t v, int m) {
-  uint32_t lo = (uint32_t)v, hi = (uint32_t)(v >> 32);
-  lo = __shfl_xor_sync(0xffffffffu, lo, m);
-  hi = __shfl_xor_sync(0xffffffffu, hi, m);
-  return ((uint64_t)hi << 32) | lo;
-}
-__device__ __forceinline__ uint64_t shfl_u64(uint64_t v, int src) {
-  uint32_t lo = (uint32_t)v, hi = (uint32_t)(v >> 32);
-  lo = __shfl_sync(0xffffffffu, lo, src);
-  hi = __shfl_sync(0xffffffffu, hi, src);
-  return ((uint64_t)hi << 32) | lo;
-}
-__device__ __forceinline__ uint64_t umin64(uint64_t a, uint64_t b) { return a < b ? a : b; }
-__device__ __forceinline__ uint64_t umax64(uint64_t a, uint64_t b) { return a < b ? b : a; }
-
-__device__ __forceinline__ uint64_t warp_sort_asc(uint64_t v, int lane) {
-#pragma unroll
-  for (int k = 2; k <= 32; k <<= 1) {
-#pragma unroll
-    for (int j = k >> 1; j > 0; j >>= 1) {
-      const uint64_t o = shfl_xor_u64(v, j);
-      const bool up = ((lane & k) == 0);
-      const bool lower = ((lane & j) == 0);
-      v = (up == lower) ? umin64(v, o) : umax64(v, o);
-    }
-  }
-  return v;
-}
-__device__ __forceinline__ uint64_t warp_bitonic_merge_asc(uint64_t v, int lane) {
-#pragma unroll
-  for (int j = 16; j > 0; j >>= 1) {
-    const uint64_t o = shfl_xor_u64(v, j);
-    v = ((lane & j) == 0) ? umin64(v, o) : umax64(v, o);
-  }
-  return v;
-}
-
-template <int KPL>
-__device__ __forceinline__ void list_insert_run(uint64_t (&L)[KPL], uint64_t q, int lane) {
-#pragma unroll
-  for (int j = 0; j < KPL; ++j) {
-    const uint64_t r = shfl_u64(q, 31 - lane);
-    const uint64_t lo = umin64(L[j], r);
-    if (j + 1 < KPL) {
-      const uint64_t hi = umax64(L[j], r);
-      q = warp_bitonic_merge_asc(hi, lane);
-    }
-    L[j] = warp_bitonic_merge_asc(lo, lane);
-  }
-}
 
 template <int KPL, int MODE>
 __global__ void __launch_bounds__(KNN_WARPS * 32)
@@ -134,10 +82,7 @@
 #pragma unroll
       for (int c = 0; c < KNN_CPW; ++c) {
         if (MODE == P3TOK_KNN_APF_SQ) {
-          const float dot = __fmaf_rn(c2[c], p.z, __fmaf_rn(c1[c], p.y, __fmul_rn(c0[c], p.x)));
-          float tt = __fmul_rn(-2.f, dot);
-          tt = __fadd_rn(tt, cn[c]);
-          dc[c] = __fadd_rn(__fadd_rn(tt, p.w), 0.f);
+          dc[c] = knn_apf_dist(c0[c], c1[c], c2[c], cn[c], p);
           pc[c] = valid && (dc[c] < thr[c]);
         } else {
           float tt = __fmul_rn(c0[c], p.x);
@@ -430,10 +375,7 @@
     float d;
     bool pass;
     if (MODE == P3TOK_KNN_APF_SQ) {
-      const float dot = __fmaf_rn(c2, p.z, __fmaf_rn(c1, p.y, __fmul_rn(c0, p.x)));
-      float tt = __fmul_rn(-2.f, dot);
-      tt = __fadd_rn(tt, cn);
-      d = __fadd_rn(__fadd_rn(tt, p.w), 0.f);
+      d = knn_apf_dist(c0, c1, c2, cn, p);
       pass = (id >= 0) && (d <= thr);
     } else {
       float tt = __fmul_rn(c0, p.x);
diff --git a/adapting-2d-vits-for-3d-point-cloud-understanding_b200/p3tok/_build.py b/adapting-2d-vits-for-3d-point-cloud-understanding_b200/p3tok/_build.py
--- a/adapting-2d-vits-for-3d-point-cloud-understanding_b200/p3tok/_build.py
+++ b/adapting-2d-vits-for-3d-point-cloud-understanding_b200/p3tok/_build.py
@@ -13,7 +13,7 @@
 LIB_PATH = os.path.join(_PKG, "libp3tok.so")
 OBJ_DIR = os.path.join(CSRC, "_obj")
 
-SOURCES = ["capi.cu", "fps.cu", "fps_culled.cu", "fps_nd.cu", "sqdist.cu", "knn.cu", "group.cu", "mlp_f32.cu", "embed_tc.cu", "embed_fused.cu", "embed_stage.cu", "embed_gather.cu", "vit.cu", "train.cu", "train_vit.cu"]
+SOURCES = ["capi.cu", "fps.cu", "fps_culled.cu", "fps_nd.cu", "sqdist.cu", "knn.cu", "group.cu", "group_fused.cu", "mlp_f32.cu", "embed_tc.cu", "embed_fused.cu", "embed_stage.cu", "embed_gather.cu", "vit.cu", "train.cu", "train_vit.cu"]
 NVCC_FLAGS = [
     "-gencode", "arch=compute_100a,code=sm_100a", "-lineinfo", "-O3", "-std=c++17",
     "--expt-extended-lambda", "--expt-relaxed-constexpr", "-Xcompiler", "-fPIC",
diff --git a/adapting-2d-vits-for-3d-point-cloud-understanding_b200/p3tok/_lib.py b/adapting-2d-vits-for-3d-point-cloud-understanding_b200/p3tok/_lib.py
--- a/adapting-2d-vits-for-3d-point-cloud-understanding_b200/p3tok/_lib.py
+++ b/adapting-2d-vits-for-3d-point-cloud-understanding_b200/p3tok/_lib.py
@@ -56,6 +56,7 @@
     "p3tok_knn_prepare": (_int, [_vp, _i64, _i64, _i64, _vp, _i64, _vp]),
     "p3tok_knn_query": (_int, [_vp, _i64, _i64, _i64, _vp, _i64, _i64, _int, _vp, _int, _vp, _vp]),
     "p3tok_morton_order": (_int, [_vp, _i64, _i64, _vp, _vp, _vp]),
+    "p3tok_apf_group_indices": (_int, [_vp, _i64, _i64, _i64, _vp, _i64, _i64, _vp, _vp, _vp, _vp, _vp]),
     "p3tok_apf_group": (_int, [_vp, _i64, _i64, _i64, _vp, _vp, _vp, _i64, _i64, _vp, _vp, _vp]),
     "p3tok_group_gather": (_int, [_vp, _vp, _i64, _i64, _i64, _vp, _i64, _i64, _vp, _vp, _vp]),
     "p3tok_patch_embed_workspace_bytes": (_i64, [ctypes.POINTER(MlpStruct), _i64, _i64, _int]),
diff --git a/adapting-2d-vits-for-3d-point-cloud-understanding_b200/p3tok/modules.py b/adapting-2d-vits-for-3d-point-cloud-understanding_b200/p3tok/modules.py
--- a/adapting-2d-vits-for-3d-point-cloud-understanding_b200/p3tok/modules.py
+++ b/adapting-2d-vits-for-3d-point-cloud-understanding_b200/p3tok/modules.py
@@ -59,7 +59,10 @@
         self.group_size = group_size
 
     def indices(self, x: torch.Tensor, start_idx: Optional[torch.Tensor] = None):
-        fps_idx, ws = ops.fps_with_knn_prepare(x, _start(x, start_idx), self.num_group)
+        start = _start(x, start_idx)
+        if ops.group_fused_applies(x, self.num_group, self.group_size):
+            return ops.apf_group_indices(x, start, self.num_group, self.group_size)
+        fps_idx, ws = ops.fps_with_knn_prepare(x, start, self.num_group)
         center = ops.gather_points(x, fps_idx)[..., :3].contiguous() if x.shape[-1] != 3 else ops.gather_points(x, fps_idx)
         knn_idx = ops.knn_query(x, ws, center, self.group_size, _lib.KNN_APF_SQ, False)
         perm = ops.morton_order(center)[0]
diff --git a/adapting-2d-vits-for-3d-point-cloud-understanding_b200/p3tok/ops.py b/adapting-2d-vits-for-3d-point-cloud-understanding_b200/p3tok/ops.py
--- a/adapting-2d-vits-for-3d-point-cloud-understanding_b200/p3tok/ops.py
+++ b/adapting-2d-vits-for-3d-point-cloud-understanding_b200/p3tok/ops.py
@@ -371,6 +371,48 @@
 def _(centres):
     s = (centres.shape[0], centres.shape[1])
     return centres.new_empty(s, dtype=torch.int64), centres.new_empty(s, dtype=torch.int64)
+
+
+_GROUP_FUSED = os.environ.get("P3TOK_GROUP_FUSED", "1") != "0"
+GROUP_FUSED_MAX_N, GROUP_FUSED_MAX_G, GROUP_FUSED_MAX_K = 8192, 1024, 64
+
+
+def group_fused_applies(x: torch.Tensor, G: int, k: int) -> bool:
+    if not _GROUP_FUSED or x.dim() != 3 or x.shape[-1] < 3:
+        return False
+    N = int(x.shape[1])
+    return 0 < N <= GROUP_FUSED_MAX_N and 1 <= G <= GROUP_FUSED_MAX_G and 1 <= k <= min(GROUP_FUSED_MAX_K, N)
+
+
+@torch.library.custom_op("p3tok::apf_group_indices", mutates_args=(), device_types="cuda")
+def apf_group_indices(x: torch.Tensor, start_idx: torch.Tensor, G: int,
+                      k: int) -> Tuple[torch.Tensor, torch.Tensor, torch.Tensor, torch.Tensor]:
+    _need_cuda("apf_group_indices", x, start_idx)
+    x = x if x.dtype == torch.float32 else x.float()
+    x, stride = _point_stride(x)
+    B, N = int(x.shape[0]), int(x.shape[1])
+    start = start_idx.to(torch.int64).contiguous()
+    if start.shape != (B,):
+        raise RuntimeError(f"p3tok::apf_group_indices: start_idx must have shape ({B},)")
+    if k > N:
+        raise RuntimeError(f"p3tok::apf_group_indices: selected index k out of range (k={k} > N={N})")
+    dev = x.device
+    fps_idx = torch.empty((B, G), dtype=torch.int64, device=dev)
+    center = torch.empty((B, G, 3), dtype=torch.float32, device=dev)
+    knn_idx = torch.empty((B, G, k), dtype=torch.int64, device=dev)
+    perm = torch.empty((B, G), dtype=torch.int64, device=dev)
+    with torch.cuda.device(dev), _timed("group_idx"):
+        check(_L().p3tok_apf_group_indices(x.data_ptr(), B, N, stride, start.data_ptr(), G, k, fps_idx.data_ptr(),
+                                           center.data_ptr(), knn_idx.data_ptr(), perm.data_ptr(), _stream()),
+              "apf_group_indices")
+    return fps_idx, center, knn_idx, perm
+
+
+@apf_group_indices.register_fake
+def _(x, start_idx, G, k):
+    B = x.shape[0]
+    return (x.new_empty((B, G), dtype=torch.int64), x.new_empty((B, G, 3), dtype=torch.float32),
+            x.new_empty((B, G, k), dtype=torch.int64), x.new_empty((B, G), dtype=torch.int64))
 
 
 @torch.library.custom_op("p3tok::apf_group", mutates_args=(), device_types="cuda")
diff --git a/include/p3tok.h b/include/p3tok.h
--- a/include/p3tok.h
+++ b/include/p3tok.h
@@ -66,6 +66,10 @@
 
 P3TOK_API int p3tok_morton_order(const float* centres, int64_t B, int64_t G, int64_t* perm,
                        int64_t* codes_out, void* stream);
+
+P3TOK_API int p3tok_apf_group_indices(const float* x, int64_t B, int64_t N, int64_t pt_stride, const int64_t* start_idx,
+                            int64_t G, int64_t k, int64_t* fps_idx, float* center, int64_t* knn_idx, int64_t* perm,
+                            void* stream);
 
 P3TOK_API int p3tok_apf_group(const float* x, int64_t B, int64_t N, int64_t C, const int64_t* fps_idx,
                     const int64_t* knn_idx, const int64_t* perm, int64_t G, int64_t k,
diff --git a/profiles/group_fused_time.py b/profiles/group_fused_time.py
--- /dev/null
+++ b/profiles/group_fused_time.py
@@ -0,0 +1,72 @@
+import argparse
+import json
+import os
+import subprocess
+import sys
+
+ROOT = os.path.dirname(os.path.dirname(os.path.abspath(__file__)))
+sys.path.insert(0, os.path.join(ROOT, "adapting-2d-vits-for-3d-point-cloud-understanding_b200"))
+sys.dont_write_bytecode = True
+
+import torch
+
+from p3tok import _lib, ops, synth
+
+
+def timed(fn, iters):
+    for _ in range(3):
+        fn()
+    torch.cuda.synchronize()
+    e0, e1 = torch.cuda.Event(enable_timing=True), torch.cuda.Event(enable_timing=True)
+    e0.record()
+    for _ in range(iters):
+        fn()
+    e1.record()
+    torch.cuda.synchronize()
+    return 1e3 * e0.elapsed_time(e1) / iters
+
+
+def main():
+    ap = argparse.ArgumentParser()
+    ap.add_argument("--workload", default="c2", choices=["c2", "c2c"])
+    ap.add_argument("--iters", type=int, default=200)
+    a = ap.parse_args()
+    B, N, G, k = 128, 2048, 128, 32
+    kind = "uniform" if a.workload == "c2" else "clustered"
+    x = torch.from_numpy(synth.make_cloud(kind, B, N, 1234, 3)).cuda()
+    st = torch.from_numpy(synth.start_indices(B, N, 1234)).cuda()
+    fidx = ops.fps_sweep(x, st, G)
+    ws = ops.knn_prepare(x)
+    ctr = ops.gather_points(x, fidx)
+    parts = {
+        "fps": lambda: ops.fps_sweep(x, st, G),
+        "knn_prepare": lambda: ops.knn_prepare(x),
+        "gather": lambda: ops.gather_points(x, fidx),
+        "knn_query": lambda: ops.knn_query(x, ws, ctr, k, _lib.KNN_APF_SQ, False),
+        "morton": lambda: ops.morton_order(ctr),
+    }
+
+    def separate():
+        f = ops.fps_sweep(x, st, G)
+        w = ops.knn_prepare(x)
+        c = ops.gather_points(x, f)
+        ops.knn_query(x, w, c, k, _lib.KNN_APF_SQ, False)
+        ops.morton_order(c)
+
+    res = {"workload": a.workload, "B": B, "N": N, "G": G, "k": k, "iters": a.iters,
+           "gpu": torch.cuda.get_device_name(0),
+           "knn_warps": int(os.environ.get("P3TOK_GROUP_KNN_WARPS", "8"))}
+    try:
+        res["power_limit"] = subprocess.run(["nvidia-smi", "--query-gpu=power.limit", "--format=csv,noheader", "-i", "0"],
+                                            capture_output=True, text=True, timeout=10).stdout.strip()
+    except Exception:
+        res["power_limit"] = None
+    res["fused_us"] = timed(lambda: ops.apf_group_indices(x, st, G, k), a.iters)
+    res["separate_chain_us"] = timed(separate, a.iters)
+    res["separate_parts_us"] = {n: timed(f, a.iters) for n, f in parts.items()}
+    res["separate_parts_sum_us"] = sum(res["separate_parts_us"].values())
+    print(json.dumps(res), flush=True)
+
+
+if __name__ == "__main__":
+    main()
```

Result: no change. 154,200, median of 6 (-0.1%).
